# VIS4ROB-lab/covins

Hardware: AMD Instinct MI355X
Metric: GBA iterations/sec, 5-agent EuRoC merged map (higher is better)
Workload: dtype f64

## Files before the change

covins_amd/csrc/common.hpp:

```cpp
#pragma once
#include <hip/hip_runtime.h>
#include <atomic>
#include <cstdlib>
#include <stdint.h>

#include <map>
#include <unordered_map>
#include <utility>
#include <vector>

#include "../../include/covgpu.h"

namespace covgpu {

constexpr int kTile = 128;

struct DevProblem {
  int K, A, L, O, I, E, S;
  int D;
  int n;
  int npad;
  int N;
  int vi;
  int lm_group;
  double reproj_loss_a, gravity;

  double *pose, *sb, *lm;
  double *pose_c, *sb_c, *lm_c;
  double *pose0, *sb0, *lm0;
  uint8_t* fixed;
  int* kf_cam;
  double *cam_extr, *cam_intr, *cam_dist;
  int* cam_dist_type;

  int *lm_obs_ptr, *obs_kf, *obs_lm;
  double *obs_u, *obs_v, *obs_sigma;

  int *kf_obs_ptr, *kf_obs_idx;
  double* kobs;
  int *kobs_lm, *obs_zpos;
  int npairs;
  int *pair_ptr, *pair_i, *pair_j;
  int *pair_oa, *pair_ob;
  double *obsZ;
  double *lmRT;
  double *cost_part;

  int *imu_i, *imu_j, *imu_ptr;
  double *imu_samples, *imu_first;
  double *imu_noise;
  double *pre_delta;
  double *pre_J;
  double *pre_P;
  double *pre_W;
  double *pre_bias;

  int *edge_i, *edge_j;
  double *edge_meas, *edge_sqrt_info, *edge_loss_a;

  int nchains;
  int max_chain_len;
  int* perm;
  int* pos_kf;
  int* chain_ptr;
  int* pos_chain_end;

  double* Sred;
  double* bred;
  double *Ad, *Ae;
  double *Bp, *Bs, *Bn;
  int* pos_chain_begin;
  double* bp;
  double* grad;
  double* hdiag;
  double* HllInv;
  double* gn;
  double* step;
  double* vtmp;
  double* Linv;
  double* scal;
  double* part;
  int part_n, part_imu, part_edge, part_vec;
  double *imuAd, *imuBs, *imuCd, *imuG;
  double* edgeOut;
  int *kf_edge_ptr, *kf_edge_ent;
  int nepairs;
  int *epair_ptr, *epair_i, *epair_j, *epair_ent;
  int* flag;

  int shard;
  double* vw;

  int nd, nd_nnodes, nd_nlev, nd_maxd;
  int *nd_vnode, *nd_voff, *nd_vord;
  int *nd_vown;
  int *nd_ndepth, *nd_nI;
  long long* nd_ntab;
  int* nd_abase;
  int* nd_fidx;
  double *nd_M, *nd_rhs, *nd_Linv;
  double* nd_dummy;

  double* tr;
  double* scal_r; int* flag_r;

  int uni;
  int* cam_model;
  double* cam_xi;
};

enum {
  TR_RADIUS = 0, TR_MU, TR_LMDF, TR_COST, TR_ALPHA, TR_GG, TR_GN2, TR_GDOT, TR_DNORM, TR_CG, TR_CN, TR_MODEL, TR_SN, TR_RHO, TR_COSTNEW,
  TR_OK, TR_VALID, TR_ACC, TR_TERM, TR_FNCONV, TR_RETRY, TR_FIRST, TR_INITCOST, TR_REUSE,
  TR_JA, TR_JB, TR_JC, TR_VV, TR_VG, TR_NN, TR_XN2,
  TR_COUNT = 32
};
static_assert(TR_XN2 < TR_COUNT, "trust-region state slots");
struct TrConsts {
  int strategy;
  double max_radius, min_relative_decrease, function_tolerance, parameter_tolerance, gradient_tolerance;
};

__device__ __forceinline__ double* nd_entry(const DevProblem& P, int va, int vb, int ra, int rb) {
  const int na = P.nd_vnode[va], nb = P.nd_vnode[vb];
  if (na < 0 || nb < 0) return P.nd_dummy;
  if (na == nb) {
    const int oa = P.nd_voff[va] + ra, ob = P.nd_voff[vb] + rb;
    const int hi = oa > ob ? oa : ob, lo = oa > ob ? ob : oa;
    return P.nd_M + P.nd_ntab[2 * na] + (size_t)hi * (size_t)P.nd_ntab[2 * na + 1] + lo;
  }
  const int da = P.nd_ndepth[na], db = P.nd_ndepth[nb];
  const int no = da > db ? na : nb, vo = da > db ? va : vb, ro = da > db ? ra : rb;
  const int vA = da > db ? vb : va, rA = da > db ? rb : ra, dA = da > db ? db : da;
  const int base = P.nd_abase[(size_t)no * P.nd_maxd + dA];
  const int row = base < 0 ? -1 : P.nd_fidx[base + P.nd_vord[vA]];
  if (row < 0) return P.nd_dummy;
  return P.nd_M + P.nd_ntab[2 * no] + (size_t)(row + rA) * (size_t)P.nd_ntab[2 * no + 1] + (P.nd_voff[vo] + ro);
}

__device__ __forceinline__ double* c_entry(const DevProblem& P, int pi, int pj, int r, int c) {
  if (P.nd) return nd_entry(P, 2 * pi, 2 * pj, r, c);
  return P.Sred + (size_t)(6 * pi + r) * P.npad + (6 * pj + c);
}

enum { SC_COST = 0, SC_JV2 = 1, SC_GG = 2, SC_GN2 = 3, SC_GDOT = 4, SC_GMAX = 5, SC_GS = 6, SC_SN2 = 7, SC_XN2 = 8,
       SC_VV = 9, SC_VG = 10, SC_NN = 11, SC_JA = 12, SC_JB = 13, SC_JC = 14,
       SC_COUNT = 16 };

struct CholAux;
inline bool first_use_on_device(std::atomic<unsigned long long>& seen) {
  int d = 0;
  if (hipGetDevice(&d) != hipSuccess || d < 0 || d > 63) return true;
  const unsigned long long bit = 1ull << d;
  return (seen.fetch_or(bit, std::memory_order_acq_rel) & bit) == 0;
}
struct DevSignal { long long* flag = nullptr; long long seq = 0; };
inline int env_int(const char* name, int fallback) {
  const char* e = getenv(name);
  return e != nullptr ? atoi(e) : fallback;
}
void launch_kobs_build(const DevProblem& P, int* pair_oa, int* pair_ob, size_t nent, hipStream_t st);
void launch_lm_lin(const DevProblem& P, double mu, hipStream_t st, DevSignal sig = DevSignal());
void launch_lm_build(const DevProblem& P, double mu, hipStream_t st, hipEvent_t pose_system_cleared = nullptr, hipStream_t side = nullptr,
                     hipEvent_t ev_lin = nullptr, hipEvent_t ev_kf = nullptr, CholAux* ax = nullptr);
void launch_lm_backsub(const DevProblem& P, const double* dp, double* out_all, hipStream_t st);
void launch_obs_jvp(const DevProblem& P, const double* v_all, hipStream_t st);
void launch_obs_cost(const DevProblem& P, const double* pose, const double* lm, hipStream_t st);
void launch_obs_linearize(const DevProblem& P, double* r, double* Jp, double* Jl, double* cost, hipStream_t st);
void launch_obs_norms(const DevProblem& P, double* norms, hipStream_t st);
void launch_lm_outliers(const DevProblem& P, double th, unsigned char* erase, int* left, unsigned long long* counts, hipStream_t st);

void launch_preintegrate(const DevProblem& P, hipStream_t st);
void launch_imu_build(const DevProblem& P, hipStream_t st);
void launch_imu_jvp(const DevProblem& P, const double* v_all, hipStream_t st);
void launch_imu_cost(const DevProblem& P, const double* pose, const double* sb, hipStream_t st);
void launch_imu_linearize(const DevProblem& P, double* r, double* J, hipStream_t st);

void launch_edge_build(const DevProblem& P, hipStream_t st);
void launch_edge_jvp(const DevProblem& P, const double* v_all, hipStream_t st);
void launch_edge_cost(const DevProblem& P, const double* pose, hipStream_t st);
void launch_edge_linearize(const DevProblem& P, double* r, double* J, double* cost, hipStream_t st);

void launch_finalize_diag(const DevProblem& P, double mu, int which, hipStream_t st);
void launch_part_clear(const DevProblem& P, int slot0, int nslots, hipStream_t st);
void launch_part_finish(const DevProblem& P, int slot0, int nslots, hipStream_t st);
void launch_imu_gather(const DevProblem& P, int which, hipStream_t st);
void launch_edge_gather(const DevProblem& P, hipStream_t st);
struct PgoPlan;
void launch_pose_graph_solve(const DevProblem& P, double* dst, hipStream_t st, CholAux& ax, PgoPlan* pgo);
void launch_zero_system(const DevProblem& P, hipStream_t st);
enum KernelForm {
  KF_POTRF_PANEL = 0, KF_POTRF_PANEL_FRONTS, KF_POTRF_PANEL4, KF_POTRF_PANEL4_FRONTS, KF_POTRF_SKIPPED,
  KF_TRSM_SUB4_4, KF_TRSM_SUB4_8, KF_TRSM_SUB4_12, KF_TRSM_SUB4_16,
  KF_GEMM_TRI_FULL, KF_GEMM_TRI_QUAD, KF_GEMM_TRI_GRID, KF_GEMM_RECT_FULL, KF_GEMM_RECT_QUAD,
  KF_BULK_ONE_LAUNCH, KF_BULK_TWO_LAUNCHES, KF_LAST_UPDATE_WHOLE, KF_LAST_UPDATE_SPLIT, KF_PANEL_ONE_TILE, KF_KD_CUT, KF_KD_ZERO, KF_GEMM_BETA0,
  KF_BWD_FRONT, KF_BWD_PIPE, KF_BWD_PIPE64, KF_BWD_TREE, KF_BWD_TREE64, KF_BWD_GIVEN, KF_BWD_STEP_SUB,
  KF_ND_EXTEND_REC, KF_ND_EXTEND, KF_ND_EXTEND_SPLIT,
  KF_ND_TOP_PACK, KF_ND_GH, KF_ND_TOP_DAMP, KF_ND_PANEL_XFER, KF_DIST_PANEL,
  KF_PGO_ARROW, KF_PGO_DENSE,
  KF_COUNT
};
extern const char* const kFormNames[KF_COUNT];
struct FormCensus { long long n[KF_COUNT] = {}; };
extern thread_local FormCensus* t_forms;
inline void form_hit(int f, long long k = 1) { if (t_forms != nullptr) t_forms->n[f] += k; }
struct FormScope {
  FormCensus* prev;
  explicit FormScope(FormCensus* c) : prev(t_forms) { t_forms = c; }
  ~FormScope() { t_forms = prev; }
  FormScope(const FormScope&) = delete; FormScope& operator=(const FormScope&) = delete;
};
struct CholAux {
  hipStream_t aux = nullptr, mid = nullptr, head = nullptr;
  hipEvent_t ev_fill = nullptr;
  hipEvent_t ev_xb = nullptr;
  int* bwd_cnt = nullptr;
  double* bwd_scr = nullptr; size_t bwd_scr_elems = 0;
  double* bwd_pipe = nullptr; size_t bwd_pipe_elems = 0;
  bool pipe_broken = false;
  hipEvent_t ev_xa = nullptr;
  hipEvent_t ev_zero = nullptr;
  hipEvent_t ev_lin = nullptr, ev_kf = nullptr;
  std::vector<hipEvent_t> ev, prof_ev, panel_ev;
  std::vector<double> prof_flops;
  std::vector<hipEvent_t> prof_ev2;
  std::vector<double> prof_flops2;
  double potrf_ms = 0, potrf_flops = 0;
  long n_potrf = 0;
  struct TriCache {
    std::vector<int*> list; std::vector<int> count; int key = -1;
    std::vector<int*> listC; std::vector<int> countC;
    int *listA = nullptr, *listB = nullptr; int countA = 0, countB = 0;
    void clear();
  };
  FormCensus forms;
  TriCache tri0;
  std::vector<TriCache> tri_lev;
  void tri_clear();
  void (*reduce)(void* ctx, double* dev, size_t n, int op, hipStream_t st) = nullptr;
  void* reduce_ctx = nullptr;
  int panel_n = 0;
  std::vector<int> panel_tag;
  void mark(hipStream_t s, int tag);
  bool profile = false;
  double syrk_ms = 0, syrk_flops = 0;
  long n_syrk = 0;
  void init();
  void destroy();
// ... 27 lines not shown
  const int *own_g = nullptr, *st_g = nullptr, *own_dims = nullptr, *st_dims = nullptr;
  double* x = nullptr;
  int first = 0;
};
struct DenseBatch {
  int n = 0; size_t sM = 0, sL = 0, sR = 0;
  const int* live = nullptr; int tI = 0; const int* live_h = nullptr;
  const long long* tab = nullptr;
  int tri_slot = -1;
  BwdXfer xfer;
  int split_ta = 0;
  hipEvent_t pre_trsm = nullptr;
  int* bwd_cnt = nullptr;
  double* bwd_scr = nullptr;
  double* bwd_pipe = nullptr;
  int *pipe_dead = nullptr, *pipe_dead_h = nullptr; double pipe_timeout_s = 3.0;
  const int* own_dims_h = nullptr;
  const int* own_dims = nullptr;
  const int* beta0_off = nullptr; const int* beta0 = nullptr;
  const int* plist = nullptr; const int* pbig_h = nullptr; const int* psmall_h = nullptr;
  int own_max = 0;
};
void dense_cholesky_solve_raw(double* S, double* b, double* Linv, int* flag, int npad, hipStream_t st, CholAux& ax, int tstop = -1,
                              bool solve = true, DenseBatch bt = DenseBatch());
struct DistPanels {
  int np = 0;
  const int* const* tri = nullptr;
  const int* tri_cnt = nullptr;
  bool lead = false;
  void (*exchange)(void* ctx, int P) = nullptr;
  void* ctx = nullptr;
};
void dense_cholesky_dist(double* S, double* b, double* Linv, int* flag, int npad, hipStream_t st, CholAux& ax, int tstop, DenseBatch bt,
                         const DistPanels& d);
constexpr int kBwdFrontMaxTiles = 4;
constexpr int kBwdPipeMinTiles = 2;
bool bwd_pipe_on();
void dense_backward_solve(double* S, double* b, double* Linv, int npad, hipStream_t st, int tfact, int tend, DenseBatch bt = DenseBatch());
void launch_potrf_panel(double* S, size_t ld, int t0, int w, double* Linv, int* flag, double* b, int npad, int nbt, size_t sM, size_t sL, size_t sR,
                        hipStream_t st, const long long* btab = nullptr, int nb = -1, const int* own = nullptr, const int* list = nullptr, int n_big = 0,
                        int n_small = 0);
void launch_bwd_given(const double* S, size_t ld, int r0, int r1, double* y, double* x, int ncol, int nbt, size_t sM, size_t sR, hipStream_t st,
                      const long long* btab, const int* live, int tI, BwdXfer xf = BwdXfer());
void launch_bwd_front(const double* S, int tI, int ntiles, int nchunk, double* y, const double* Linv, int nbt, size_t sL, size_t sR, hipStream_t st,
                      const long long* btab, const int* live, BwdXfer xf, int* cnt, double* scr);
void launch_bwd_pipe(const double* S, int tI, int ntiles, int nchunk, double* y, const double* Linv, int nbt, size_t sL, size_t sR, hipStream_t st,
                     const long long* btab, const int* live, BwdXfer xf, double* pipe, int* dead, int* dead_h, double timeout_s);
void launch_pipe_fill(double* buf, size_t n, hipStream_t st);
constexpr int kBwdTreeMax = 8;
constexpr int kPipeChunk = 128;
struct BwdTreeLevel {
  int nbt, T, nchunk, tI, first;
  double* y; size_t bsR; const double* Dinv; size_t bsL; const long long* btab; const int* live;
  size_t scr_off, xpub_off;
};
void launch_bwd_tree(const double* M, const BwdTreeLevel* lev, int nlev, BwdXfer xf, double* pipe, int* dead, int* dead_h, double timeout_s, hipStream_t st,
                     bool form64 = false);
unsigned long long pipe_empty_word();
void launch_trsm_sub(double* S, size_t ld, int t0, int w, int r0, int r1, const double* Linv, double* b, int npad, int nbt, size_t sM, size_t sL,
                     size_t sR, const int* live, int tI, hipStream_t st, bool chain = false, const long long* btab = nullptr, int nb = -1, const int* own = nullptr);
void launch_bwd_step_sub(const double* S, size_t ld, int p, const double* Linv_p, double* y, double* x, int ncol, int nblocks, int nbt, size_t sM,
                         size_t sL, size_t sR, hipStream_t st, const long long* btab = nullptr, const int* live = nullptr, int tI = 0,
                         BwdXfer xf = BwdXfer());

struct PgoHostPlan { std::vector<std::vector<int>> block_kf; std::vector<int> border_kf; };
bool pgo_plan_analyse(int K, int E, const int* ei, const int* ej, PgoHostPlan& out);
struct PgoPlan {
  bool active = false;
  int nblk = 0, nIpad = 0, ntot = 0;
  int nb = 0;
  int* idx = nullptr;
  double *M = nullptr, *rhs = nullptr, *Linv = nullptr;
  int* idx_b = nullptr;
  double *Sb = nullptr, *rhs_b = nullptr, *Linv_b = nullptr;
};
void launch_pgo_block_solve(const DevProblem& P, PgoPlan& plan, hipStream_t st, CholAux& ax);

struct PairLists {
  int npairs = 0; size_t nent = 0;
  int *pair_ptr = nullptr, *pair_i = nullptr, *pair_j = nullptr;
  int *pair_oa = nullptr, *pair_ob = nullptr;
};
bool build_pairs_device(int L, int K, const int* d_lm_obs_ptr, const int* d_obs_kf, const int* d_key_of_kf, bool want_obs, hipStream_t st, PairLists& out);
void launch_obs_unpack(int L, int O, const int* lm_obs_ptr, const double* uv, int* obs_lm, double* u, double* v, int* iota, hipStream_t st);
bool build_kf_lists_device(int O, int K, const int* d_obs_kf, const int* d_iota, int* kf_obs_ptr, int* kf_obs_idx, hipStream_t st);
struct Round2Lists {
  int L2 = 0, O2 = 0;
  double *lm0 = nullptr, *obs_u = nullptr, *obs_v = nullptr, *obs_sigma = nullptr;
  int *lm_obs_ptr = nullptr, *lm_old = nullptr, *obs_kf = nullptr, *obs_lm = nullptr, *kf_obs_ptr = nullptr, *kf_obs_idx = nullptr;
  void free_all() {
    for (void* q : {(void*)lm0, (void*)obs_u, (void*)obs_v, (void*)obs_sigma, (void*)lm_obs_ptr, (void*)lm_old, (void*)obs_kf, (void*)obs_lm, (void*)kf_obs_ptr, (void*)kf_obs_idx})
      if (q) (void)hipFree(q);
  }
};
bool round2_compact_device(int L, int O, int K, const unsigned char* d_erase, const int* d_left, const int* d_obs_kf, const int* d_obs_lm, const double* d_u,
                           const double* d_v, const double* d_sigma, const double* d_lm0, hipStream_t st, Round2Lists& out);

struct NdHostPlan;
constexpr int kExtRec = 144;
struct NdLevel {
  int n = 0, nI = 0, ntot = 0;
  int first = 0;
  size_t rhs_off = 0, linv_off = 0;
  int* live = nullptr;
  std::vector<int> live_h;
  int own_max = 0;
  int* plist = nullptr; std::vector<int> plist_h, pbig, psmall;
  int ext_first = 0, ext_count = 0;
  int ext_countA = 0;
  int split_ta = 0;
  int ext2_first = 0, ext2_count = 0, ext2_countA = 0;
  std::vector<int> dx_first, dx_nt, dx_nr, dt_first, dt_cnt;
  std::vector<const int*> dt_dev;
};
struct NdDev {
  bool active = false;
  int nnodes = 0;
  int top_lev0 = 0;
  std::vector<NdLevel> lev;
  int *own_dims = nullptr, *st_dims = nullptr, *own_g = nullptr, *st_g = nullptr;
  int *gidx = nullptr;
  int tree_levels = 0; int* tree_fill = nullptr; std::vector<int> h_tree_fill;
  int tree_top0 = 0;
  int *cptr = nullptr, *cidx = nullptr;
  int *cptr2 = nullptr, *cidx2 = nullptr;
  int *inv_off = nullptr, *inv = nullptr;
  int *rhs_node = nullptr;
  int *ext = nullptr;
  int *extw = nullptr, *extc = nullptr, *extc2 = nullptr;
  std::vector<int> h_extw, h_extc, h_extc2, h_ext_kind;
  int* extr = nullptr; size_t ext_over = 0; std::vector<int> h_extr;
  int *bb_off = nullptr, *bb = nullptr;
  int *top_var = nullptr, *top_r = nullptr, *top_g = nullptr;
  int ntop = 0;
  int* top_tiles = nullptr; int n_top_tiles = 0; double* top_pack = nullptr;
  std::vector<int> h_top_tiles;
  size_t M_sub = 0, rhs_top = 0, gh_off = 0;
  std::vector<int> h_vnode, h_voff, h_vord, h_vown, h_ndepth, h_nI, h_abase, h_fidx, h_own_dims, h_st_dims, h_own_g, h_st_g, h_gidx, h_cptr, h_cidx, h_cptr2,
      h_cidx2, h_inv_off, h_inv, h_rhs_node, h_ext, h_top_var, h_top_r, h_top_g, h_bb_off, h_bb;
  std::vector<long long> h_ntab;
  bool dist = false, dist_lead = false;
  int* dist_ent = nullptr; int* dist_tri = nullptr; double* dist_buf = nullptr;
  std::vector<int> h_dist_ent, h_dist_tri;
  size_t dist_buf_elems = 0, dist_solve_elems = 0;
  size_t M_elems = 0, rhs_elems = 0, linv_elems = 0;
  double plan_flops = 0;
};
void nd_tables(const NdHostPlan& hp, const int* pos_kf, int D, int rank, NdDev& dev);
void launch_nd_init(const DevProblem& P, const NdDev& nd, hipStream_t st);
void launch_nd_zero(const DevProblem& P, const NdDev& nd, hipStream_t st);
bool launch_nd_solve(const DevProblem& P, NdDev& nd, double* dst, double mu, hipStream_t st, CholAux& ax);

void launch_tail_stats(const DevProblem& P, hipStream_t st);
void launch_tail_jvp(const DevProblem& P, bool two, hipStream_t st);
void launch_tail_cost(const DevProblem& P, hipStream_t st);
void launch_tail_finish(const DevProblem& P, TrConsts tc, int stage, bool two, bool with_logic, int fresh, hipStream_t st);
void launch_tail_logic(const DevProblem& P, TrConsts tc, int stage, int fresh, hipStream_t st);
void launch_tail_apply(const DevProblem& P, hipStream_t st);

void launch_dogleg_stats(const DevProblem& P, hipStream_t st);
void launch_cauchy_vec(const DevProblem& P, hipStream_t st);
void launch_combine_step(const DevProblem& P, double cg, double cn, hipStream_t st);
void launch_tr_after_solve(const DevProblem& P, TrConsts tc, int fresh, hipStream_t st);
void launch_combine_step_dev(const DevProblem& P, hipStream_t st);
void launch_tr_after_model(const DevProblem& P, TrConsts tc, hipStream_t st);
void launch_tr_decide(const DevProblem& P, TrConsts tc, hipStream_t st);
void launch_apply_step(const DevProblem& P, hipStream_t st);
void launch_accept(const DevProblem& P, hipStream_t st);
void launch_tr_accept(const DevProblem& P, hipStream_t st, double* box = nullptr, double seq = 0.0);
void launch_xnorm(const DevProblem& P, hipStream_t st);
void launch_relpose(int num, const int* ptr, const double* pB, const double* pA, const double* kpA, const double* kpB, const double* sigA,
                    const double* sigB, const double* camA, const int* distA, const double* camB, const int* distB, double th, int min_inliers,
                    double* T, unsigned char* outlier, int* inliers, hipStream_t st,
                    const int* modelA = nullptr, const double* xiA = nullptr, const int* modelB = nullptr, const double* xiB = nullptr);
void launch_abspose(int num, const int* ptr, const double* f, const double* P, const double* sig, const unsigned long long* seed, double* T,
                    unsigned char* inlier, int* inliers, int* iterations, int* best_draw, int min_inliers, int max_iterations, double probability,
                    double threshold, int max_n, hipStream_t st);
void launch_p3p(int num, const double* F, const double* P, double* T, int* nsol, int* chosen, hipStream_t st);
constexpr int kMatchScanRows = 256;
size_t match_assign_lds_bytes(int maxA, int maxB);
void launch_match(int mode, int num_jobs, int maxA, int maxB, const unsigned char* desc, const unsigned char* skip, const int* row_ptr,
                  const int* set_a, const int* set_b, const int* out_off, int* lists, int* match, int* dist, int* nmatches, int dcut,
                  float thr, float ratio, hipStream_t st);
void launch_reanchor(int K, const double* pose_old, const double* pose_new, double* vel, int L, const int* ref, double* lm,
                     hipStream_t st);

}
```

covins_amd/csrc/k_inertial.hip:

```cpp
#include "common.hpp"
#include "dev_math.hpp"
#include "reduce.hpp"
#include "inertial_dev.hpp"

namespace covgpu {
using namespace covdev;

__global__ __launch_bounds__(64 * kImuWaves) void k_preintegrate(DevProblem P) {
  __shared__ double sm[kImuWaves][225 * 4 + 270];
  const int lane = threadIdx.x & 63, wave = threadIdx.x >> 6;
  const int f = blockIdx.x * kImuWaves + wave;
  const bool live = f < P.I;
  double* F = sm[wave];
  double* J = F + 225;
  double* C = J + 225;
  double* T = C + 225;
  double* V = T + 225;
  const int fj = live ? P.imu_j[f] : 0;
  const V3 ba = ld3(P.sb + 9 * fj + 3), bg = ld3(P.sb + 9 * fj + 6);
  for (int k = lane; k < 225; k += 64) { F[k] = 0.0; J[k] = (k % 16 == 0) ? 1.0 : 0.0; C[k] = 0.0; }
  for (int k = lane; k < 270; k += 64) V[k] = 0.0;
  V3 dp = v3(0, 0, 0), dv = v3(0, 0, 0);
  Q4 dq = Q4{0, 0, 0, 1};
  double dtsum = 0.0;
// ... 72 lines not shown
    __syncthreads();
    if (on) {
#pragma unroll
      for (int u = 0; u < 4; ++u) {
        const int e = lane + 64 * u;
        if (e < 225) { J[e] = jn[u]; T[e] = tn[u]; }
      }
    }
    __syncthreads();
    if (on) {
#pragma unroll
      for (int u = 0; u < 4; ++u) {
        const int e = lane + 64 * u;
        if (e < 225) {
          const int r = e / 15, c = e - 15 * r;
          double s2 = 0.0;
#pragma unroll
          for (int k = 0; k < 15; ++k) s2 += T[15 * r + k] * F[15 * c + k];
#pragma unroll
          for (int k = 0; k < 18; ++k) s2 += V[18 * r + k] * nd[k / 3] * V[18 * c + k];
          C[e] = s2;
        }
      }
    }
    __syncthreads();
  }
  if (!live) return;
  if (lane == 0) {
    double* d = P.pre_delta + 11 * (size_t)f;
    d[0] = dp.x; d[1] = dp.y; d[2] = dp.z; d[3] = dq.x; d[4] = dq.y; d[5] = dq.z; d[6] = dq.w;
    d[7] = dv.x; d[8] = dv.y; d[9] = dv.z; d[10] = dtsum;
    double* pb = P.pre_bias + 6 * (size_t)f;
    pb[0] = ba.x; pb[1] = ba.y; pb[2] = ba.z; pb[3] = bg.x; pb[4] = bg.y; pb[5] = bg.z;
  }
  for (int k = lane; k < 225; k += 64) { P.pre_J[225 * (size_t)f + k] = J[k]; P.pre_P[225 * (size_t)f + k] = C[k]; }
  __builtin_amdgcn_fence(__ATOMIC_ACQ_REL, "workgroup");
  __builtin_amdgcn_wave_barrier();
  double* Wm = P.pre_W + 225 * (size_t)f;
  if (lane == 0) {
    bool ok = true;
    for (int c = 0; c < 15 && ok; ++c) {
      double dd = C[16 * c];
      for (int k = 0; k < c; ++k) dd -= C[15 * c + k] * C[15 * c + k];
      if (!(dd > 0.0)) { ok = false; break; }
      dd = sqrt(dd);
      C[16 * c] = dd;
      for (int r = c + 1; r < 15; ++r) {
        double s2 = C[15 * r + c];
        for (int k = 0; k < c; ++k) s2 -= C[15 * r + k] * C[15 * c + k];
        C[15 * r + c] = s2 / dd;
      }
    }
    for (int k = 0; k < 225; ++k) F[k] = 0.0;
    if (!ok) atomicAdd(P.flag + 1, 1);
    if (ok)
      for (int c = 0; c < 15; ++c) {
        F[16 * c] = 1.0 / C[16 * c];
        for (int r = c + 1; r < 15; ++r) {
          double s2 = 0.0;
          for (int k = c; k < r; ++k) s2 += C[15 * r + k] * F[15 * k + c];
          F[15 * r + c] = -s2 / C[16 * r];
        }
      }
    for (int k = 0; k < 225; ++k) Wm[k] = F[k];
  }
}

__global__ __launch_bounds__(64 * kImuWaves) void k_imu_build(DevProblem P) {
  __shared__ double sm[kImuWaves][kImuLds];
  const int lane = threadIdx.x & 63, wave = threadIdx.x >> 6;
  const int f = blockIdx.x * kImuWaves + wave;
  const bool live = f < P.I;
  double* sl = sm[wave];
  imu_stage<true>(P, P.pose, P.sb, f, live, lane, sl);
  {
    double c2 = (live && lane < 15) ? 0.5 * sl[1141 + lane] * sl[1141 + lane] : 0.0;
    c2 = wave_sum(c2);
    part_put(P, SC_COST, P.part_imu + blockIdx.x * kImuWaves + wave, c2);
  }
  if (!live) return;
  const double* Jw = sl + 450;
  const double* r = sl + 1141;
  const int i = P.imu_i[f], j = P.imu_j[f];
  const int pi = P.perm[i], pj = P.perm[j];
  const size_t K = (size_t)P.K;
  if (lane < 30) {
    const int a = lane, role = a / 15, la = a % 15;
    double ga = 0.0, haa = 0.0;
    for (int k = 0; k < 15; ++k) { ga += Jw[30 * k + a] * r[k]; haa += Jw[30 * k + a] * Jw[30 * k + a]; }
    double* g = P.imuG + (role * K + (role ? pj : pi)) * 30;
    g[la] = ga; g[15 + la] = haa;
  }
  for (int e = lane; e < 900; e += 64) {
    const int a = e / 30, b = e - 30 * a;
    const int ga_ = a / 15, la = a % 15, gb_ = b / 15, lb = b % 15;
    double h = 0.0;
#pragma unroll
    for (int k = 0; k < 15; ++k) h += Jw[30 * k + a] * Jw[30 * k + b];
    const size_t slot = ga_ * K + (ga_ ? pj : pi);
    if (la < 6 && lb < 6) {
      if (ga_ == gb_) P.imuCd[slot * 36 + 6 * la + lb] = h;
      else if (ga_ == 1) P.imuCd[(2 * K + pj) * 36 + 6 * la + lb] = h;
    } else if (la >= 6 && lb >= 6) {
      if (ga_ == gb_) P.imuAd[slot * 81 + 9 * (la - 6) + (lb - 6)] = h;
      else if (ga_ == 1) P.Ae[(size_t)81 * pj + 9 * (la - 6) + (lb - 6)] = h;
    } else if (la >= 6) {
      if (ga_ == gb_) P.imuBs[slot * 54 + 6 * (la - 6) + lb] = h;
      else if (ga_ == 0) P.Bn[(size_t)54 * pi + 6 * (la - 6) + lb] = h;
      else P.Bp[(size_t)54 * pj + 6 * (la - 6) + lb] = h;
    }
  }
}

__global__ __launch_bounds__(256) void k_imu_gather(DevProblem P, int which) {
  const int t = blockIdx.x * blockDim.x + threadIdx.x;
  const int pos = t / 201, e = t - 201 * pos;
  if (pos >= P.K) return;
  const size_t K = (size_t)P.K, s0 = (size_t)pos, s1 = K + pos;
  if (e < 81) {
    if (which != 0) P.Ad[81 * s0 + e] = P.imuAd[81 * s0 + e] + P.imuAd[81 * s1 + e];
  } else if (e < 135) {
    const int q = e - 81;
    if (which != 0) P.Bs[54 * s0 + q] = P.imuBs[54 * s0 + q] + P.imuBs[54 * s1 + q];
  } else if (e < 171) {
    const int q = e - 135, r = q / 6, c = q - 6 * r;
    if (which != 1) {
      if (c <= r) *c_entry(P, pos, pos, r, c) += P.imuCd[36 * s0 + q] + P.imuCd[36 * s1 + q];
      const double x = P.imuCd[36 * (2 * K + pos) + q];
      if (x != 0.0) *c_entry(P, pos, pos - 1, r, c) += x;
    }
  } else {
    const int q = e - 171, kf = P.pos_kf[pos];
    const int dim = q < 15 ? q : q - 15;
    if (which != 2 && (which == 0) != (dim < 6)) return;
    const double v = P.imuG[30 * s0 + q] + P.imuG[30 * s1 + q];
    if (q < 15) { P.grad[(size_t)15 * kf + q] += v; P.bred[(size_t)15 * kf + q] -= v; }
    else P.hdiag[(size_t)15 * kf + q - 15] += v;
  }
}

__global__ __launch_bounds__(64 * kImuWaves) void k_imu_jvp(DevProblem P, const double* __restrict__ v_all) {
  __shared__ double sm[kImuWaves][kImuLds];
  const int lane = threadIdx.x & 63, wave = threadIdx.x >> 6;
  const int f = blockIdx.x * kImuWaves + wave;
  const bool live = f < P.I;
  double* sl = sm[wave];
  imu_stage<true>(P, P.pose, P.sb, f, live, lane, sl);
  double acc = 0.0;
  if (live && lane < 15) {
    const double* Jw = sl + 450;
    const double* vi = v_all + 15 * (size_t)P.imu_i[f];
    const double* vj = v_all + 15 * (size_t)P.imu_j[f];
    double s2 = 0.0;
    for (int c = 0; c < 15; ++c) s2 += Jw[30 * lane + c] * vi[c] + Jw[30 * lane + 15 + c] * vj[c];
    acc = s2 * s2;
  }
  acc = wave_sum(acc);
  part_put(P, SC_JV2, P.part_imu + blockIdx.x * kImuWaves + wave, acc);
}

__global__ __launch_bounds__(64 * kImuWaves) void k_imu_cost(DevProblem P, const double* __restrict__ pose, const double* __restrict__ sb) {
  __shared__ double sm[kImuWaves][kImuLds];
  const int lane = threadIdx.x & 63, wave = threadIdx.x >> 6;
  const int f = blockIdx.x * kImuWaves + wave;
  const bool live = f < P.I;
  double* sl = sm[wave];
// ... 48 lines not shown
```

covins_amd/csrc/k_pairs.hip:

```cpp
#include <rocprim/device/device_radix_sort.hpp>
#include <rocprim/device/device_run_length_encode.hpp>
#include <rocprim/device/device_scan.hpp>

#include <algorithm>

#include "common.hpp"

namespace covgpu {

__global__ __launch_bounds__(256) void k_pair_count(int L, const int* __restrict__ lm_obs_ptr, const int* __restrict__ obs_kf, const int* __restrict__ key_of_kf,
                                                     unsigned long long* __restrict__ cnt) {
  const int l = blockIdx.x * blockDim.x + threadIdx.x;
  if (l >= L) return;
  const int o0 = lm_obs_ptr[l], o1 = lm_obs_ptr[l + 1];
  unsigned long long n = 0;
  for (int a = o0; a < o1; ++a) {
    const int pa = key_of_kf[obs_kf[a]];
    if (pa < 0) continue;
    for (int b = o0; b < o1; ++b) { const int pb = key_of_kf[obs_kf[b]]; n += (pb >= 0 && pb < pa) ? 1 : 0; }
  }
  cnt[l] = n;
}
__global__ __launch_bounds__(256) void k_pair_emit(int L, const int* __restrict__ lm_obs_ptr, const int* __restrict__ obs_kf, const int* __restrict__ key_of_kf,
                                                    const unsigned long long* __restrict__ off, unsigned long long* __restrict__ keys,
// ... 90 lines not shown
  R2_HIP(hipMalloc((void**)&keepO, (size_t)O * 4)); R2_HIP(hipMalloc((void**)&opos, (size_t)O * 4));
  hipLaunchKernelGGL(k_r2_keep_lm, dim3((L + 255) / 256), dim3(256), 0, st, L, d_left, keepL);
  hipLaunchKernelGGL(k_r2_keep_obs, dim3((O + 255) / 256), dim3(256), 0, st, O, d_erase, d_obs_lm, (const unsigned*)keepL, keepO);
  if (!scan(keepL, lpos, (size_t)L) || !scan(keepO, opos, (size_t)O)) { ok = false; goto done; }
  R2_HIP(hipMemcpyAsync(&tail[0], keepL + (L - 1), 4, hipMemcpyDeviceToHost, st)); R2_HIP(hipMemcpyAsync(&tail[1], lpos + (L - 1), 4, hipMemcpyDeviceToHost, st));
  R2_HIP(hipMemcpyAsync(&tail[2], keepO + (O - 1), 4, hipMemcpyDeviceToHost, st)); R2_HIP(hipMemcpyAsync(&tail[3], opos + (O - 1), 4, hipMemcpyDeviceToHost, st));
  R2_HIP(hipStreamSynchronize(st));
  out.L2 = (int)(tail[0] + tail[1]); out.O2 = (int)(tail[2] + tail[3]);
  {
    const size_t L2 = (size_t)std::max(out.L2, 1), O2 = (size_t)std::max(out.O2, 1);
    R2_HIP(hipMalloc((void**)&out.lm0, 3 * L2 * 8)); R2_HIP(hipMalloc((void**)&out.lm_obs_ptr, (L2 + 1) * 4)); R2_HIP(hipMalloc((void**)&out.lm_old, L2 * 4));
    R2_HIP(hipMalloc((void**)&out.obs_kf, O2 * 4)); R2_HIP(hipMalloc((void**)&out.obs_lm, O2 * 4));
    R2_HIP(hipMalloc((void**)&out.obs_u, O2 * 8)); R2_HIP(hipMalloc((void**)&out.obs_v, O2 * 8)); R2_HIP(hipMalloc((void**)&out.obs_sigma, O2 * 8));
    R2_HIP(hipMalloc((void**)&out.kf_obs_ptr, ((size_t)K + 1) * 4)); R2_HIP(hipMalloc((void**)&out.kf_obs_idx, O2 * 4));
    R2_HIP(hipMalloc((void**)&nobs, L2 * 4)); R2_HIP(hipMalloc((void**)&nw, L2 * 4)); R2_HIP(hipMalloc((void**)&nscan, L2 * 4));
    R2_HIP(hipMalloc((void**)&iota, O2 * 4)); R2_HIP(hipMalloc((void**)&keys2, O2 * 4));
    R2_HIP(hipMalloc((void**)&kcnt, (size_t)K * 4)); R2_HIP(hipMalloc((void**)&kscan, (size_t)K * 4));
    R2_HIP(hipMemsetAsync(kcnt, 0, (size_t)K * 4, st));
    R2_HIP(hipMemsetAsync(out.lm_obs_ptr, 0, (L2 + 1) * 4, st)); R2_HIP(hipMemsetAsync(out.kf_obs_ptr, 0, ((size_t)K + 1) * 4, st));
  }
  if (out.L2 > 0 && out.O2 > 0) {
    hipLaunchKernelGGL(k_r2_gather_lm, dim3((L + 255) / 256), dim3(256), 0, st, L, (const unsigned*)keepL, (const unsigned*)lpos, d_left, d_lm0, out.lm0, nobs, out.lm_old);
    hipLaunchKernelGGL(k_r2_gather_obs, dim3((O + 255) / 256), dim3(256), 0, st, O, (const unsigned*)keepO, (const unsigned*)opos, (const unsigned*)lpos, d_obs_kf, d_obs_lm,
                       d_u, d_v, d_sigma, out.obs_kf, out.obs_lm, out.obs_u, out.obs_v, out.obs_sigma, iota);
    hipLaunchKernelGGL(k_r2_widen, dim3((out.L2 + 255) / 256), dim3(256), 0, st, out.L2, (const int*)nobs, nw);
    if (!scan(nw, nscan, (size_t)out.L2)) { ok = false; goto done; }
    hipLaunchKernelGGL(k_r2_ptr, dim3((out.L2 + 255) / 256), dim3(256), 0, st, out.L2, (const unsigned*)nscan, (const unsigned*)nw, out.lm_obs_ptr);
    hipLaunchKernelGGL(k_r2_kf_count, dim3((out.O2 + 255) / 256), dim3(256), 0, st, out.O2, (const int*)out.obs_kf, kcnt);
    if (!scan(kcnt, kscan, (size_t)K)) { ok = false; goto done; }
    hipLaunchKernelGGL(k_r2_ptr, dim3((K + 255) / 256), dim3(256), 0, st, K, (const unsigned*)kscan, (const unsigned*)kcnt, out.kf_obs_ptr);
    {
      size_t b = 0;
      R2_HIP(rocprim::radix_sort_pairs(nullptr, b, out.obs_kf, keys2, iota, out.kf_obs_idx, (size_t)out.O2, 0u, (unsigned)kbits, st));
      if (!need_tmp(b)) { ok = false; goto done; }
      R2_HIP(rocprim::radix_sort_pairs(tmp, b, out.obs_kf, keys2, iota, out.kf_obs_idx, (size_t)out.O2, 0u, (unsigned)kbits, st));
    }
  }
  R2_HIP(hipStreamSynchronize(st));
done:
  for (void* q : {(void*)keepL, (void*)keepO, (void*)lpos, (void*)opos, (void*)kcnt, (void*)kscan, (void*)nw, (void*)nscan, (void*)nobs, (void*)iota, (void*)keys2, tmp}) if (q) (void)hipFree(q);
  if (!ok) { out.free_all(); out = Round2Lists(); }
  return ok;
}

__global__ __launch_bounds__(256) void k_obs_unpack(int L, int O, const int* __restrict__ lm_obs_ptr, const double* __restrict__ uv, int* __restrict__ obs_lm,
                                                     double* __restrict__ u, double* __restrict__ v, int* __restrict__ iota) {
  const int t = blockIdx.x * 256 + threadIdx.x;
  if (t < O) { u[t] = uv[2 * (size_t)t]; v[t] = uv[2 * (size_t)t + 1]; iota[t] = t; }
  if (t < L) for (int o = lm_obs_ptr[t]; o < lm_obs_ptr[t + 1]; ++o) obs_lm[o] = t;
}
bool build_kf_lists_device(int O, int K, const int* d_obs_kf, const int* d_iota, int* kf_obs_ptr, int* kf_obs_idx, hipStream_t st) {
  bool ok = true;
  unsigned *kcnt = nullptr, *kscan = nullptr; int* keys2 = nullptr; void* tmp = nullptr;
  int kbits = 1;
  while ((1 << kbits) < K) ++kbits;
  if (hipMemsetAsync(kf_obs_ptr, 0, ((size_t)K + 1) * 4, st) != hipSuccess) return false;
  if (O <= 0) return true;
  if (hipMalloc((void**)&kcnt, (size_t)K * 4) != hipSuccess || hipMalloc((void**)&kscan, (size_t)K * 4) != hipSuccess || hipMalloc((void**)&keys2, (size_t)O * 4) != hipSuccess) ok = false;
  if (ok) {
    (void)hipMemsetAsync(kcnt, 0, (size_t)K * 4, st);
    hipLaunchKernelGGL(k_r2_kf_count, dim3((O + 255) / 256), dim3(256), 0, st, O, d_obs_kf, kcnt);
    size_t b1 = 0, b2 = 0;
    ok = rocprim::exclusive_scan(nullptr, b1, kcnt, kscan, 0u, (size_t)K, rocprim::plus<unsigned>(), st) == hipSuccess &&
         rocprim::radix_sort_pairs(nullptr, b2, d_obs_kf, keys2, d_iota, kf_obs_idx, (size_t)O, 0u, (unsigned)kbits, st) == hipSuccess;
    const size_t b = std::max(b1, b2);
    if (ok && hipMalloc(&tmp, std::max<size_t>(b, 16)) != hipSuccess) ok = false;
    if (ok) {
      size_t bb = b1;
      ok = rocprim::exclusive_scan(tmp, bb, kcnt, kscan, 0u, (size_t)K, rocprim::plus<unsigned>(), st) == hipSuccess;
      hipLaunchKernelGGL(k_r2_ptr, dim3((K + 255) / 256), dim3(256), 0, st, K, (const unsigned*)kscan, (const unsigned*)kcnt, kf_obs_ptr);
      bb = b2;
      ok = ok && rocprim::radix_sort_pairs(tmp, bb, d_obs_kf, keys2, d_iota, kf_obs_idx, (size_t)O, 0u, (unsigned)kbits, st) == hipSuccess;
      ok = ok && hipStreamSynchronize(st) == hipSuccess;
    }
  }
  for (void* q : {(void*)kcnt, (void*)kscan, (void*)keys2, tmp}) if (q) (void)hipFree(q);
  return ok;
}
void launch_obs_unpack(int L, int O, const int* lm_obs_ptr, const double* uv, int* obs_lm, double* u, double* v, int* iota, hipStream_t st) {
  const int n = std::max(L, O);
  if (n > 0) hipLaunchKernelGGL(k_obs_unpack, dim3((n + 255) / 256), dim3(256), 0, st, L, O, lm_obs_ptr, uv, obs_lm, u, v, iota);
}

#define PB_HIP(expr) do { if ((expr) != hipSuccess) { ok = false; goto done; } } while (0)

bool build_pairs_device(int L, int K, const int* d_lm_obs_ptr, const int* d_obs_kf, const int* d_key_of_kf, bool want_obs, hipStream_t st, PairLists& out) {
  out = PairLists();
  bool ok = true;
  unsigned long long *d_cnt = nullptr, *d_off = nullptr, *d_keys = nullptr, *d_vals = nullptr, *d_keys2 = nullptr, *d_vals2 = nullptr, *d_uniq = nullptr, *d_scan = nullptr;
  int *d_counts = nullptr, *d_nruns = nullptr;
  void* d_tmp = nullptr; size_t tmp_bytes = 0;
  unsigned long long total = 0, last_cnt = 0, last_off = 0;
  int nruns = 0;
  int kbits = 1;
  while ((1 << kbits) < K) ++kbits;
  auto need_tmp = [&](size_t bytes) { if (bytes > tmp_bytes) { if (d_tmp) (void)hipFree(d_tmp); d_tmp = nullptr; if (hipMalloc(&d_tmp, bytes) != hipSuccess) return false; tmp_bytes = bytes; } return true; };
  if (L <= 0) { goto empty; }
  PB_HIP(hipMalloc((void**)&d_cnt, (size_t)L * 8)); PB_HIP(hipMalloc((void**)&d_off, (size_t)L * 8));
  hipLaunchKernelGGL(k_pair_count, dim3((L + 255) / 256), dim3(256), 0, st, L, d_lm_obs_ptr, d_obs_kf, d_key_of_kf, d_cnt);
  {
    size_t b = 0;
    PB_HIP(rocprim::exclusive_scan(nullptr, b, d_cnt, d_off, 0ull, (size_t)L, rocprim::plus<unsigned long long>(), st));
    if (!need_tmp(b)) { ok = false; goto done; }
    PB_HIP(rocprim::exclusive_scan(d_tmp, b, d_cnt, d_off, 0ull, (size_t)L, rocprim::plus<unsigned long long>(), st));
  }
  PB_HIP(hipMemcpyAsync(&last_cnt, d_cnt + (L - 1), 8, hipMemcpyDeviceToHost, st));
  PB_HIP(hipMemcpyAsync(&last_off, d_off + (L - 1), 8, hipMemcpyDeviceToHost, st));
  PB_HIP(hipStreamSynchronize(st));
  total = last_cnt + last_off;
  if (total == 0) goto empty;
  if (total >= (1ull << 31)) { ok = false; goto done; }
  PB_HIP(hipMalloc((void**)&d_keys, total * 8)); PB_HIP(hipMalloc((void**)&d_vals, total * 8));
  PB_HIP(hipMalloc((void**)&d_keys2, total * 8)); PB_HIP(hipMalloc((void**)&d_vals2, total * 8));
  hipLaunchKernelGGL(k_pair_emit, dim3((L + 255) / 256), dim3(256), 0, st, L, d_lm_obs_ptr, d_obs_kf, d_key_of_kf, d_off, d_keys, d_vals);
  {
    size_t b = 0;
    PB_HIP(rocprim::radix_sort_pairs(nullptr, b, d_keys, d_keys2, d_vals, d_vals2, (size_t)total, 0u, (unsigned)(32 + kbits), st));
    if (!need_tmp(b)) { ok = false; goto done; }
    PB_HIP(rocprim::radix_sort_pairs(d_tmp, b, d_keys, d_keys2, d_vals, d_vals2, (size_t)total, 0u, (unsigned)(32 + kbits), st));
  }
  PB_HIP(hipMalloc((void**)&d_counts, total * 4)); PB_HIP(hipMalloc((void**)&d_nruns, 4));
  d_uniq = d_keys;
  {
    size_t b = 0;
    PB_HIP(rocprim::run_length_encode(nullptr, b, d_keys2, (unsigned)total, d_uniq, d_counts, d_nruns, st));
    if (!need_tmp(b)) { ok = false; goto done; }
    PB_HIP(rocprim::run_length_encode(d_tmp, b, d_keys2, (unsigned)total, d_uniq, d_counts, d_nruns, st));
  }
  PB_HIP(hipMemcpyAsync(&nruns, d_nruns, 4, hipMemcpyDeviceToHost, st));
  PB_HIP(hipStreamSynchronize(st));
  out.npairs = nruns; out.nent = (size_t)total;
  PB_HIP(hipMalloc((void**)&out.pair_i, (size_t)nruns * 4)); PB_HIP(hipMalloc((void**)&out.pair_j, (size_t)nruns * 4));
  PB_HIP(hipMalloc((void**)&out.pair_ptr, ((size_t)nruns + 1) * 4));
  hipLaunchKernelGGL(k_pair_split, dim3((unsigned)((nruns + 255) / 256)), dim3(256), 0, st, (size_t)nruns, d_uniq, out.pair_i, out.pair_j);
  d_scan = d_vals;
  if ((size_t)2 * nruns > total) { d_scan = nullptr; PB_HIP(hipMalloc((void**)&d_scan, (size_t)2 * nruns * 8)); }
  hipLaunchKernelGGL(k_count_widen, dim3((nruns + 255) / 256), dim3(256), 0, st, nruns, d_counts, d_scan);
  {
    size_t b = 0;
    PB_HIP(rocprim::exclusive_scan(nullptr, b, d_scan, d_scan + nruns, 0ull, (size_t)nruns, rocprim::plus<unsigned long long>(), st));
    if (!need_tmp(b)) { ok = false; goto done; }
    PB_HIP(rocprim::exclusive_scan(d_tmp, b, d_scan, d_scan + nruns, 0ull, (size_t)nruns, rocprim::plus<unsigned long long>(), st));
  }
  hipLaunchKernelGGL(k_pair_ptr, dim3((nruns + 255) / 256), dim3(256), 0, st, nruns, d_scan + nruns, d_counts, out.pair_ptr);
  if (want_obs) {
    PB_HIP(hipMalloc((void**)&out.pair_oa, (size_t)total * 4)); PB_HIP(hipMalloc((void**)&out.pair_ob, (size_t)total * 4));
    hipLaunchKernelGGL(k_pair_split, dim3((unsigned)((total + 255) / 256)), dim3(256), 0, st, (size_t)total, d_vals2, out.pair_oa, out.pair_ob);
  }
  PB_HIP(hipStreamSynchronize(st));
  goto done;
empty:
  PB_HIP(hipMalloc((void**)&out.pair_ptr, 4)); PB_HIP(hipMemsetAsync(out.pair_ptr, 0, 4, st));
  PB_HIP(hipMalloc((void**)&out.pair_i, 4)); PB_HIP(hipMalloc((void**)&out.pair_j, 4));
  if (want_obs) { PB_HIP(hipMalloc((void**)&out.pair_oa, 4)); PB_HIP(hipMalloc((void**)&out.pair_ob, 4)); }
  PB_HIP(hipStreamSynchronize(st));
done:
  if (d_scan != nullptr && d_scan != d_vals) (void)hipFree(d_scan);
  for (void* q : {(void*)d_cnt, (void*)d_off, (void*)d_keys, (void*)d_vals, (void*)d_keys2, (void*)d_vals2, (void*)d_counts, (void*)d_nruns, d_tmp}) if (q) (void)hipFree(q);
  if (!ok) { for (int* q : {out.pair_ptr, out.pair_i, out.pair_j, out.pair_oa, out.pair_ob}) if (q) (void)hipFree(q); out = PairLists(); }
  return ok;
}

}
```

covins_amd/csrc/k_tail.hip:

```cpp
#include "between_dev.hpp"
#include "common.hpp"
#include "dev_math.hpp"
#include "inertial_dev.hpp"
#include "reduce.hpp"
#include "visual_dev.hpp"

namespace covgpu {
using namespace covdev;

static inline int tail_grid(int n, int cap) {
  const int b = (n + 255) / 256;
  return b < 1 ? 1 : (b > cap ? cap : b);
}
COV_DEV void tail_put(const DevProblem& P, double v, int slot, int index) {
  v = wave_sum(v);
  part_put(P, slot, index, v);
}

__global__ __launch_bounds__(256) void k_tail_stats(DevProblem P) {
  double gg = 0, gn2 = 0, gd = 0, gm = 0, vv = 0, vg = 0, nn = 0, xn = 0;
  const int stride = gridDim.x * blockDim.x, t0 = blockIdx.x * blockDim.x + threadIdx.x;
  for (int q = t0; q < P.N; q += stride) {
    const double g = P.grad[q], d = clamp_diag(P.hdiag[q]), s = P.gn[q];
    const double w = P.vw ? P.vw[q] : 1.0;
    const double c = g / (d * d);
    P.vtmp[q] = c;
    gg += w * (g / d) * (g / d); gn2 += w * (d * s) * (d * s); gd += w * g * s; gm = fmax(gm, w * fabs(g));
    vv += w * c * c; vg += w * c * s; nn += w * s * s;
  }
  for (int t = t0; t < P.K; t += stride) {
    const double wp = P.vw ? P.vw[(size_t)P.D * t] : 1.0, ws = (P.vw && P.vi) ? P.vw[(size_t)P.D * t + 6] : 1.0;
    if (!P.fixed[t]) for (int k = 0; k < 7; ++k) xn += wp * P.pose[7 * t + k] * P.pose[7 * t + k];
    if (P.vi) for (int k = 0; k < 9; ++k) xn += ws * P.sb[9 * t + k] * P.sb[9 * t + k];
  }
  for (int q = t0; q < 3 * P.L; q += stride) xn += P.lm[q] * P.lm[q];
  const int idx = P.part_vec + blockIdx.x * 4 + (threadIdx.x >> 6);
  tail_put(P, gg, SC_GG, idx); tail_put(P, gn2, SC_GN2, idx); tail_put(P, gd, SC_GDOT, idx);
  tail_put(P, vv, SC_VV, idx); tail_put(P, vg, SC_VG, idx); tail_put(P, nn, SC_NN, idx); tail_put(P, xn, SC_XN2, idx);
#pragma unroll
  for (int off = 32; off >= 1; off >>= 1) gm = fmax(gm, __shfl_xor(gm, off, 64));
  if ((threadIdx.x & 63) == 0) atomicMax(reinterpret_cast<unsigned long long*>(&P.scal[SC_GMAX]), (unsigned long long)__double_as_longlong(gm));
}

static_assert(kImuWaves == 4, "k_tail_jvp / k_tail_cost index their IMU and edge segments as 4 waves / 256 threads per workgroup");
template <bool TWO, bool UNI>
__global__ __launch_bounds__(64 * kImuWaves) void k_tail_jvp(DevProblem P, const double* __restrict__ va, const double* __restrict__ vb, int nb_obs, int nb_imu) {
  __shared__ double sm[kImuWaves][kImuLds];
  const int lane = threadIdx.x & 63, wave = threadIdx.x >> 6;
  double ja = 0.0, jb = 0.0, jc = 0.0;
  int idx;
  if ((int)blockIdx.x < nb_obs) {
    for (int o = blockIdx.x * blockDim.x + threadIdx.x; o < P.O; o += nb_obs * blockDim.x) {
      ObsLin e;
      const int kf = P.obs_kf[o], l = P.obs_lm[o];
      eval_obs<true, UNI>(P, P.pose, P.lm, o, kf, l, e);
      {
        const double* vp = vb + (size_t)P.D * kf;
        const double* vl = vb + P.n + 3 * (size_t)l;
        double s0 = e.jl[0] * vl[0] + e.jl[1] * vl[1] + e.jl[2] * vl[2];
        double s1 = e.jl[3] * vl[0] + e.jl[4] * vl[1] + e.jl[5] * vl[2];
#pragma unroll
        for (int k = 0; k < 6; ++k) { s0 += e.jp[k] * vp[k]; s1 += e.jp[6 + k] * vp[k]; }
        jb += s0 * s0 + s1 * s1;
        if (TWO) {
          const double* up = va + (size_t)P.D * kf;
          const double* ul = va + P.n + 3 * (size_t)l;
          double t0 = e.jl[0] * ul[0] + e.jl[1] * ul[1] + e.jl[2] * ul[2];
          double t1 = e.jl[3] * ul[0] + e.jl[4] * ul[1] + e.jl[5] * ul[2];
#pragma unroll
          for (int k = 0; k < 6; ++k) { t0 += e.jp[k] * up[k]; t1 += e.jp[6 + k] * up[k]; }
          ja += t0 * t0 + t1 * t1; jc += t0 * s0 + t1 * s1;
        }
      }
    }
    idx = blockIdx.x * 4 + wave;
  } else if ((int)blockIdx.x < nb_obs + nb_imu) {
    const int bi = blockIdx.x - nb_obs;
    const int f = bi * kImuWaves + wave;
    const bool live = f < P.I;
    double* sl = sm[wave];
    imu_stage<true>(P, P.pose, P.sb, f, live, lane, sl);
    if (live && lane < 15) {
      const double* Jw = sl + 450;
      const size_t oi = 15 * (size_t)P.imu_i[f], oj = 15 * (size_t)P.imu_j[f];
      double s2 = 0.0, t2 = 0.0;
      for (int c = 0; c < 15; ++c) {
        s2 += Jw[30 * lane + c] * vb[oi + c] + Jw[30 * lane + 15 + c] * vb[oj + c];
        if (TWO) t2 += Jw[30 * lane + c] * va[oi + c] + Jw[30 * lane + 15 + c] * va[oj + c];
      }
      jb = s2 * s2; ja = t2 * t2; jc = s2 * t2;
    }
    idx = P.part_imu + bi * kImuWaves + wave;
  } else {
    const int be = blockIdx.x - nb_obs - nb_imu;
    const int e = be * 256 + threadIdx.x;
    if (e < P.E) {
      double r[6], J[72];
      eval_edge<true>(P, P.pose, e, r, J);
      const size_t oi = (size_t)P.D * P.edge_i[e], oj = (size_t)P.D * P.edge_j[e];
#pragma unroll
      for (int a = 0; a < 6; ++a) {
        double s = 0.0, t = 0.0;
#pragma unroll
        for (int c = 0; c < 6; ++c) {
          s += J[12 * a + c] * vb[oi + c] + J[12 * a + 6 + c] * vb[oj + c];
          if (TWO) t += J[12 * a + c] * va[oi + c] + J[12 * a + 6 + c] * va[oj + c];
        }
        jb += s * s; ja += t * t; jc += s * t;
      }
    }
    idx = P.part_edge + be * 4 + wave;
    if (be * 4 + wave >= (P.E + 63) / 64) idx = -1;
  }
  jb = wave_sum(jb);
  if (TWO) { ja = wave_sum(ja); jc = wave_sum(jc); }
  if (idx >= 0) {
    part_put(P, SC_JB, idx, jb);
    if (TWO) { part_put(P, SC_JA, idx, ja); part_put(P, SC_JC, idx, jc); }
  }
}

template <bool UNI>
__global__ __launch_bounds__(64 * kImuWaves) void k_tail_cost(DevProblem P, int nb_obs, int nb_imu) {
  __shared__ double sm[kImuWaves][kImuLds];
  const int lane = threadIdx.x & 63, wave = threadIdx.x >> 6;
  double acc = 0.0;
  int idx;
  if ((int)blockIdx.x < nb_obs) {
    for (int o = blockIdx.x * blockDim.x + threadIdx.x; o < P.O; o += nb_obs * blockDim.x) {
      ObsLin e;
      eval_obs<false, UNI>(P, P.pose_c, P.lm_c, o, P.obs_kf[o], P.obs_lm[o], e);
      acc += e.cost;
    }
    idx = blockIdx.x * 4 + wave;
  } else if ((int)blockIdx.x < nb_obs + nb_imu) {
    const int bi = blockIdx.x - nb_obs;
    const int f = bi * kImuWaves + wave;
    const bool live = f < P.I;
    double* sl = sm[wave];
    imu_stage<false>(P, P.pose_c, P.sb_c, f, live, lane, sl);
    if (live && lane < 15) { const double rv = sl[1141 + lane]; acc = 0.5 * rv * rv; }
    idx = P.part_imu + bi * kImuWaves + wave;
  } else {
    const int be = blockIdx.x - nb_obs - nb_imu;
    const int e = be * 256 + threadIdx.x;
    if (e < P.E) { double r[6]; acc = eval_edge<false>(P, P.pose_c, e, r, nullptr); }
    idx = P.part_edge + be * 4 + wave;
    if (be * 4 + wave >= (P.E + 63) / 64) idx = -1;
  }
  acc = wave_sum(acc);
  if (idx >= 0) part_put(P, SC_COST, idx, acc);
}

struct ScalRead {
  const double* p; bool dev_scope;
  COV_DEV double operator()(int i) const { return dev_scope ? __hip_atomic_load(p + i, __ATOMIC_RELAXED, __HIP_MEMORY_SCOPE_AGENT) : p[i]; }
};
COV_DEV void tail_logic_a(const DevProblem& P, const TrConsts& tc, int fresh, const ScalRead& sc, int flag0) {
  double* t = P.tr;
  t[TR_RETRY] = 0.0; t[TR_VALID] = 0.0; t[TR_ACC] = 0.0; t[TR_FNCONV] = 0.0; t[TR_MODEL] = 0.0; t[TR_SN] = 0.0;
  if (fresh) {
    if (t[TR_FIRST] != 0.0) { t[TR_COST] = sc(SC_COST); t[TR_INITCOST] = sc(SC_COST); t[TR_FIRST] = 0.0; }
    const bool ok = flag0 == 0;
    t[TR_OK] = ok ? 1.0 : 0.0;
    if (!ok && tc.strategy == COVGPU_DOGLEG && t[TR_MU] * 10.0 < 1.0) { t[TR_MU] *= 10.0; t[TR_RETRY] = 1.0; return; }
    if (!ok && tc.strategy == COVGPU_DOGLEG) t[TR_MU] *= 10.0;
    if (sc(SC_GMAX) <= tc.gradient_tolerance) { t[TR_TERM] = 3.0; return; }
    t[TR_GG] = sc(SC_GG); t[TR_GN2] = sc(SC_GN2); t[TR_GDOT] = sc(SC_GDOT);
    t[TR_JA] = sc(SC_JA); t[TR_JB] = sc(SC_JB); t[TR_JC] = sc(SC_JC); t[TR_VV] = sc(SC_VV); t[TR_VG] = sc(SC_VG); t[TR_NN] = sc(SC_NN);
    t[TR_XN2] = sc(SC_XN2);
    if (tc.strategy == COVGPU_DOGLEG) t[TR_ALPHA] = t[TR_GG] / t[TR_JA];
  }
  double cg = 0.0, cn = 1.0;
  if (tc.strategy == COVGPU_DOGLEG) {
    const double radius = t[TR_RADIUS], alpha = t[TR_ALPHA], GG = t[TR_GG], GN2 = t[TR_GN2], GDOT = t[TR_GDOT];
    const double gn_norm = sqrt(GN2), g_norm = sqrt(GG);
    if (gn_norm <= radius) { cg = 0.0; cn = 1.0; t[TR_DNORM] = gn_norm; }
    else if (g_norm * alpha >= radius) { cg = -radius / g_norm; cn = 0.0; t[TR_DNORM] = radius; }
    else {
      const double b_dot_a = -alpha * GDOT, a_sq = alpha * alpha * GG;
      const double bma = GN2 - 2.0 * b_dot_a + a_sq, cc = b_dot_a - a_sq;
      const double dd = sqrt(cc * cc + bma * (radius * radius - a_sq));
      const double beta = (cc <= 0.0) ? (dd - cc) / bma : (radius * radius - a_sq) / (dd + cc);
      cg = -alpha * (1.0 - beta); cn = beta; t[TR_DNORM] = radius;
    }
  }
  t[TR_CG] = cg; t[TR_CN] = cn;
  if (t[TR_TERM] != 0.0) return;
  const bool ok = t[TR_OK] != 0.0;
  const double gs = cg * t[TR_GG] + cn * t[TR_GDOT];
  const double jv2 = cg * cg * t[TR_JA] + 2.0 * cg * cn * t[TR_JC] + cn * cn * t[TR_JB];
  const double sn2 = cg * cg * t[TR_VV] + 2.0 * cg * cn * t[TR_VG] + cn * cn * t[TR_NN];
  const double model = ok ? -(gs + 0.5 * jv2) : 0.0, sn = ok ? sqrt(fmax(sn2, 0.0)) : 0.0;
  t[TR_MODEL] = model; t[TR_SN] = sn;
  const bool valid = ok && model > 0.0;
  t[TR_VALID] = valid ? 1.0 : 0.0;
  if (valid && sn <= tc.parameter_tolerance * (sqrt(t[TR_XN2]) + tc.parameter_tolerance)) t[TR_TERM] = 2.0;
}
COV_DEV void tail_logic_b(const DevProblem& P, const TrConsts& tc, const ScalRead& sc) {
  double* t = P.tr;
  if (t[TR_RETRY] != 0.0 || t[TR_TERM] != 0.0) return;
  const bool lm = tc.strategy == COVGPU_LM;
  int acc = 0;
  if (t[TR_VALID] == 0.0) {
// ... 8 lines not shown
    acc = rho > tc.min_relative_decrease;
    if (acc) {
      t[TR_FNCONV] = fabs(cost - cost_new) <= tc.function_tolerance * cost ? 1.0 : 0.0;
      t[TR_COST] = cost_new;
      if (lm) {
        const double u = 2.0 * rho - 1.0;
        t[TR_RADIUS] = fmin(tc.max_radius, t[TR_RADIUS] / fmax(1.0 / 3.0, 1.0 - u * u * u));
        t[TR_LMDF] = 2.0;
      } else {
        if (rho < 0.25) t[TR_RADIUS] *= 0.5;
        if (rho > 0.75) t[TR_RADIUS] = fmax(t[TR_RADIUS], 3.0 * t[TR_DNORM]);
        t[TR_MU] = fmax(1e-8, 2.0 * t[TR_MU] / 10.0);
      }
      t[TR_REUSE] = 0.0;
    } else if (lm) { t[TR_RADIUS] /= t[TR_LMDF]; t[TR_LMDF] *= 2.0; t[TR_REUSE] = 0.0; }
    else { t[TR_RADIUS] *= 0.5; t[TR_REUSE] = 1.0; }
    if (t[TR_FNCONV] != 0.0) t[TR_TERM] = 1.0;
  }
  t[TR_ACC] = acc ? 1.0 : 0.0;
}

struct SlotList { int n; int slot[12]; };
__global__ __launch_bounds__(1024) void k_tail_finish(DevProblem P, SlotList sl, TrConsts tc, int logic, int fresh) {
  __shared__ double sc[1024];
  __shared__ int s_ticket;
  const int slot = sl.slot[blockIdx.x];
  const double* src = P.part + (size_t)slot * P.part_n;
  double a0 = 0.0, a1 = 0.0, a2 = 0.0, a3 = 0.0;
  int k = threadIdx.x;
  for (; k + 3072 < P.part_n; k += 4096) { a0 += src[k]; a1 += src[k + 1024]; a2 += src[k + 2048]; a3 += src[k + 3072]; }
  for (; k < P.part_n; k += 1024) a0 += src[k];
  sc[threadIdx.x] = (a0 + a1) + (a2 + a3);
  __syncthreads();
  for (int s2 = 512; s2 > 0; s2 >>= 1) {
    if (threadIdx.x < s2) sc[threadIdx.x] += sc[threadIdx.x + s2];
    __syncthreads();
  }
  if (logic == 0) { if (threadIdx.x == 0) P.scal[slot] = sc[0]; return; }
  if (threadIdx.x == 0) {
    __hip_atomic_store(&P.scal[slot], sc[0], __ATOMIC_RELAXED, __HIP_MEMORY_SCOPE_AGENT);
    asm volatile("s_waitcnt vmcnt(0)" ::: "memory");
    s_ticket = __hip_atomic_fetch_add(&P.flag[2], 1, __ATOMIC_ACQ_REL, __HIP_MEMORY_SCOPE_AGENT);
  }
  __syncthreads();
  if (s_ticket != (int)gridDim.x - 1 || threadIdx.x != 0) return;
  __hip_atomic_store(&P.flag[2], 0, __ATOMIC_RELAXED, __HIP_MEMORY_SCOPE_AGENT);
  const ScalRead rd{P.scal, true};
  if (logic == 1) tail_logic_a(P, tc, fresh, rd, __hip_atomic_load(&P.flag[0], __ATOMIC_RELAXED, __HIP_MEMORY_SCOPE_AGENT));
  else tail_logic_b(P, tc, rd);
}
__global__ void k_tail_logic(DevProblem P, TrConsts tc, int stage, int fresh) {
  if (threadIdx.x != 0 || blockIdx.x != 0) return;
  const ScalRead rd{P.scal_r, false};
  if (stage == 1) tail_logic_a(P, tc, fresh, rd, P.flag_r[0]);
  else tail_logic_b(P, tc, rd);
}

__global__ __launch_bounds__(256) void k_tail_apply(DevProblem P) {
  const double cg = P.tr[TR_CG], cn = P.tr[TR_CN];
  const int t = blockIdx.x * blockDim.x + threadIdx.x;
  auto st = [&](size_t q) { const double s = cn * P.gn[q]; return cg != 0.0 ? s + cg * P.vtmp[q] : s; };
  if (t < P.K) {
    const size_t b = (size_t)P.D * t;
    const double* x = P.pose + 7 * t;
    double* y = P.pose_c + 7 * t;
    if (P.fixed[t]) {
      for (int k = 0; k < 7; ++k) y[k] = x[k];
    } else {
      const Q4 q = qnormalize(qmul(ldq(x), qexp(V3{st(b), st(b + 1), st(b + 2)})));
      y[0] = q.x; y[1] = q.y; y[2] = q.z; y[3] = q.w;
      y[4] = x[4] + st(b + 3); y[5] = x[5] + st(b + 4); y[6] = x[6] + st(b + 5);
    }
    if (P.vi)
      for (int k = 0; k < 9; ++k) P.sb_c[9 * t + k] = P.sb[9 * t + k] + st(b + 6 + k);
  }
  for (int q = t; q < 3 * P.L; q += gridDim.x * blockDim.x) P.lm_c[q] = P.lm[q] + st((size_t)P.n + q);
}

static inline void tail_segments(const DevProblem& P, int& nb_obs, int& nb_imu, int& nb_edge) {
  nb_obs = P.O > 0 ? tail_grid(P.O, 2048) : 0;
  nb_imu = (P.vi && P.I > 0) ? (P.I + kImuWaves - 1) / kImuWaves : 0;
  nb_edge = P.E > 0 ? (P.E + 255) / 256 : 0;
}
void launch_tail_stats(const DevProblem& P, hipStream_t st) {
  hipLaunchKernelGGL(k_tail_stats, dim3(tail_grid(P.N, 256)), dim3(256), 0, st, P);
}
void launch_tail_jvp(const DevProblem& P, bool two, hipStream_t st) {
  int a, b, c;
  tail_segments(P, a, b, c);
  if (a + b + c == 0) return;
  if (P.uni) {
    if (two) hipLaunchKernelGGL((k_tail_jvp<true, true>), dim3(a + b + c), dim3(64 * kImuWaves), 0, st, P, (const double*)P.vtmp, (const double*)P.gn, a, b);
    else hipLaunchKernelGGL((k_tail_jvp<false, true>), dim3(a + b + c), dim3(64 * kImuWaves), 0, st, P, (const double*)nullptr, (const double*)P.gn, a, b);
    return;
  }
  if (two) hipLaunchKernelGGL((k_tail_jvp<true, false>), dim3(a + b + c), dim3(64 * kImuWaves), 0, st, P, (const double*)P.vtmp, (const double*)P.gn, a, b);
  else hipLaunchKernelGGL((k_tail_jvp<false, false>), dim3(a + b + c), dim3(64 * kImuWaves), 0, st, P, (const double*)nullptr, (const double*)P.gn, a, b);
}
void launch_tail_cost(const DevProblem& P, hipStream_t st) {
  int a, b, c;
  tail_segments(P, a, b, c);
  if (a + b + c == 0) return;
  if (P.uni) hipLaunchKernelGGL(k_tail_cost<true>, dim3(a + b + c), dim3(64 * kImuWaves), 0, st, P, a, b);
  else hipLaunchKernelGGL(k_tail_cost<false>, dim3(a + b + c), dim3(64 * kImuWaves), 0, st, P, a, b);
}
void launch_tail_finish(const DevProblem& P, TrConsts tc, int stage, bool two, bool with_logic, int fresh, hipStream_t st) {
  SlotList sl;
  sl.n = 0;
  auto add = [&](int s) { sl.slot[sl.n++] = s; };
  if (stage == 1) {
    add(SC_GG); add(SC_GN2); add(SC_GDOT); add(SC_VV); add(SC_VG); add(SC_NN); add(SC_XN2); add(SC_JB);
    if (two) { add(SC_JA); add(SC_JC); }
  } else add(SC_COST);
  for (int i = sl.n; i < 12; ++i) sl.slot[i] = 0;
  hipLaunchKernelGGL(k_tail_finish, dim3(sl.n), dim3(1024), 0, st, P, sl, tc, with_logic ? stage : 0, fresh);
}
void launch_tail_logic(const DevProblem& P, TrConsts tc, int stage, int fresh, hipStream_t st) {
  hipLaunchKernelGGL(k_tail_logic, dim3(1), dim3(64), 0, st, P, tc, stage, fresh);
}
void launch_tail_apply(const DevProblem& P, hipStream_t st) {
  const int n = P.K > 3 * P.L ? P.K : 3 * P.L;
  int g = (P.K + 255) / 256;
  const int g2 = tail_grid(n, 2048);
  if (g2 > g) g = g2;
  hipLaunchKernelGGL(k_tail_apply, dim3(g), dim3(256), 0, st, P);
}

}
```

covins_amd/csrc/k_visual.hip:

```cpp
#include <type_traits>

#include "common.hpp"
#include "dev_math.hpp"
#include "reduce.hpp"
#include "visual_dev.hpp"

namespace covgpu {
using namespace covdev;

COV_DEV void group_sync() {
  __builtin_amdgcn_fence(__ATOMIC_ACQ_REL, "workgroup");
  __builtin_amdgcn_wave_barrier();
}

template <int G>
COV_DEV double group_sum(double v) {
#pragma unroll
  for (int off = G / 2; off >= 1; off >>= 1) v += __shfl_xor(v, off, G);
  return v;
}

COV_DEV void inv3sym(const double* h, double* o) {
  const double c00 = h[3] * h[5] - h[4] * h[4], c01 = h[2] * h[4] - h[1] * h[5], c02 = h[1] * h[4] - h[2] * h[3];
  const double det = h[0] * c00 + h[1] * c01 + h[2] * c02;
  const double id = (fabs(det) > 0.0) ? 1.0 / det : 0.0;
  o[0] = c00 * id; o[1] = c01 * id; o[2] = c02 * id;
  o[3] = (h[0] * h[5] - h[2] * h[2]) * id; o[4] = (h[1] * h[2] - h[0] * h[4]) * id; o[5] = (h[0] * h[3] - h[1] * h[1]) * id;
}

constexpr int kBuildThreads = 256;

constexpr int kRec = 39;

COV_DEV void chol3(const double* h, double* r) {
  const double r00 = h[0] > 0.0 ? sqrt(h[0]) : 0.0, i00 = r00 > 0.0 ? 1.0 / r00 : 0.0;
  const double r10 = h[1] * i00, r20 = h[2] * i00;
  const double d1 = h[3] - r10 * r10, r11 = d1 > 0.0 ? sqrt(d1) : 0.0, i11 = r11 > 0.0 ? 1.0 / r11 : 0.0;
  const double r21 = (h[4] - r20 * r10) * i11;
  const double d2 = h[5] - r20 * r20 - r21 * r21, r22 = d2 > 0.0 ? sqrt(d2) : 0.0;
  r[0] = r00; r[1] = r10; r[2] = r11; r[3] = r20; r[4] = r21; r[5] = r22;
}
COV_DEV void z_of(const ObsLin& e, const double* R, double* Z) {
#pragma unroll
  for (int r = 0; r < 6; ++r) {
    const double w0 = e.jp[r] * e.jl[0] + e.jp[6 + r] * e.jl[3], w1 = e.jp[r] * e.jl[1] + e.jp[6 + r] * e.jl[4], w2 = e.jp[r] * e.jl[2] + e.jp[6 + r] * e.jl[5];
    Z[3 * r] = w0 * R[0] + w1 * R[1] + w2 * R[3];
    Z[3 * r + 1] = w1 * R[2] + w2 * R[4];
    Z[3 * r + 2] = w2 * R[5];
  }
}

template <int G, bool UNI>
__global__ __launch_bounds__(kBuildThreads) void k_lm_lin(DevProblem P, double mu, DevSignal sig) {
  constexpr int GROUPS = kBuildThreads / G;
  if (sig.flag != nullptr && blockIdx.x == 0 && threadIdx.x == 0) __hip_atomic_store(sig.flag, sig.seq, __ATOMIC_RELAXED, __HIP_MEMORY_SCOPE_AGENT);
  const int lane = threadIdx.x % G, grp = threadIdx.x / G;
  const int l = blockIdx.x * GROUPS + grp;
  const bool lm_ok = l < P.L;
  const int o0 = lm_ok ? P.lm_obs_ptr[l] : 0;
  const int nobs = lm_ok ? P.lm_obs_ptr[l + 1] - o0 : 0;
  const int nchunk = (nobs + G - 1) / G;

  double h[6] = {0, 0, 0, 0, 0, 0}, gl[3] = {0, 0, 0}, cost = 0.0;
  ObsLin e;
  int kf = 0;
  for (int c = 0; c < nchunk; ++c) {
    const int a = c * G + lane;
    if (a < nobs) {
      kf = P.obs_kf[o0 + a];
      eval_obs<true, UNI>(P, P.pose, P.lm, o0 + a, kf, l, e);
      h[0] += e.jl[0] * e.jl[0] + e.jl[3] * e.jl[3];
      h[1] += e.jl[0] * e.jl[1] + e.jl[3] * e.jl[4];
      h[2] += e.jl[0] * e.jl[2] + e.jl[3] * e.jl[5];
      h[3] += e.jl[1] * e.jl[1] + e.jl[4] * e.jl[4];
      h[4] += e.jl[1] * e.jl[2] + e.jl[4] * e.jl[5];
      h[5] += e.jl[2] * e.jl[2] + e.jl[5] * e.jl[5];
      gl[0] += e.jl[0] * e.r0 + e.jl[3] * e.r1;
      gl[1] += e.jl[1] * e.r0 + e.jl[4] * e.r1;
      gl[2] += e.jl[2] * e.r0 + e.jl[5] * e.r1;
      cost += e.cost;
    }
  }
#pragma unroll
  for (int k = 0; k < 6; ++k) h[k] = group_sum<G>(h[k]);
#pragma unroll
  for (int k = 0; k < 3; ++k) gl[k] = group_sum<G>(gl[k]);
  double hi[6];
  {
    double hd[6] = {h[0], h[1], h[2], h[3], h[4], h[5]};
    const double d0 = clamp_diag(h[0]), d1 = clamp_diag(h[3]), d2 = clamp_diag(h[5]);
    hd[0] += mu * d0 * d0; hd[3] += mu * d1 * d1; hd[5] += mu * d2 * d2;
    inv3sym(hd, hi);
  }
  double R[6];
  chol3(hi, R);
  if (lm_ok && lane == 0) {
    double* gg = P.grad + P.n + 3 * (size_t)l;
    double* hh = P.hdiag + P.n + 3 * (size_t)l;
    gg[0] = gl[0]; gg[1] = gl[1]; gg[2] = gl[2];
    hh[0] = h[0]; hh[1] = h[3]; hh[2] = h[5];
    double* hv = P.HllInv + 6 * (size_t)l;
#pragma unroll
    for (int k = 0; k < 6; ++k) hv[k] = hi[k];
    double* rt = P.lmRT + 9 * (size_t)l;
#pragma unroll
    for (int k = 0; k < 6; ++k) rt[k] = R[k];
    rt[6] = R[0] * gl[0] + R[1] * gl[1] + R[3] * gl[2];
    rt[7] = R[2] * gl[1] + R[4] * gl[2];
    rt[8] = R[5] * gl[2];
  }
  cost = wave_sum(cost);
  __shared__ double scost[kBuildThreads / 64];
  if ((threadIdx.x & 63) == 0) scost[threadIdx.x >> 6] = cost;
  __syncthreads();
  if (threadIdx.x == 0) {
    double c4 = 0.0;
#pragma unroll
    for (int k = 0; k < kBuildThreads / 64; ++k) c4 += scost[k];
    P.cost_part[blockIdx.x] = c4;
  }

  for (int c = 0; c < nchunk; ++c) {
    const int a = c * G + lane;
    if (a >= nobs) continue;
    if (nchunk > 1) {
      kf = P.obs_kf[o0 + a];
      eval_obs<true, UNI>(P, P.pose, P.lm, o0 + a, kf, l, e);
    }
    double Z[18];
    z_of(e, R, Z);
    double2* zo = reinterpret_cast<double2*>(P.obsZ + 18 * (size_t)P.obs_zpos[o0 + a]);
#pragma unroll
    for (int k = 0; k < 9; ++k) zo[k] = double2{Z[2 * k], Z[2 * k + 1]};
  }
}

__global__ __launch_bounds__(256) void k_cost_finish(DevProblem P, int nparts) {
  __shared__ double sc[256];
  double acc = 0.0;
  for (int k = threadIdx.x; k < nparts; k += 256) acc += P.cost_part[k];
  sc[threadIdx.x] = acc;
  __syncthreads();
  for (int s2 = 128; s2 > 0; s2 >>= 1) {
    if (threadIdx.x < s2) sc[threadIdx.x] += sc[threadIdx.x + s2];
    __syncthreads();
  }
  if (threadIdx.x == 0) P.part[(size_t)SC_COST * P.part_n + 0] = sc[0];
}

template <bool UNI>
__global__ __launch_bounds__(64) void k_kf_reduce(DevProblem P) {
  __shared__ double sp[kRec][65];
  const int kf = blockIdx.x, lane = threadIdx.x;
  if (P.fixed[kf]) return;
  const int o0 = P.kf_obs_ptr[kf], o1 = P.kf_obs_ptr[kf + 1];
  double part[kRec];
#pragma unroll
  for (int k = 0; k < kRec; ++k) part[k] = 0.0;
  for (int t = o0 + lane; t < o1; t += 64) {
    const int l = P.kobs_lm[t];
    const double* uvs = P.kobs + 3 * (size_t)t;
    ObsLin e;
    eval_obs_uvs<true, UNI>(P, P.pose, P.lm, uvs[0], uvs[1], uvs[2], kf, l, e);
    const double* rt = P.lmRT + 9 * (size_t)l;
    double R[6], Z[18];
#pragma unroll
    for (int k = 0; k < 6; ++k) R[k] = rt[k];
    const double t0 = rt[6], t1 = rt[7], t2 = rt[8];
    z_of(e, R, Z);
    int q = 0;
#pragma unroll
    for (int r = 0; r < 6; ++r)
#pragma unroll
      for (int cc = 0; cc <= r; ++cc)
        part[q++] += e.jp[r] * e.jp[cc] + e.jp[6 + r] * e.jp[6 + cc] - (Z[3 * r] * Z[3 * cc] + Z[3 * r + 1] * Z[3 * cc + 1] + Z[3 * r + 2] * Z[3 * cc + 2]);
#pragma unroll
    for (int r = 0; r < 6; ++r) {
      part[21 + r] += e.jp[r] * e.jp[r] + e.jp[6 + r] * e.jp[6 + r];
      part[27 + r] += e.jp[r] * e.r0 + e.jp[6 + r] * e.r1;
      part[33 + r] += Z[3 * r] * t0 + Z[3 * r + 1] * t1 + Z[3 * r + 2] * t2;
    }
  }
#pragma unroll
  for (int k = 0; k < kRec; ++k) sp[k][lane] = part[k];
  __syncthreads();
  double acc = 0.0;
  if (lane < kRec) {
    double a0 = 0.0, a1 = 0.0, a2 = 0.0, a3 = 0.0;
#pragma unroll
    for (int t = 0; t < 64; t += 4) { a0 += sp[lane][t]; a1 += sp[lane][t + 1]; a2 += sp[lane][t + 2]; a3 += sp[lane][t + 3]; }
    acc = (a0 + a1) + (a2 + a3);
  }
  const double gp = __shfl(acc, (lane >= 33 && lane < 39) ? lane - 6 : lane, 64);
  const size_t base = (size_t)P.D * kf;
  const int pos = P.perm[kf];
  if (lane < 21) {
    int r = 0;
    while ((r + 1) * (r + 2) / 2 <= lane) ++r;
    const int c = lane - r * (r + 1) / 2;
    *c_entry(P, pos, pos, r, c) = acc;
  } else if (lane < 27) {
    P.hdiag[base + lane - 21] = acc;
  } else if (lane < 33) {
    P.grad[base + lane - 27] = acc;
  } else if (lane < 39) {
    P.bred[base + lane - 33] = acc - gp;
  }
}

constexpr int kPairLanes = 16, kPairsPerWg = 8;
constexpr int kPairChunk = 64;
__global__ __launch_bounds__(kPairLanes * kPairsPerWg) void k_pair_blocks(DevProblem P) {
  __shared__ double sp[kPairsPerWg][36][kPairLanes + 1];
  const int grp = threadIdx.x / kPairLanes, g = threadIdx.x % kPairLanes;
  const int nblk = (P.npairs + kPairsPerWg - 1) / kPairsPerWg;
  const int kx = (int)blockIdx.x >> 3, xcd = (int)blockIdx.x & 7;
  const int lb = ((kx / kPairChunk) * 8 + xcd) * kPairChunk + kx % kPairChunk;
  const int p = lb * kPairsPerWg + grp;
  const bool ok = lb < nblk && p < P.npairs;
  const int e0 = ok ? P.pair_ptr[p] : 0, e1 = ok ? P.pair_ptr[p + 1] : 0;
  double acc[36];
#pragma unroll
  for (int k = 0; k < 36; ++k) acc[k] = 0.0;
  for (int e = e0 + g; e < e1; e += 2 * kPairLanes) {
    const int e2 = e + kPairLanes;
    const bool two = e2 < e1;
    const double2* y = reinterpret_cast<const double2*>(P.obsZ + 18 * (size_t)P.pair_oa[e]);
    const double2* w = reinterpret_cast<const double2*>(P.obsZ + 18 * (size_t)P.pair_ob[e]);
    const double2* y2 = reinterpret_cast<const double2*>(P.obsZ + 18 * (size_t)P.pair_oa[two ? e2 : e]);
    const double2* w2 = reinterpret_cast<const double2*>(P.obsZ + 18 * (size_t)P.pair_ob[two ? e2 : e]);
    double yv[18], wv[18], yu[18], wu[18];
#pragma unroll
    for (int k = 0; k < 9; ++k) {
      const double2 a2 = y[k], b2 = w[k], c2 = y2[k], d2 = w2[k];
      yv[2 * k] = a2.x; yv[2 * k + 1] = a2.y; wv[2 * k] = b2.x; wv[2 * k + 1] = b2.y;
      yu[2 * k] = c2.x; yu[2 * k + 1] = c2.y; wu[2 * k] = d2.x; wu[2 * k + 1] = d2.y;
    }
#pragma unroll
    for (int r = 0; r < 6; ++r)
#pragma unroll
      for (int c = 0; c < 6; ++c) acc[6 * r + c] += yv[3 * r] * wv[3 * c] + yv[3 * r + 1] * wv[3 * c + 1] + yv[3 * r + 2] * wv[3 * c + 2];
    if (two) {
#pragma unroll
      for (int r = 0; r < 6; ++r)
#pragma unroll
        for (int c = 0; c < 6; ++c) acc[6 * r + c] += yu[3 * r] * wu[3 * c] + yu[3 * r + 1] * wu[3 * c + 1] + yu[3 * r + 2] * wu[3 * c + 2];
    }
  }
#pragma unroll
  for (int k = 0; k < 36; ++k) sp[grp][k][g] = acc[k];
  __syncthreads();
  if (!ok) return;
  const int pi = P.pair_i[p], pj = P.pair_j[p];
  for (int k = g; k < 36; k += kPairLanes) {
    double a0 = 0.0, a1 = 0.0;
#pragma unroll
    for (int t = 0; t < kPairLanes; t += 2) { a0 += sp[grp][k][t]; a1 += sp[grp][k][t + 1]; }
    *c_entry(P, pi, pj, k / 6, k % 6) = -(a0 + a1);
  }
}

template <int G, bool UNI>
__global__ __launch_bounds__(kBuildThreads) void k_lm_backsub(DevProblem P, const double* __restrict__ dp, double* __restrict__ out_all) {
  constexpr int GROUPS = kBuildThreads / G;
  const int lane = threadIdx.x % G, grp = threadIdx.x / G;
  const int l = blockIdx.x * GROUPS + grp;
  const bool lm_ok = l < P.L;
  const int o0 = lm_ok ? P.lm_obs_ptr[l] : 0;
  const int nobs = lm_ok ? P.lm_obs_ptr[l + 1] - o0 : 0;
  double t[3] = {0, 0, 0};
  for (int a = lane; a < nobs; a += G) {
    ObsLin e;
    const int kf = P.obs_kf[o0 + a];
    eval_obs<true, UNI>(P, P.pose, P.lm, o0 + a, kf, l, e);
    const double* d = dp + (size_t)P.D * kf;
    const double s0 = e.jp[0] * d[0] + e.jp[1] * d[1] + e.jp[2] * d[2] + e.jp[3] * d[3] + e.jp[4] * d[4] + e.jp[5] * d[5];
    const double s1 = e.jp[6] * d[0] + e.jp[7] * d[1] + e.jp[8] * d[2] + e.jp[9] * d[3] + e.jp[10] * d[4] + e.jp[11] * d[5];
    t[0] += e.jl[0] * s0 + e.jl[3] * s1;
    t[1] += e.jl[1] * s0 + e.jl[4] * s1;
    t[2] += e.jl[2] * s0 + e.jl[5] * s1;
  }
#pragma unroll
  for (int k = 0; k < 3; ++k) t[k] = group_sum<G>(t[k]);
  if (lm_ok && lane == 0) {
    const double* gl = P.grad + P.n + 3 * (size_t)l;
    const double* hi = P.HllInv + 6 * (size_t)l;
    const double x = -gl[0] - t[0], y = -gl[1] - t[1], z = -gl[2] - t[2];
    double* o = out_all + P.n + 3 * (size_t)l;
    o[0] = hi[0] * x + hi[1] * y + hi[2] * z;
    o[1] = hi[1] * x + hi[3] * y + hi[4] * z;
    o[2] = hi[2] * x + hi[4] * y + hi[5] * z;
  }
}

template <bool UNI>
__global__ __launch_bounds__(256) void k_obs_jvp(DevProblem P, const double* __restrict__ v_all) {
  double acc = 0.0;
  for (int o = blockIdx.x * blockDim.x + threadIdx.x; o < P.O; o += gridDim.x * blockDim.x) {
    ObsLin e;
    const int kf = P.obs_kf[o], l = P.obs_lm[o];
    eval_obs<true, UNI>(P, P.pose, P.lm, o, kf, l, e);
    const double* vp = v_all + (size_t)P.D * kf;
    const double* vl = v_all + P.n + 3 * (size_t)l;
    double s0 = e.jl[0] * vl[0] + e.jl[1] * vl[1] + e.jl[2] * vl[2];
    double s1 = e.jl[3] * vl[0] + e.jl[4] * vl[1] + e.jl[5] * vl[2];
#pragma unroll
    for (int k = 0; k < 6; ++k) { s0 += e.jp[k] * vp[k]; s1 += e.jp[6 + k] * vp[k]; }
    acc += s0 * s0 + s1 * s1;
  }
  acc = wave_sum(acc);
  part_put(P, SC_JV2, blockIdx.x * 4 + (threadIdx.x >> 6), acc);
}

template <bool UNI>
__global__ __launch_bounds__(256) void k_obs_cost(DevProblem P, const double* __restrict__ pose, const double* __restrict__ lm) {
  double acc = 0.0;
  for (int o = blockIdx.x * blockDim.x + threadIdx.x; o < P.O; o += gridDim.x * blockDim.x) {
    ObsLin e;
    eval_obs<false, UNI>(P, pose, lm, o, P.obs_kf[o], P.obs_lm[o], e);
    acc += e.cost;
  }
  acc = wave_sum(acc);
  part_put(P, SC_COST, blockIdx.x * 4 + (threadIdx.x >> 6), acc);
}

template <bool UNI>
__global__ __launch_bounds__(256) void k_obs_linearize(DevProblem P, double* r, double* Jp, double* Jl, double* cost) {
  const int o = blockIdx.x * blockDim.x + threadIdx.x;
  if (o >= P.O) return;
  ObsLin e;
  eval_obs<true, UNI>(P, P.pose, P.lm, o, P.obs_kf[o], P.obs_lm[o], e);
  r[2 * o] = e.r0; r[2 * o + 1] = e.r1; cost[o] = e.cost;
  for (int k = 0; k < 12; ++k) Jp[12 * (size_t)o + k] = e.jp[k];
  for (int k = 0; k < 6; ++k) Jl[6 * (size_t)o + k] = e.jl[k];
}

template <bool UNI>
__global__ __launch_bounds__(256) void k_obs_norms(DevProblem P, double* norms) {
  const int o = blockIdx.x * blockDim.x + threadIdx.x;
  if (o >= P.O) return;
  ObsLin e;
  eval_obs<false, UNI>(P, P.pose, P.lm, o, P.obs_kf[o], P.obs_lm[o], e);
  norms[o] = sqrt(e.r0 * e.r0 + e.r1 * e.r1);
}

static inline int stream_grid(int n) {
  const int b = (n + 255) / 256;
  return b < 1 ? 1 : (b > 2048 ? 2048 : b);
}

template <typename F> static void with_group(int g, F&& f) {
  if (g == 4) f(std::integral_constant<int, 4>()); else if (g == 8) f(std::integral_constant<int, 8>()); else f(std::integral_constant<int, 16>());
}
template <typename F> static void with_uni(const DevProblem& P, F&& f) {
  if (P.uni) f(std::true_type()); else f(std::false_type());
}
static int lm_blocks(const DevProblem& P) { const int g = P.lm_group == 4 || P.lm_group == 8 ? P.lm_group : 16; const int groups = kBuildThreads / g; return (P.L + groups - 1) / groups; }

void launch_lm_lin(const DevProblem& P, double mu, hipStream_t st, DevSignal sig) {
  if (P.L == 0) return;
  const int nblk = lm_blocks(P);
  with_uni(P, [&](auto U) { with_group(P.lm_group, [&](auto G) {
    hipLaunchKernelGGL((k_lm_lin<decltype(G)::value, decltype(U)::value>), dim3(nblk), dim3(kBuildThreads), 0, st, P, mu, sig); }); });
}
void launch_lm_build(const DevProblem& P, double mu, hipStream_t st, hipEvent_t pose_system_cleared, hipStream_t side, hipEvent_t ev_lin, hipEvent_t ev_kf, CholAux* ax) {
  auto record = [&](hipEvent_t e, hipStream_t s) { if (ax) ax->record(e, s); else (void)hipEventRecord(e, s); };
  auto wait = [&](hipStream_t s, hipEvent_t e0, hipEvent_t e1 = nullptr) { if (ax) ax->wait(s, e0, e1); else { if (e0) (void)hipStreamWaitEvent(s, e0, 0); if (e1) (void)hipStreamWaitEvent(s, e1, 0); } };
  if (P.L == 0) { if (pose_system_cleared) wait(st, pose_system_cleared); return; }
  const int nblk = lm_blocks(P);
  const bool fork = side != nullptr && ev_lin != nullptr && ev_kf != nullptr && P.npairs > 0;
  hipStream_t s2 = fork ? side : st;
  if (fork) { record(ev_lin, st); wait(s2, ev_lin, pose_system_cleared); if (pose_system_cleared) wait(st, pose_system_cleared); }
  else if (pose_system_cleared) wait(s2, pose_system_cleared);
  hipLaunchKernelGGL(k_cost_finish, dim3(1), dim3(256), 0, s2, P, nblk);
  with_uni(P, [&](auto U) { hipLaunchKernelGGL(k_kf_reduce<decltype(U)::value>, dim3(P.K), dim3(64), 0, s2, P); });
  if (P.npairs) {
    const int nblk = (P.npairs + kPairsPerWg - 1) / kPairsPerWg;
    const int nchunk8 = (nblk + 8 * kPairChunk - 1) / (8 * kPairChunk);
    hipLaunchKernelGGL(k_pair_blocks, dim3(nchunk8 * 8 * kPairChunk), dim3(kPairLanes * kPairsPerWg), 0, st, P);
  }
}
__global__ __launch_bounds__(256) void k_kobs_build(DevProblem P) {
  const int t = blockIdx.x * blockDim.x + threadIdx.x;
  if (t >= P.O) return;
  const int o = P.kf_obs_idx[t];
  P.kobs[3 * (size_t)t] = P.obs_u[o]; P.kobs[3 * (size_t)t + 1] = P.obs_v[o]; P.kobs[3 * (size_t)t + 2] = P.obs_sigma[o];
  P.kobs_lm[t] = P.obs_lm[o];
  P.obs_zpos[o] = t;
}
__global__ __launch_bounds__(256) void k_remap_idx(size_t n, int* __restrict__ a, int* __restrict__ b, const int* __restrict__ map) {
  const size_t q = (size_t)blockIdx.x * 256 + threadIdx.x;
  if (q < n) { a[q] = map[a[q]]; b[q] = map[b[q]]; }
}
void launch_kobs_build(const DevProblem& P, int* pair_oa, int* pair_ob, size_t nent, hipStream_t st) {
  if (P.O == 0) return;
  hipLaunchKernelGGL(k_kobs_build, dim3((P.O + 255) / 256), dim3(256), 0, st, P);
  if (nent > 0) hipLaunchKernelGGL(k_remap_idx, dim3((unsigned)((nent + 255) / 256)), dim3(256), 0, st, nent, pair_oa, pair_ob, (const int*)P.obs_zpos);
}
void launch_lm_backsub(const DevProblem& P, const double* dp, double* out_all, hipStream_t st) {
  if (P.L == 0) return;
  with_uni(P, [&](auto U) { with_group(P.lm_group, [&](auto G) {
    hipLaunchKernelGGL((k_lm_backsub<decltype(G)::value, decltype(U)::value>), dim3(lm_blocks(P)), dim3(kBuildThreads), 0, st, P, dp, out_all); }); });
}
void launch_obs_jvp(const DevProblem& P, const double* v_all, hipStream_t st) {
  if (P.O == 0) return;
  with_uni(P, [&](auto U) { hipLaunchKernelGGL(k_obs_jvp<decltype(U)::value>, dim3(stream_grid(P.O)), dim3(256), 0, st, P, v_all); });
}
void launch_obs_cost(const DevProblem& P, const double* pose, const double* lm, hipStream_t st) {
  if (P.O == 0) return;
  with_uni(P, [&](auto U) { hipLaunchKernelGGL(k_obs_cost<decltype(U)::value>, dim3(stream_grid(P.O)), dim3(256), 0, st, P, pose, lm); });
}
void launch_obs_linearize(const DevProblem& P, double* r, double* Jp, double* Jl, double* cost, hipStream_t st) {
  if (P.O == 0) return;
  with_uni(P, [&](auto U) { hipLaunchKernelGGL(k_obs_linearize<decltype(U)::value>, dim3((P.O + 255) / 256), dim3(256), 0, st, P, r, Jp, Jl, cost); });
}
template <int G, bool UNI>
__global__ __launch_bounds__(kBuildThreads) void k_lm_outliers(DevProblem P, double th, unsigned char* __restrict__ erase, int* __restrict__ left,
                                                               unsigned long long* __restrict__ counts) {
  constexpr int GROUPS = kBuildThreads / G;
  const int lane = threadIdx.x % G, grp = threadIdx.x / G;
  const int l = blockIdx.x * GROUPS + grp;
  const bool lm_ok = l < P.L;
  const int o0 = lm_ok ? P.lm_obs_ptr[l] : 0;
  const int nobs = lm_ok ? P.lm_obs_ptr[l + 1] - o0 : 0;
  double kept = 0.0, bad = 0.0;
  for (int a = lane; a < nobs; a += G) {
    ObsLin e;
    eval_obs<false, UNI>(P, P.pose, P.lm, o0 + a, P.obs_kf[o0 + a], l, e);
    const bool out = sqrt(e.r0 * e.r0 + e.r1 * e.r1) > th;
    erase[o0 + a] = out ? 1 : 0;
    kept += out ? 0.0 : 1.0; bad += out ? 1.0 : 0.0;
  }
  kept = group_sum<G>(kept); bad = group_sum<G>(bad);
  if (lm_ok && lane == 0) {
    left[l] = (int)kept;
    if (bad > 0.0) atomicAdd(&counts[0], (unsigned long long)bad);
    if (kept < 2.0) atomicAdd(&counts[1], 1ull);
  }
}
void launch_lm_outliers(const DevProblem& P, double th, unsigned char* erase, int* left, unsigned long long* counts, hipStream_t st) {
  if (P.L == 0) return;
  with_uni(P, [&](auto U) { with_group(P.lm_group, [&](auto G) {
    hipLaunchKernelGGL((k_lm_outliers<decltype(G)::value, decltype(U)::value>), dim3(lm_blocks(P)), dim3(kBuildThreads), 0, st, P, th, erase, left, counts); }); });
}

void launch_obs_norms(const DevProblem& P, double* norms, hipStream_t st) {
  if (P.O == 0) return;
  with_uni(P, [&](auto U) { hipLaunchKernelGGL(k_obs_norms<decltype(U)::value>, dim3((P.O + 255) / 256), dim3(256), 0, st, P, norms); });
}

}
```

covins_amd/csrc/solver.hip:

```cpp
#include <dlfcn.h>

#include <algorithm>
#include <atomic>
#include <chrono>
#include <condition_variable>
#include <memory>
#include <mutex>
#include <cmath>
#include <cstdio>
#include <cstdlib>
#include <cstring>
#include <string>
#include <thread>
#include <vector>

#include "common.hpp"
#include "nd_plan.hpp"

using namespace covgpu;

static thread_local std::string g_err;
extern "C" const char* covgpu_last_error(void) { return g_err.c_str(); }

#define HIPCHK(expr)                                                                            \
// ... 596 lines not shown
    for (int v : h.own[n]) own_var[o++] = ir(v);
    for (int v : h.strct[n]) st_var[s++] = ir(v);
  }
  own_ptr[h.nnodes] = o; st_ptr[h.nnodes] = s;
}

extern "C" int32_t covgpu_shard_plan(const covgpu_options* opt, const covgpu_problem* p, int32_t world, covgpu_nd_plan** plan_out, int32_t* lm_rank,
                                     int32_t* imu_rank, int32_t* edge_rank) {
  *plan_out = nullptr;
  if (world < 1) return 0;
  int policy = opt->shard_policy;
  if (const char* e = getenv("COVGPU_SHARD_POLICY")) policy = atoi(e);
  if (policy != 0 && policy != 1) { g_err = "covgpu_shard_plan: shard_policy must be 0 or 1"; return 0; }
  covgpu_nd_plan* pl = nullptr;
  {
    const char* e_tree = getenv("COVGPU_SHARD_TREE");
    const char* e_cap = getenv("COVGPU_SHARD_CAP_MIB");
    std::vector<int> modes = e_tree ? std::vector<int>{atoi(e_tree) != 0 ? 1 : 0} : std::vector<int>{0, 1};
    std::vector<double> caps = e_cap ? std::vector<double>{atof(e_cap)} : std::vector<double>{48.0, 512.0};
    double best_cost = 0.0;
    for (int mode : modes) {
      covgpu_nd_plan* cand = nullptr;
      if (nd_plan_create_mode(opt, p, 0, &cand, mode) != COVGPU_OK) continue;
      for (double cap : caps) {
        NdHostPlan trial = cand->hp;
        if (policy == 1) nd_shard_assign_dist(trial, world, cap * 1048576.0);
        else nd_shard_assign(trial, world, cap * 1048576.0);
        if (trial.nsub == 0) continue;
        const double cost = nd_shard_cost(trial, world);
        if (pl == nullptr || cost < best_cost) {
          if (pl == nullptr) { pl = new covgpu_nd_plan(); pl->pos_kf = cand->pos_kf; }
          pl->hp = std::move(trial); best_cost = cost;
        }
      }
      delete cand;
    }
    if (pl == nullptr) return 0;
  }
  NdHostPlan& hp = pl->hp;
  const bool vi = !opt->visual_only;
  std::vector<int> perm(p->num_kf);
  for (int q = 0; q < p->num_kf; ++q) perm[pl->pos_kf[q]] = q;
  auto owner = [&](std::initializer_list<int> vars) {
    int best = -1, depth = -1;
    for (int v : vars) { const int n = hp.vnode[v]; if (n >= 0 && hp.depth[n] > depth) { depth = hp.depth[n]; best = n; } }
    return best < 0 ? -1 : hp.node_rank[best];
  };
  for (int l = 0; l < p->num_lm; ++l) {
    int best = -1, depth = -1;
    for (int o = p->lm_obs_ptr[l]; o < p->lm_obs_ptr[l + 1]; ++o) {
      const int kf = p->obs_kf[o];
      if (p->kf_fixed[kf]) continue;
      const int n = hp.vnode[2 * perm[kf]];
      if (hp.depth[n] > depth) { depth = hp.depth[n]; best = n; }
    }
    const int r = best < 0 ? -1 : hp.node_rank[best];
    lm_rank[l] = r >= 0 ? r : l % world;
  }
  for (int f = 0; f < p->num_imu; ++f) {
    const int a = perm[p->imu_kf_i[f]], b = perm[p->imu_kf_j[f]];
    const int r = vi ? owner({2 * a, 2 * a + 1, 2 * b, 2 * b + 1}) : -1;
    imu_rank[f] = r >= 0 ? r : f % world;
  }
  for (int e = 0; e < p->num_edge; ++e) {
    const int r = owner({2 * perm[p->edge_i[e]], 2 * perm[p->edge_j[e]]});
    edge_rank[e] = r >= 0 ? r : e % world;
  }
  *plan_out = pl;
  return hp.nsub;
}
extern "C" void covgpu_nd_plan_ranks(const covgpu_nd_plan* pl, int32_t* node_rank) {
  for (int n = 0; n < pl->hp.nnodes; ++n) node_rank[n] = pl->hp.node_rank.empty() ? 0 : pl->hp.node_rank[n];
}
extern "C" void covgpu_nd_plan_owner(const covgpu_nd_plan* pl, int32_t* pose_rank, int32_t* sb_rank) {
  const NdHostPlan& hp = pl->hp;
  for (int q = 0; q < hp.K; ++q) {
    const int kf = pl->pos_kf[q];
    const int np = hp.vnode[2 * q], ns = hp.vnode[2 * q + 1];
    pose_rank[kf] = (np >= 0 && !hp.node_rank.empty()) ? hp.node_rank[np] : -1;
    sb_rank[kf] = (ns >= 0 && !hp.node_rank.empty()) ? hp.node_rank[ns] : -1;
  }
}

static int upload_impl(covgpu_context* c, const covgpu_options* opt, const covgpu_problem* p, bool pgo, bool allow_arrow = true) {
  HIPCHK(hipSetDevice(c->device));
  static const bool tm_on = getenv("COVGPU_PLAN_TIMING") != nullptr;
  auto tm_last = std::chrono::steady_clock::now();
  auto tm = [&](const char* what) {
    if (!tm_on) return;
    const auto now = std::chrono::steady_clock::now();
    std::fprintf(stderr, "[covgpu] upload: %-28s %.2f ms\n", what, std::chrono::duration<double>(now - tm_last).count() * 1e3);
    tm_last = now;
  };
  const bool vi = !pgo && !opt->visual_only;
  RC(validate(p, pgo, vi));
  free_problem(c);
  c->chol.forms = FormCensus();
  DevProblem& P = c->P;
  std::memset(&P, 0, sizeof(P));
  P.K = p->num_kf; P.A = p->num_cam;
  P.L = pgo ? 0 : p->num_lm; P.O = pgo ? 0 : p->num_obs;
  P.I = vi ? p->num_imu : 0; P.E = p->num_edge;
  P.S = P.I ? p->imu_sample_ptr[P.I] : 0;
  P.vi = vi; P.D = vi ? 15 : 6; P.n = P.D * P.K;
  {
    const double mean_track = P.L > 0 ? (double)P.O / P.L : 0.0;
    P.lm_group = mean_track <= 5.0 ? 4 : (mean_track <= 8.0 ? 8 : 16);
  }
  P.npad = ((6 * P.K + kTile - 1) / kTile) * kTile;
  P.N = P.n + 3 * P.L;
  std::vector<int> perm, pos_kf, chain_ptr;
  const bool pgo_nd_on = env_int("COVGPU_PGO_ND", 1) != 0;
  const char* e_pgo_dense = getenv("COVGPU_PGO_DENSE");
  const bool pgo_nd = pgo && pgo_nd_on && allow_arrow && p->num_edge > 0 && !(e_pgo_dense && e_pgo_dense[0] == '1') && !c->sharded;
  if (pgo_nd) build_chains_pgo(p, perm, pos_kf, chain_ptr);
  else RC(build_chains(p, vi, perm, pos_kf, chain_ptr));
  std::vector<int> chain_end(P.K);
  P.nchains = (int)chain_ptr.size() - 1;
  P.max_chain_len = 1;
  for (int ci = 0; ci < P.nchains; ++ci) P.max_chain_len = std::max(P.max_chain_len, chain_ptr[ci + 1] - chain_ptr[ci]);
  for (int c = 0; c < P.nchains; ++c)
    for (int q = chain_ptr[c]; q < chain_ptr[c + 1]; ++q) chain_end[q] = chain_ptr[c + 1];
  P.reproj_loss_a = opt->reproj_loss_a; P.gravity = opt->gravity;
  const char* e_dense = getenv("COVGPU_GBA_DENSE");
  const bool use_nd = (!pgo && allow_arrow) || pgo_nd;
  if (c->sharded && !use_nd) { g_err = "the agent-sharded solve is for GBA problems (covgpu_upload)"; return COVGPU_ERR_INVALID_ARG; }
  const size_t K = P.K;
  RC(dev_upload(c, &P.pose0, p->kf_pose, 7 * K));
  if (p->kf_speed_bias) RC(dev_upload(c, &P.sb0, p->kf_speed_bias, 9 * K)); else { RC(dev_alloc(c, &P.sb0, 9 * K)); HIPCHK(hipMemsetAsync(P.sb0, 0, 9 * K * sizeof(double), c->st)); }
  RC(dev_upload(c, &P.lm0, p->lm_pos, (size_t)3 * P.L));
  RC(dev_alloc(c, &P.pose, 7 * K)); RC(dev_alloc(c, &P.sb, 9 * K)); RC(dev_alloc(c, &P.lm, (size_t)3 * P.L));
  RC(dev_alloc(c, &P.pose_c, 7 * K)); RC(dev_alloc(c, &P.sb_c, 9 * K)); RC(dev_alloc(c, &P.lm_c, (size_t)3 * P.L));
  RC(dev_upload(c, &P.fixed, (const uint8_t*)p->kf_fixed, K));
  RC(dev_upload(c, &P.kf_cam, (const int*)p->kf_cam, K));
  RC(dev_upload(c, &P.cam_extr, p->cam_extr, (size_t)7 * P.A));
  RC(dev_upload(c, &P.cam_intr, p->cam_intr, (size_t)4 * P.A));
  RC(dev_upload(c, &P.cam_dist, p->cam_dist, (size_t)4 * P.A));
  RC(dev_upload(c, &P.cam_dist_type, (const int*)p->cam_dist_type, (size_t)P.A));
  if (!pgo && p->cam_model) {
    std::vector<int> model(P.A);
    std::vector<double> xi(P.A, 0.0);
    for (int a = 0; a < P.A; ++a) {
      model[a] = p->cam_model[a];
      if (model[a] == COVGPU_CAM_UNIFIED) { xi[a] = p->cam_xi[a]; P.uni = 1; }
    }
    if (P.uni) {
      RC(dev_upload(c, &P.cam_model, (const int*)model.data(), (size_t)P.A));
      RC(dev_upload(c, &P.cam_xi, (const double*)xi.data(), (size_t)P.A));
      HIPCHK(hipStreamSynchronize(c->st));
    }
  }
  std::vector<int> ptr0(1, 0);
  RC(dev_upload(c, &P.lm_obs_ptr, P.L ? (const int*)p->lm_obs_ptr : ptr0.data(), (size_t)P.L + 1));
  RC(dev_upload(c, &P.obs_kf, (const int*)p->obs_kf, (size_t)P.O));
  RC(dev_upload(c, &P.obs_sigma, p->obs_sigma, (size_t)P.O));
  RC(dev_alloc(c, &P.obs_lm, (size_t)P.O)); RC(dev_alloc(c, &P.obs_u, (size_t)P.O)); RC(dev_alloc(c, &P.obs_v, (size_t)P.O));
  RC(dev_alloc(c, &P.kf_obs_ptr, (size_t)P.K + 1)); RC(dev_alloc(c, &P.kf_obs_idx, (size_t)P.O));
  {
    double* d_uv = nullptr; int* d_iota = nullptr;
    HIPCHK(hipMalloc((void**)&d_uv, std::max<size_t>((size_t)2 * P.O, 2) * sizeof(double)));
    if (hipMalloc((void**)&d_iota, std::max<size_t>((size_t)P.O, 1) * sizeof(int)) != hipSuccess) { (void)hipFree(d_uv); g_err = "hipMalloc: out of memory"; return COVGPU_ERR_OUT_OF_MEMORY; }
    hipError_t e = P.O ? hipMemcpyAsync(d_uv, p->obs_uv, (size_t)2 * P.O * sizeof(double), hipMemcpyHostToDevice, c->st) : hipSuccess;
    launch_obs_unpack(P.L, P.O, P.lm_obs_ptr, d_uv, P.obs_lm, P.obs_u, P.obs_v, d_iota, c->st);
    const bool ok = e == hipSuccess && build_kf_lists_device(P.O, P.K, P.obs_kf, d_iota, P.kf_obs_ptr, P.kf_obs_idx, c->st);
    (void)hipStreamSynchronize(c->st);
    (void)hipFree(d_uv); (void)hipFree(d_iota);
    if (!ok) { g_err = "upload: device-side observation lists failed (allocation)"; return COVGPU_ERR_OUT_OF_MEMORY; }
  }
  tm("validate, chains, states, observation stream");
  std::vector<int> h_pair_i, h_pair_j;
  {
    std::vector<int> key(P.K);
    for (int k = 0; k < P.K; ++k) key[k] = p->kf_fixed[k] ? -1 : perm[k];
    int* d_key = nullptr;
    RC(dev_upload(c, &d_key, key.data(), key.size()));
    c->d_pairkey = d_key; c->h_perm = perm;
    PairLists pl;
    if (!build_pairs_device(P.L, P.K, P.lm_obs_ptr, P.obs_kf, d_key, true, c->st, pl)) { g_err = "covisible pair lists: device allocation failed (or more than 2^31 entries)"; return COVGPU_ERR_OUT_OF_MEMORY; }
    for (int* q : {pl.pair_ptr, pl.pair_i, pl.pair_j, pl.pair_oa, pl.pair_ob}) if (q) c->allocs.push_back(q);
    c->alloc_bytes += ((size_t)pl.npairs * 3 + 1 + 2 * pl.nent) * sizeof(int);
    P.npairs = pl.npairs; P.pair_ptr = pl.pair_ptr; P.pair_i = pl.pair_i; P.pair_j = pl.pair_j; P.pair_oa = pl.pair_oa; P.pair_ob = pl.pair_ob;
    std::vector<int> pi(P.npairs), pj(P.npairs);
    if (P.npairs) {
      HIPCHK(hipMemcpyAsync(pi.data(), P.pair_i, (size_t)P.npairs * sizeof(int), hipMemcpyDeviceToHost, c->st));
      HIPCHK(hipMemcpyAsync(pj.data(), P.pair_j, (size_t)P.npairs * sizeof(int), hipMemcpyDeviceToHost, c->st));
    }
    RC(dev_alloc(c, &P.obsZ, (size_t)18 * P.O)); RC(dev_alloc(c, &P.lmRT, (size_t)9 * P.L));
    RC(dev_alloc(c, &P.kobs, (size_t)3 * P.O)); RC(dev_alloc(c, &P.kobs_lm, (size_t)P.O)); RC(dev_alloc(c, &P.obs_zpos, (size_t)P.O));
    launch_kobs_build(P, P.pair_oa, P.pair_ob, pl.nent, c->st);
    RC(dev_alloc(c, &P.cost_part, (size_t)(P.L / 4 + 64)));
    HIPCHK(hipStreamSynchronize(c->st));
    h_pair_i.swap(pi); h_pair_j.swap(pj);
  }
  tm("covisible pair lists");
  RC(dev_upload(c, &P.imu_i, (const int*)p->imu_kf_i, (size_t)P.I));
  RC(dev_upload(c, &P.imu_j, (const int*)p->imu_kf_j, (size_t)P.I));
  RC(dev_upload(c, &P.imu_ptr, P.I ? (const int*)p->imu_sample_ptr : ptr0.data(), (size_t)P.I + 1));
  RC(dev_upload(c, &P.imu_samples, p->imu_samples, (size_t)7 * P.S));
  RC(dev_upload(c, &P.imu_first, p->imu_first, (size_t)6 * P.I));
  {
    std::vector<double> nz((size_t)5 * P.I);
    for (int f = 0; f < P.I; ++f) {
      double* r = &nz[(size_t)5 * f];
      if (p->imu_noise) std::memcpy(r, p->imu_noise + (size_t)5 * f, 5 * sizeof(double));
      else { r[0] = opt->sigma_a; r[1] = opt->sigma_g; r[2] = opt->sigma_aw; r[3] = opt->sigma_gw; r[4] = opt->gravity; }
      if (!(r[0] > 0 && r[1] > 0 && r[2] > 0 && r[3] > 0) || !(r[4] >= 9.0)) {
        g_err = "invalid problem: IMU noise must be positive and gravity >= 9 (factor " + std::to_string(f) + ")";
        return COVGPU_ERR_INVALID_ARG;
      }
    }
    RC(dev_upload(c, &P.imu_noise, nz.data(), nz.size()));
    HIPCHK(hipStreamSynchronize(c->st));
  }
  RC(dev_alloc(c, &P.pre_delta, (size_t)11 * P.I)); RC(dev_alloc(c, &P.pre_J, (size_t)225 * P.I));
  RC(dev_alloc(c, &P.pre_P, (size_t)225 * P.I)); RC(dev_alloc(c, &P.pre_W, (size_t)225 * P.I));
  RC(dev_alloc(c, &P.pre_bias, (size_t)6 * P.I));
  RC(dev_upload(c, &P.edge_i, (const int*)p->edge_i, (size_t)P.E));
  RC(dev_upload(c, &P.edge_j, (const int*)p->edge_j, (size_t)P.E));
  RC(dev_upload(c, &P.edge_meas, p->edge_meas, (size_t)7 * P.E));
  RC(dev_upload(c, &P.edge_sqrt_info, p->edge_sqrt_info, (size_t)36 * P.E));
  RC(dev_upload(c, &P.edge_loss_a, p->edge_loss_a, (size_t)P.E));
  RC(dev_upload(c, &P.perm, perm.data(), K)); RC(dev_upload(c, &P.pos_kf, pos_kf.data(), K));
  RC(dev_upload(c, &P.chain_ptr, chain_ptr.data(), chain_ptr.size()));
  RC(dev_upload(c, &P.pos_chain_end, chain_end.data(), K));
  RC(dev_alloc(c, &P.bred, (size_t)P.n));
  RC(dev_alloc(c, &P.bp, (size_t)2 * P.npad));
  const size_t Kv = vi ? K : 0;
  RC(dev_alloc(c, &P.Ad, 81 * Kv)); RC(dev_alloc(c, &P.Ae, 81 * Kv));
  RC(dev_alloc(c, &P.Bp, 54 * Kv)); RC(dev_alloc(c, &P.Bs, 54 * Kv)); RC(dev_alloc(c, &P.Bn, 54 * Kv));
  {
    std::vector<int> cbeg(P.K);
    for (int ch = 0; ch < P.nchains; ++ch) for (int q = chain_ptr[ch]; q < chain_ptr[ch + 1]; ++q) cbeg[q] = chain_ptr[ch];
    RC(dev_upload(c, &P.pos_chain_begin, cbeg.data(), cbeg.size()));
    HIPCHK(hipStreamSynchronize(c->st));
  }
  RC(dev_alloc(c, &P.grad, (size_t)P.N)); RC(dev_alloc(c, &P.hdiag, (size_t)P.N));
  RC(dev_alloc(c, &P.HllInv, (size_t)6 * P.L));
  RC(dev_alloc(c, &P.gn, (size_t)P.N)); RC(dev_alloc(c, &P.step, (size_t)P.N)); RC(dev_alloc(c, &P.vtmp, (size_t)P.N));
  HIPCHK(hipMemsetAsync(P.gn, 0, (size_t)P.N * sizeof(double), c->st)); HIPCHK(hipMemsetAsync(P.step, 0, (size_t)P.N * sizeof(double), c->st));
  HIPCHK(hipMemsetAsync(P.vtmp, 0, (size_t)P.N * sizeof(double), c->st));
  RC(dev_alloc(c, &P.scal, (size_t)SC_COUNT)); RC(dev_alloc(c, &P.flag, (size_t)4));
  RC(dev_alloc(c, &P.tr, (size_t)TR_COUNT));
  P.scal_r = P.scal; P.flag_r = P.flag;
  P.part_imu = 8192; P.part_edge = P.part_imu + ((P.I + 3) / 4) * 4; P.part_vec = P.part_edge + (P.E + 63) / 64;
  P.part_n = P.part_vec + 8192;
  RC(dev_alloc(c, &P.part, (size_t)SC_COUNT * P.part_n));
  HIPCHK(hipMemsetAsync(P.part, 0, (size_t)SC_COUNT * P.part_n * sizeof(double), c->st));
  RC(dev_alloc(c, &P.imuAd, 2 * 81 * Kv)); RC(dev_alloc(c, &P.imuBs, 2 * 54 * Kv));
  RC(dev_alloc(c, &P.imuCd, 3 * 36 * Kv)); RC(dev_alloc(c, &P.imuG, 2 * 30 * Kv));
  RC(dev_alloc(c, &P.edgeOut, (size_t)132 * P.E));
  {
    std::vector<int> kptr(P.K + 1, 0), kent(2 * (size_t)P.E);
    for (int e = 0; e < P.E; ++e) {
      if (p->edge_i[e] == p->edge_j[e]) { g_err = "invalid problem: self edge"; return COVGPU_ERR_INVALID_ARG; }
      kptr[p->edge_i[e] + 1]++; kptr[p->edge_j[e] + 1]++;
    }
    for (int k = 0; k < P.K; ++k) kptr[k + 1] += kptr[k];
    { std::vector<int> cur(kptr.begin(), kptr.end() - 1);
      for (int e = 0; e < P.E; ++e) { kent[cur[p->edge_i[e]]++] = 2 * e; kent[cur[p->edge_j[e]]++] = 2 * e + 1; } }
    struct PE { int i, j, ent; };
    std::vector<PE> pe(P.E);
    for (int e = 0; e < P.E; ++e) {
      const int a = perm[p->edge_i[e]], b = perm[p->edge_j[e]];
      pe[e] = (a > b) ? PE{a, b, 2 * e} : PE{b, a, 2 * e + 1};
    }
    std::stable_sort(pe.begin(), pe.end(), [](const PE& x, const PE& y) { return x.i != y.i ? x.i < y.i : x.j < y.j; });
    std::vector<int> eptr, ei, ej, eent(P.E);
    for (int q = 0; q < P.E; ++q) {
      if (q == 0 || pe[q].i != pe[q - 1].i || pe[q].j != pe[q - 1].j) { eptr.push_back(q); ei.push_back(pe[q].i); ej.push_back(pe[q].j); }
      eent[q] = pe[q].ent;
    }
    eptr.push_back(P.E);
    P.nepairs = (int)ei.size();
    RC(dev_upload(c, &P.kf_edge_ptr, kptr.data(), kptr.size())); RC(dev_upload(c, &P.kf_edge_ent, kent.data(), kent.size()));
    RC(dev_upload(c, &P.epair_ptr, eptr.data(), eptr.size())); RC(dev_upload(c, &P.epair_i, ei.data(), ei.size()));
    RC(dev_upload(c, &P.epair_j, ej.data(), ej.size())); RC(dev_upload(c, &P.epair_ent, eent.data(), eent.size()));
    HIPCHK(hipStreamSynchronize(c->st));
    tm("IMU, edges, vectors");
    if (use_nd) {
      NdHostPlan nhp;
      if (c->sharded) {
        if ((int)c->shard_plan->K != P.K || (c->shard_plan->vi != 0) != vi) { g_err = "sharded solve: the problem does not match the shard plan"; return COVGPU_ERR_INVALID_ARG; }
        nhp = *c->shard_plan;
        std::vector<int> to_pos(2 * (size_t)P.K);
        for (int k = 0; k < P.K; ++k) { to_pos[2 * k] = 2 * perm[k]; to_pos[2 * k + 1] = 2 * perm[k] + 1; }
        nd_plan_remap(nhp, to_pos);
      } else {
        const bool one_front = e_dense && e_dense[0] == '1';
        const int leaf = one_front ? 0x3fffffff : nd_leaf_dims(0);
        std::vector<uint64_t> keys(h_pair_i.size() + ei.size());
        {
          std::vector<uint64_t> ka(h_pair_i.size()), kb(ei.size());
          for (size_t q = 0; q < ka.size(); ++q) ka[q] = ((uint64_t)(uint32_t)h_pair_i[q] << 32) | (uint32_t)h_pair_j[q];
          for (size_t q = 0; q < kb.size(); ++q) kb[q] = ((uint64_t)(uint32_t)ei[q] << 32) | (uint32_t)ej[q];
          if (!std::is_sorted(ka.begin(), ka.end())) std::sort(ka.begin(), ka.end());
          std::merge(ka.begin(), ka.end(), kb.begin(), kb.end(), keys.begin());
          keys.erase(std::unique(keys.begin(), keys.end()), keys.end());
        }
        PlanCache& pc = c->plan_cache;
// ... 95 lines not shown
      plan.nb = (((int)idxb.size() + kTile - 1) / kTile) * kTile;
      if (plan.nb == 0) plan.nb = kTile;
      idxb.resize(plan.nb, -1);
      RC(dev_upload(c, &plan.idx_b, idxb.data(), idxb.size()));
      RC(dev_alloc(c, &plan.Sb, (size_t)plan.nb * plan.nb)); RC(dev_alloc(c, &plan.rhs_b, (size_t)2 * plan.nb));
      RC(dev_alloc(c, &plan.Linv_b, (size_t)plan.nb * kTile));
      plan.nblk = (int)hp.block_kf.size();
      size_t big = 0;
      for (auto& bk : hp.block_kf) big = std::max(big, bk.size());
      plan.nIpad = (((int)big * 6 + 2 * kTile - 1) / (2 * kTile)) * (2 * kTile);
      plan.ntot = plan.nIpad + plan.nb;
      std::vector<int> idx((size_t)plan.nblk * plan.ntot, -1);
      for (int a = 0; a < plan.nblk; ++a) {
        int* row = idx.data() + (size_t)a * plan.ntot;
        int q = 0;
        for (int kf : hp.block_kf[a]) for (int r = 0; r < 6; ++r) row[q++] = 6 * kf + r;
        std::copy(idxb.begin(), idxb.end(), row + plan.nIpad);
      }
      RC(dev_upload(c, &plan.idx, idx.data(), idx.size()));
      RC(dev_alloc(c, &plan.M, (size_t)plan.nblk * plan.ntot * plan.ntot)); RC(dev_alloc(c, &plan.rhs, (size_t)plan.nblk * 2 * plan.ntot));
      RC(dev_alloc(c, &plan.Linv, (size_t)plan.nblk * plan.nIpad * kTile));
      plan.active = true;
    }
  }
  HIPCHK(hipMemsetAsync(P.scal, 0, SC_COUNT * sizeof(double), c->st));
  HIPCHK(hipMemsetAsync(P.flag, 0, 4 * sizeof(int), c->st));
  HIPCHK(hipStreamSynchronize(c->st));
  c->have = true; c->pgo = pgo;
  return COVGPU_OK;
}

static int reset_state(covgpu_context* c) {
  DevProblem& P = c->P;
  HIPCHK(hipMemcpyAsync(P.pose, P.pose0, (size_t)7 * P.K * sizeof(double), hipMemcpyDeviceToDevice, c->st));
  HIPCHK(hipMemcpyAsync(P.sb, P.sb0, (size_t)9 * P.K * sizeof(double), hipMemcpyDeviceToDevice, c->st));
  if (P.L) HIPCHK(hipMemcpyAsync(P.lm, P.lm0, (size_t)3 * P.L * sizeof(double), hipMemcpyDeviceToDevice, c->st));
  return COVGPU_OK;
}

static int read_scalars(covgpu_context* c) {
  HIPCHK(hipMemcpyAsync(c->h_scal, c->P.scal, SC_COUNT * sizeof(double), hipMemcpyDeviceToHost, c->st));
  HIPCHK(hipMemcpyAsync(c->h_scal + SC_COUNT, c->P.flag, sizeof(int), hipMemcpyDeviceToHost, c->st));
  HIPCHK(hipStreamSynchronize(c->st));
  HIPCHK(hipGetLastError());
  return COVGPU_OK;
}
static int chol_failed(covgpu_context* c) { int f; std::memcpy(&f, c->h_scal + SC_COUNT, sizeof(int)); return f; }

static void enqueue_build(covgpu_context* c, double mu) {
  const DevProblem& P = c->P;
  c->cur_damp = mu;
  if (c->profiling) (void)hipEventRecord(c->ev[0], c->st);
  c->chol.init();
  hipStream_t side = c->chol.mid;
  {
    DevSignal sig = P.L > 0 ? c->chol.publish_handle(c->chol.ev_zero, c->st, 1) : DevSignal();
    if (sig.flag == nullptr) c->chol.record(c->chol.ev_zero, c->st, 1);
    launch_lm_lin(P, mu, c->st, sig);
  }
  c->chol.wait(side, c->chol.ev_zero);
  launch_zero_system(P, side);
  const bool forked = P.L > 0 && P.npairs > 0;
  if (!forked) { c->chol.record(c->chol.ev_lin, side, 2); c->chol.wait(c->st, c->chol.ev_lin); }
  if (P.nd) { launch_nd_zero(P, c->nd, c->chol.head); (void)hipMemsetAsync(P.nd_rhs, 0, c->nd.rhs_elems * sizeof(double), c->chol.head); }
  else (void)hipMemsetAsync(P.Sred, 0, (size_t)P.npad * P.npad * sizeof(double), c->chol.head);
  c->chol.record(c->chol.ev_fill, c->chol.head, 3);
  launch_imu_build(P, side);
  if (P.vi) {
    launch_imu_gather(P, 1, side);
    launch_finalize_diag(P, mu, 1, side);
  }
  launch_edge_build(P, side);
  launch_lm_build(P, mu, c->st, c->chol.ev_fill, side, c->chol.ev_lin, c->chol.ev_kf, &c->chol);
  if (forked) launch_part_finish(P, SC_COST, 1, side);
  c->chol.record(c->chol.ev_kf, side, 4);
  c->chol.wait(c->st, c->chol.ev_kf);
  launch_imu_gather(P, 0, c->st);
  launch_edge_gather(P, c->st);
  launch_finalize_diag(P, mu, P.vi ? 0 : 2, c->st);
  if (!forked) launch_part_finish(P, SC_COST, 1, c->st);
  if (c->profiling) (void)hipEventRecord(c->ev[1], c->st);
}

static void enqueue_solve(covgpu_context* c, double* dst_all) {
  const DevProblem& P = c->P;
  if (c->profiling) (void)hipEventRecord(c->ev[2], c->st);
  FormScope census(&c->chol.forms);
  if (P.nd) {
    if (!launch_nd_solve(P, c->nd, dst_all, c->cur_damp, c->st, c->chol) && !c->coll_failed) { c->coll_failed = true; c->coll_err = "scratch allocation of the backward substitution failed"; }
  }
  else launch_pose_graph_solve(P, dst_all, c->st, c->chol, c->pgo_plan.active ? &c->pgo_plan : nullptr);
  if (c->profiling) (void)hipEventRecord(c->ev[3], c->st);
  launch_lm_backsub(P, dst_all, dst_all, c->st);
}

static void collect_profile(covgpu_context* c, bool built, bool solved) {
  if (solved && !c->profiling) c->chol.collect();
  if (!c->profiling) return;
  float ms = 0;
  if (built && hipEventElapsedTime(&ms, c->ev[0], c->ev[1]) == hipSuccess) { c->prof.t_build_ms += ms; c->prof.n_build++; }
  if (solved && hipEventElapsedTime(&ms, c->ev[2], c->ev[3]) == hipSuccess) { c->prof.t_factor_ms += ms; c->prof.n_factor++; }
  if (solved) c->chol.collect();
}

static void enqueue_jvp(covgpu_context* c, const double* v_all) {
  const DevProblem& P = c->P;
  launch_obs_jvp(P, v_all, c->st);
  launch_imu_jvp(P, v_all, c->st);
  launch_edge_jvp(P, v_all, c->st);
  launch_part_finish(P, SC_JV2, 1, c->st);
}

static void enqueue_cost_candidate(covgpu_context* c) {
  const DevProblem& P = c->P;
  launch_obs_cost(P, P.pose_c, P.lm_c, c->st);
  launch_imu_cost(P, P.pose_c, P.sb_c, c->st);
  launch_edge_cost(P, P.pose_c, c->st);
  launch_part_finish(P, SC_COST, 1, c->st);
}

__global__ void k_shard_scal_pack(DevProblem P, double* buf, int rank, int world) {
  const int t = threadIdx.x;
  if (t < SC_COUNT) buf[t] = (t == SC_GMAX) ? 0.0 : P.scal[t];
  if (t < world) { buf[SC_COUNT + t] = t == rank ? P.scal[SC_GMAX] : 0.0; buf[SC_COUNT + world + t] = t == rank ? (double)P.flag[0] : 0.0; }
}
__global__ void k_shard_scal_unpack(DevProblem P, const double* buf, int world) {
  const int t = threadIdx.x;
  if (t < SC_COUNT && t != SC_GMAX) P.scal_r[t] = buf[t];
  if (t == 0) {
    double gm = 0.0, fl = 0.0;
    for (int r = 0; r < world; ++r) { gm = fmax(gm, buf[SC_COUNT + r]); fl = fmax(fl, buf[SC_COUNT + world + r]); }
    P.scal_r[SC_GMAX] = gm; P.flag_r[0] = fl != 0.0 ? 1 : 0;
  }
}
static void reduce_scalars(covgpu_context* c) {
  if (!c->sharded || !c->reducer) return;
  hipLaunchKernelGGL(k_shard_scal_pack, dim3(1), dim3(64), 0, c->st, c->P, c->d_red, c->rank, c->world);
  if (c->reducer->allreduce(c->d_red, (size_t)SC_COUNT + 2 * (size_t)c->world, 0, c->st) != 0) coll_latch(c);
  hipLaunchKernelGGL(k_shard_scal_unpack, dim3(1), dim3(64), 0, c->st, c->P, (const double*)c->d_red, c->world);
}

static bool dist_sharded(const covgpu_context* c) { return c->sharded && c->shard_plan && c->shard_plan->shard_policy == 1; }
static int dist_fail(covgpu_context* c) {
  if (c->reducer) c->reducer->abort();
  if (c->peer_fail) c->peer_fail->store(1);
  const std::string why = c->coll_failed ? c->coll_err
                                         : std::string("a device-flag gate or a hand-over of the backward substitution timed out (the distributed top does not repeat a solve on one rank)");
  g_err = "sharded solve, rank " + std::to_string(c->rank) + ": " + why;
  return COVGPU_ERR_NO_DEVICE;
}

static int wait_iteration(covgpu_context* c) {
  if (c->sharded && c->reducer) {
    static const double limit = getenv("COVGPU_COLL_TIMEOUT_S") ? std::max(1.0, atof(getenv("COVGPU_COLL_TIMEOUT_S"))) : 300.0;
    RcclReducer* rr = dynamic_cast<RcclReducer*>(c->reducer);
    const auto t0 = std::chrono::steady_clock::now();
    long spins = 0;
    for (;;) {
      const hipError_t q = hipStreamQuery(c->st);
      if (q == hipSuccess) break;
      if (q != hipErrorNotReady) { g_err = std::string("hipStreamQuery: ") + hipGetErrorString(q); return COVGPU_ERR_NO_DEVICE; }
      ++spins;
      if (spins == 256 || (spins > 256 && (spins & 63) == 0)) {
        const char* why = nullptr;
        if (c->peer_fail && c->peer_fail->load(std::memory_order_relaxed)) why = "another rank of the call gave up";
        else if (rr && rr->async_error() != 0) why = "RCCL reported an asynchronous communicator error";
        else if (std::chrono::duration<double>(std::chrono::steady_clock::now() - t0).count() > limit) why = "collective timed out (COVGPU_COLL_TIMEOUT_S)";
        if (why) { if (!c->coll_failed) { c->coll_failed = true; c->coll_err = why; } c->reducer->abort(); break; }
      } else if (spins > 256) std::this_thread::sleep_for(std::chrono::microseconds(50));
    }
  }
  HIPCHK(hipStreamSynchronize(c->st));
  HIPCHK(hipGetLastError());
  if (dist_sharded(c) && (c->coll_failed || c->chol.gate_failed())) return dist_fail(c);
  if (c->chol.gate_failed()) {
    g_err = "solve: a device-flag gate between the context's streams timed out (COVGPU_GATE_TIMEOUT_S; COVGPU_GATES=0 selects HIP events)";
    return COVGPU_ERR_GATE_TIMEOUT;
  }
  if (c->coll_failed) {
    if (c->reducer) c->reducer->abort();
    if (c->peer_fail) c->peer_fail->store(1);
    g_err = (c->sharded ? "sharded solve, rank " + std::to_string(c->rank) + ": " : std::string("solve: ")) + c->coll_err;
    return COVGPU_ERR_NO_DEVICE;
  }
  return COVGPU_OK;
}

static int solve_impl_dev(covgpu_context* c, const covgpu_options* opt, covgpu_result* res) {
  if (!c->have) { g_err = "no problem uploaded"; return COVGPU_ERR_INVALID_ARG; }
  HIPCHK(hipSetDevice(c->device));
  DevProblem& P = c->P;
  const covgpu_options& o = *opt;
  P.reproj_loss_a = o.reproj_loss_a;
  std::memset(res, 0, sizeof(*res));
  c->coll_failed = false; c->coll_err.clear();
  const auto t_begin = std::chrono::steady_clock::now();
  c->chol.init();
  if (c->sharded) c->chol.gate_timeout_s = std::max(c->chol.gate_timeout_s, 120.0);
  RC(reset_state(c));
  HIPCHK(hipMemsetAsync(P.flag + 1, 0, sizeof(int), c->st));
  launch_preintegrate(P, c->st);
  double* h = c->h_tr;
  std::memset(h, 0, TR_COUNT * sizeof(double));
  h[TR_RADIUS] = o.initial_radius; h[TR_MU] = 1e-8; h[TR_LMDF] = 2.0; h[TR_FIRST] = 1.0; h[TR_OK] = 1.0;
  HIPCHK(hipMemcpyAsync(P.tr, h, TR_COUNT * sizeof(double), hipMemcpyHostToDevice, c->st));
  HIPCHK(hipStreamSynchronize(c->st));
  const TrConsts tc{o.strategy, o.max_radius, o.min_relative_decrease, o.function_tolerance, o.parameter_tolerance, o.gradient_tolerance};
  bool reuse = false, got_initial = false;
  int it = 0, accepted = 0, term = 0;
  static const bool fused_tail = env_int("COVGPU_TAIL", 1) != 0;
  const bool two = o.strategy == COVGPU_DOGLEG;
  const bool coll = c->sharded && c->reducer != nullptr;
  bool use_box = false;
  while (it < o.max_iterations) {
    use_box = false;
    if (fused_tail) {
      if (!reuse) {
        const double damp = (o.strategy == COVGPU_LM) ? 1.0 / h[TR_RADIUS] : h[TR_MU];
        enqueue_build(c, damp);
        enqueue_solve(c, P.gn);
        launch_tail_stats(P, c->st);
        launch_tail_jvp(P, two, c->st);
        launch_tail_finish(P, tc, 1, two, !coll, 1, c->st);
        if (coll) { reduce_scalars(c); launch_tail_logic(P, tc, 1, 1, c->st); }
      } else launch_tail_logic(P, tc, 1, 0, c->st);
      launch_tail_apply(P, c->st);
      launch_tail_cost(P, c->st);
      launch_tail_finish(P, tc, 2, two, !coll, 0, c->st);
      if (coll) { reduce_scalars(c); launch_tail_logic(P, tc, 2, 0, c->st); }
      static const bool dev_aids = getenv("COVGPU_TRACE_PANELS") != nullptr || getenv("COVGPU_GATE_LOG") != nullptr;
      use_box = c->d_box != nullptr && !coll && !c->profiling && !dev_aids;
      if (use_box) c->box_seq += 1.0;
      launch_tr_accept(P, c->st, use_box ? c->d_box : nullptr, c->box_seq);
    } else {
    if (!reuse) {
      const double damp = (o.strategy == COVGPU_LM) ? 1.0 / h[TR_RADIUS] : h[TR_MU];
      enqueue_build(c, damp);
      enqueue_solve(c, P.gn);
      if (o.strategy == COVGPU_DOGLEG) { launch_cauchy_vec(P, c->st); enqueue_jvp(c, P.vtmp); }
      launch_dogleg_stats(P, c->st);
      reduce_scalars(c);
    }
    launch_tr_after_solve(P, tc, reuse ? 0 : 1, c->st);
    launch_combine_step_dev(P, c->st);
    enqueue_jvp(c, P.step);
    launch_xnorm(P, c->st);
    reduce_scalars(c);
    launch_tr_after_model(P, tc, c->st);
    launch_apply_step(P, c->st);
    enqueue_cost_candidate(c);
    reduce_scalars(c);
    launch_tr_decide(P, tc, c->st);
    }
    if (use_box) {
      volatile double* box = c->h_box;
      bool got = false;
      for (unsigned spins = 1; !got; ++spins) {
        if (box[TR_COUNT] == c->box_seq) { got = true; break; }
        if ((spins & 4095u) == 0) { const hipError_t q = hipStreamQuery(c->st); if (q != hipErrorNotReady) break; }
      }
      std::atomic_thread_fence(std::memory_order_acquire);
      if (got) {
        for (int i = 0; i < TR_COUNT; ++i) h[i] = box[i];
        HIPCHK(hipGetLastError());
        if (dist_sharded(c) && (c->coll_failed || c->chol.gate_failed())) { HIPCHK(hipStreamSynchronize(c->st)); return dist_fail(c); }
        if (c->chol.gate_failed()) { HIPCHK(hipStreamSynchronize(c->st)); g_err = "solve: a device-flag gate between the context's streams timed out"; return COVGPU_ERR_GATE_TIMEOUT; }
      } else {
        HIPCHK(hipMemcpyAsync(h, P.tr, TR_COUNT * sizeof(double), hipMemcpyDeviceToHost, c->st));
        RC(wait_iteration(c));
      }
    } else {
      HIPCHK(hipMemcpyAsync(h, P.tr, TR_COUNT * sizeof(double), hipMemcpyDeviceToHost, c->st));
      RC(wait_iteration(c));
    }
    collect_profile(c, !reuse, !reuse);
    if (!got_initial) { res->initial_cost = h[TR_INITCOST]; got_initial = true; }
    if (h[TR_RETRY] != 0.0) { reuse = false; continue; }
    term = (int)h[TR_TERM];
    if (term == 3 || term == 2) break;
    const int acc = h[TR_ACC] != 0.0;
    accepted += acc;
    if (it < COVGPU_MAX_TRACE) { res->cost_trace[it] = h[TR_COST]; res->radius_trace[it] = h[TR_RADIUS]; res->accepted_trace[it] = acc; }
    if (o.verbose) std::printf("[covgpu] it %2d cost %.9e rho %.3f radius %.3e %s\n", it, h[TR_COST], h[TR_RHO], h[TR_RADIUS], acc ? "ok" : "rej");
    reuse = h[TR_REUSE] != 0.0;
    ++it;
    if (term == 1 || term == 4) break;
  }
  {
    int dropped = 0;
    HIPCHK(hipMemcpy(&dropped, P.flag + 1, sizeof(int), hipMemcpyDeviceToHost));
    res->reserved = dropped;
  }
  res->iterations = it; res->accepted = accepted; res->termination = term;
  res->final_cost = h[TR_COST];
  res->t_solve_s = std::chrono::duration<double>(std::chrono::steady_clock::now() - t_begin).count();
  res->t_linear_solve_s = 0.0;
  return COVGPU_OK;
}

static int download_impl(covgpu_context* c, covgpu_problem* p) {
  if (!c->have) { g_err = "no problem uploaded"; return COVGPU_ERR_INVALID_ARG; }
  const DevProblem& P = c->P;
  HIPCHK(hipMemcpyAsync(p->kf_pose, P.pose, (size_t)7 * P.K * sizeof(double), hipMemcpyDeviceToHost, c->st));
  if (P.vi && p->kf_speed_bias) HIPCHK(hipMemcpyAsync(p->kf_speed_bias, P.sb, (size_t)9 * P.K * sizeof(double), hipMemcpyDeviceToHost, c->st));
  if (P.L) HIPCHK(hipMemcpyAsync(p->lm_pos, P.lm, (size_t)3 * P.L * sizeof(double), hipMemcpyDeviceToHost, c->st));
// ... 4 lines not shown
extern "C" int covgpu_upload(covgpu_context* c, const covgpu_options* opt, const covgpu_problem* p) { return guarded([&] { return upload_impl(c, opt, p, false); }); }
extern "C" int covgpu_upload_pgo(covgpu_context* c, const covgpu_options* opt, const covgpu_problem* p) { return guarded([&] { return upload_impl(c, opt, p, true); }); }
static int solve_impl_dev(covgpu_context* c, const covgpu_options* opt, covgpu_result* res);
static int solve_any(covgpu_context* c, const covgpu_options* opt, covgpu_result* out) {
  int rc = solve_impl_dev(c, opt, out);
  if (rc == COVGPU_ERR_GATE_TIMEOUT) {
    if (c->chol.gate_dead_h[1] == -2)
      std::fprintf(stderr, "[covgpu] warning: a hand-over inside the pipelined backward substitution timed out (workgroup %d of front %d of its level); repeating the solve with a launch per tile and HIP events (this context keeps them)\n",
                   c->chol.gate_dead_h[2], c->chol.gate_dead_h[3]);
    else
    std::fprintf(stderr, "[covgpu] warning: device-flag stream ordering timed out (slot %d awaited %d, found %d; %ld signals, %ld gates so far); repeating the solve with HIP events (this context keeps them)\n",
                 c->chol.gate_dead_h[1], c->chol.gate_dead_h[2], c->chol.gate_dead_h[3], c->chol.gate_signals, c->chol.gate_waits);
    if (c->chol.gate_dead_h[1] >= 0 && c->chol.gate_dead_h[1] < (int)c->chol.gate_tag_of_slot.size()) std::fprintf(stderr, "[covgpu]          (tag of that slot: %d)\n", c->chol.gate_tag_of_slot[c->chol.gate_dead_h[1]]);
    (void)hipDeviceSynchronize();
    c->chol.gates_disable();
    rc = solve_impl_dev(c, opt, out);
    if (rc == COVGPU_ERR_GATE_TIMEOUT) { g_err = "solve: stream ordering failed"; rc = COVGPU_ERR_NO_DEVICE; }
  }
  return rc;
}
extern "C" int covgpu_solve_resident(covgpu_context* c, const covgpu_options* opt, covgpu_result* out) { return guarded([&] { return solve_any(c, opt, out); }); }
extern "C" int covgpu_download(covgpu_context* c, covgpu_problem* p) { return guarded([&] { return download_impl(c, p); }); }

static int full_solve(covgpu_context* c, const covgpu_options* opt, covgpu_problem* p, covgpu_result* out, bool pgo) {
  covgpu_result local;
  auto t0 = std::chrono::steady_clock::now();
  RC(upload_impl(c, opt, p, pgo));
  const double t_up = std::chrono::duration<double>(std::chrono::steady_clock::now() - t0).count();
  RC(solve_any(c, opt, &local));
  t0 = std::chrono::steady_clock::now();
  RC(download_impl(c, p));
  local.t_download_s = std::chrono::duration<double>(std::chrono::steady_clock::now() - t0).count();
  local.t_upload_s = t_up;
  if (out) *out = local;
  return COVGPU_OK;
}
extern "C" int covgpu_gba_solve(covgpu_context* c, const covgpu_options* opt, covgpu_problem* p, covgpu_result* out) { return guarded([&] { return full_solve(c, opt, p, out, false); }); }
extern "C" int covgpu_pgo_solve(covgpu_context* c, const covgpu_options* opt, covgpu_problem* p, covgpu_result* out) { return guarded([&] { return full_solve(c, opt, p, out, true); }); }

static int gba_two_round_impl(covgpu_context* c, const covgpu_options* opt, covgpu_problem* p, const covgpu_two_round* tr, uint8_t* obs_erase,
                              int32_t* lm_left, int64_t* counts, covgpu_result* round1, covgpu_result* round2);
extern "C" int covgpu_gba_two_round(covgpu_context* c, const covgpu_options* opt, covgpu_problem* p, const covgpu_two_round* tr, uint8_t* obs_erase,
                                    int32_t* lm_left, int64_t* counts, covgpu_result* round1, covgpu_result* round2) {
  const int rc = gba_two_round_impl(c, opt, p, tr, obs_erase, lm_left, counts, round1, round2);
  if (c) { c->have = false; }
  return rc;
}
static int gba_two_round_impl(covgpu_context* c, const covgpu_options* opt, covgpu_problem* p, const covgpu_two_round* tr, uint8_t* obs_erase,
                              int32_t* lm_left, int64_t* counts, covgpu_result* round1, covgpu_result* round2) {
  return guarded([&]() -> int {
    if (!tr || !obs_erase || !lm_left) { g_err = "covgpu_gba_two_round: NULL argument"; return (int)COVGPU_ERR_INVALID_ARG; }
    covgpu_options o1 = *opt;
    o1.max_iterations = tr->round1_iterations > 0 ? tr->round1_iterations : 5;
    auto t0 = std::chrono::steady_clock::now();
    RC(upload_impl(c, &o1, p, false));
    covgpu_result a, b;
    const double t_up = std::chrono::duration<double>(std::chrono::steady_clock::now() - t0).count();
    RC(solve_any(c, &o1, &a));
    a.t_upload_s = t_up;
    DevProblem& P = c->P;
    t0 = std::chrono::steady_clock::now();
    unsigned char* de = nullptr; int* dl = nullptr; unsigned long long* dc = nullptr;
    RC(dev_alloc(c, &de, (size_t)std::max(P.O, 1))); RC(dev_alloc(c, &dl, (size_t)std::max(P.L, 1))); RC(dev_alloc(c, &dc, (size_t)2));
    HIPCHK(hipMemsetAsync(dc, 0, 2 * sizeof(unsigned long long), c->st));
    launch_lm_outliers(P, tr->outlier_threshold, de, dl, dc, c->st);
    unsigned long long hc[2] = {0, 0};
    if (P.O) HIPCHK(hipMemcpyAsync(obs_erase, de, (size_t)P.O, hipMemcpyDeviceToHost, c->st));
    if (P.L) HIPCHK(hipMemcpyAsync(lm_left, dl, sizeof(int) * (size_t)P.L, hipMemcpyDeviceToHost, c->st));
    HIPCHK(hipMemcpyAsync(hc, dc, sizeof(hc), hipMemcpyDeviceToHost, c->st));
    Round2Lists R;
    if (!round2_compact_device(P.L, P.O, P.K, de, dl, P.obs_kf, P.obs_lm, P.obs_u, P.obs_v, P.obs_sigma, P.lm0, c->st, R)) {
      g_err = "covgpu_gba_two_round: device allocation failed while compacting the observation stream"; return (int)COVGPU_ERR_OUT_OF_MEMORY;
    }
    for (void* q : {(void*)R.lm0, (void*)R.obs_u, (void*)R.obs_v, (void*)R.obs_sigma, (void*)R.lm_obs_ptr, (void*)R.lm_old, (void*)R.obs_kf, (void*)R.obs_lm, (void*)R.kf_obs_ptr,
                    (void*)R.kf_obs_idx})
      if (q) c->allocs.push_back(q);
    if (counts) { counts[0] = (int64_t)hc[0]; counts[1] = (int64_t)hc[1]; }
    const int L1 = P.L;
    if (R.L2 > 0 && R.O2 > 0) {
      P.L = R.L2; P.O = R.O2; P.N = P.n + 3 * P.L;
      P.lm0 = R.lm0; P.lm_obs_ptr = R.lm_obs_ptr; P.obs_kf = R.obs_kf; P.obs_lm = R.obs_lm; P.obs_u = R.obs_u; P.obs_v = R.obs_v; P.obs_sigma = R.obs_sigma;
      P.kf_obs_ptr = R.kf_obs_ptr; P.kf_obs_idx = R.kf_obs_idx;
    } else { P.L = 0; P.O = 0; P.N = P.n; }
    if (tr->kf_fixed_round2 != nullptr) {
      HIPCHK(hipMemcpyAsync(P.fixed, tr->kf_fixed_round2, (size_t)P.K, hipMemcpyHostToDevice, c->st));
      std::vector<int> key(P.K);
      for (int k = 0; k < P.K; ++k) key[k] = tr->kf_fixed_round2[k] ? -1 : c->h_perm[k];
      HIPCHK(hipMemcpyAsync(c->d_pairkey, key.data(), sizeof(int) * (size_t)P.K, hipMemcpyHostToDevice, c->st));
      HIPCHK(hipStreamSynchronize(c->st));
    }
    {
      PairLists pl;
      if (!build_pairs_device(P.L, P.K, P.lm_obs_ptr, P.obs_kf, c->d_pairkey, true, c->st, pl)) { g_err = "covisible pair lists: device allocation failed"; return (int)COVGPU_ERR_OUT_OF_MEMORY; }
      for (int* q : {pl.pair_ptr, pl.pair_i, pl.pair_j, pl.pair_oa, pl.pair_ob}) if (q) c->allocs.push_back(q);
      P.npairs = pl.npairs; P.pair_ptr = pl.pair_ptr; P.pair_i = pl.pair_i; P.pair_j = pl.pair_j; P.pair_oa = pl.pair_oa; P.pair_ob = pl.pair_ob;
      launch_kobs_build(P, P.pair_oa, P.pair_ob, pl.nent, c->st);
    }
    HIPCHK(hipMemsetAsync(P.part, 0, (size_t)SC_COUNT * P.part_n * sizeof(double), c->st));
    if (!tr->use_loops_round2) { P.E = 0; P.nepairs = 0; }
    else if (P.E > 0) {
      std::vector<double> la((size_t)P.E, tr->loop_loss_round2);
      HIPCHK(hipMemcpyAsync(P.edge_loss_a, la.data(), sizeof(double) * (size_t)P.E, hipMemcpyHostToDevice, c->st));
    }
    HIPCHK(hipStreamSynchronize(c->st));
    const double t_prep = std::chrono::duration<double>(std::chrono::steady_clock::now() - t0).count();
    RC(solve_any(c, opt, &b));
    b.t_upload_s = t_prep;
    t0 = std::chrono::steady_clock::now();
    HIPCHK(hipMemcpyAsync(p->kf_pose, P.pose, (size_t)7 * P.K * sizeof(double), hipMemcpyDeviceToHost, c->st));
    if (P.vi && p->kf_speed_bias) HIPCHK(hipMemcpyAsync(p->kf_speed_bias, P.sb, (size_t)9 * P.K * sizeof(double), hipMemcpyDeviceToHost, c->st));
    std::vector<double> lm2((size_t)3 * P.L);
    std::vector<int> old((size_t)P.L);
    if (P.L) {
      HIPCHK(hipMemcpyAsync(lm2.data(), P.lm, lm2.size() * sizeof(double), hipMemcpyDeviceToHost, c->st));
      HIPCHK(hipMemcpyAsync(old.data(), R.lm_old, old.size() * sizeof(int), hipMemcpyDeviceToHost, c->st));
    }
    HIPCHK(hipStreamSynchronize(c->st));
    for (int q = 0; q < P.L; ++q) {
      if (old[q] < 0 || old[q] >= L1) { g_err = "covgpu_gba_two_round: landmark map out of range"; return (int)COVGPU_ERR_INVALID_ARG; }
      std::memcpy(p->lm_pos + 3 * (size_t)old[q], lm2.data() + 3 * (size_t)q, 3 * sizeof(double));
    }
    b.t_download_s = std::chrono::duration<double>(std::chrono::steady_clock::now() - t0).count();
    if (round1) *round1 = a;
    if (round2) *round2 = b;
    return (int)COVGPU_OK;
  });
}

namespace {
struct SubProblem {
  std::vector<double> lm_pos, obs_uv, obs_sigma, imu_samples, imu_first, imu_noise, edge_meas, edge_info, edge_loss, pose, sb;
  std::vector<int32_t> lm_obs_ptr, obs_kf, imu_i, imu_j, imu_ptr, edge_i, edge_j, lm_id, obs_id;
  covgpu_problem view;
};
void make_sub(const covgpu_problem& p, int r, const int32_t* lm_rank, const int32_t* imu_rank, const int32_t* edge_rank, SubProblem& s) {
  s.pose.assign(p.kf_pose, p.kf_pose + 7 * (size_t)p.num_kf);
  if (p.kf_speed_bias) s.sb.assign(p.kf_speed_bias, p.kf_speed_bias + 9 * (size_t)p.num_kf);
  s.lm_obs_ptr.assign(1, 0);
  for (int l = 0; l < p.num_lm; ++l) {
    if (lm_rank[l] != r) continue;
    s.lm_id.push_back(l);
    s.lm_pos.insert(s.lm_pos.end(), p.lm_pos + 3 * (size_t)l, p.lm_pos + 3 * (size_t)l + 3);
    for (int o = p.lm_obs_ptr[l]; o < p.lm_obs_ptr[l + 1]; ++o) {
      s.obs_id.push_back(o); s.obs_kf.push_back(p.obs_kf[o]);
      s.obs_uv.push_back(p.obs_uv[2 * (size_t)o]); s.obs_uv.push_back(p.obs_uv[2 * (size_t)o + 1]); s.obs_sigma.push_back(p.obs_sigma[o]);
    }
    s.lm_obs_ptr.push_back((int32_t)s.obs_kf.size());
  }
  s.imu_ptr.assign(1, 0);
  for (int f = 0; f < p.num_imu; ++f) {
    if (imu_rank[f] != r) continue;
    s.imu_i.push_back(p.imu_kf_i[f]); s.imu_j.push_back(p.imu_kf_j[f]);
    s.imu_samples.insert(s.imu_samples.end(), p.imu_samples + 7 * (size_t)p.imu_sample_ptr[f], p.imu_samples + 7 * (size_t)p.imu_sample_ptr[f + 1]);
    s.imu_ptr.push_back((int32_t)(s.imu_samples.size() / 7));
    s.imu_first.insert(s.imu_first.end(), p.imu_first + 6 * (size_t)f, p.imu_first + 6 * (size_t)f + 6);
    if (p.imu_noise) s.imu_noise.insert(s.imu_noise.end(), p.imu_noise + 5 * (size_t)f, p.imu_noise + 5 * (size_t)f + 5);
  }
  for (int e = 0; e < p.num_edge; ++e) {
    if (edge_rank[e] != r) continue;
    s.edge_i.push_back(p.edge_i[e]); s.edge_j.push_back(p.edge_j[e]);
    s.edge_meas.insert(s.edge_meas.end(), p.edge_meas + 7 * (size_t)e, p.edge_meas + 7 * (size_t)e + 7);
    s.edge_info.insert(s.edge_info.end(), p.edge_sqrt_info + 36 * (size_t)e, p.edge_sqrt_info + 36 * (size_t)e + 36);
    s.edge_loss.push_back(p.edge_loss_a[e]);
  }
  covgpu_problem& v = s.view;
  v = p;
// ... 601 lines not shown
```

Baseline: 290.5.

## Bin landmarks by track length and fuse back-substitution with JVP tail

Replaces the single global landmark group width with a per-landmark work list, radix-sorted into six segments by observation count so each segment uses a matching lane width. Landmark back-substitution is fused with the Jacobian-vector products for observations, IMU and edges. Per-observation JVP terms go to a buffer that the stats kernel reduces, and IMU Jacobians are cached during the build, so the separate tail JVP kernel that re-evaluated every residual is removed. The price is extra device memory for the cached IMU Jacobians and per-observation values, a sort plus host sync at setup, and more kernel specializations.

```diff
diff --git a/covins_amd/csrc/common.hpp b/covins_amd/csrc/common.hpp
--- a/covins_amd/csrc/common.hpp
+++ b/covins_amd/csrc/common.hpp
@@ -14,6 +14,9 @@
 namespace covgpu {
 
 constexpr int kTile = 128;
+constexpr int kLmSegs = 6;
+constexpr int kLmSegLanes[kLmSegs] = {64, 64, 32, 16, 8, 4};
+constexpr int kLmThreads = 256;
 
 struct DevProblem {
   int K, A, L, O, I, E, S;
@@ -22,8 +25,10 @@
   int npad;
   int N;
   int vi;
-  int lm_group;
   double reproj_loss_a, gravity;
+
+  int* lm_work;
+  int lm_seg_lm[kLmSegs + 1], lm_seg_blk[kLmSegs + 1];
 
   double *pose, *sb, *lm;
   double *pose_c, *sb_c, *lm_c;
@@ -45,6 +50,7 @@
   double *obsZ;
   double *lmRT;
   double *cost_part;
+  double *obs_jv;
 
   int *imu_i, *imu_j, *imu_ptr;
   double *imu_samples, *imu_first;
@@ -54,6 +60,7 @@
   double *pre_P;
   double *pre_W;
   double *pre_bias;
+  double *imuJ;
 
   int *edge_i, *edge_j;
   double *edge_meas, *edge_sqrt_info, *edge_loss_a;
@@ -164,6 +171,7 @@
 void launch_lm_build(const DevProblem& P, double mu, hipStream_t st, hipEvent_t pose_system_cleared = nullptr, hipStream_t side = nullptr,
                      hipEvent_t ev_lin = nullptr, hipEvent_t ev_kf = nullptr, CholAux* ax = nullptr);
 void launch_lm_backsub(const DevProblem& P, const double* dp, double* out_all, hipStream_t st);
+void launch_lm_backsub_jvp(const DevProblem& P, bool two, hipStream_t st);
 void launch_obs_jvp(const DevProblem& P, const double* v_all, hipStream_t st);
 void launch_obs_cost(const DevProblem& P, const double* pose, const double* lm, hipStream_t st);
 void launch_obs_linearize(const DevProblem& P, double* r, double* Jp, double* Jl, double* cost, hipStream_t st);
@@ -357,6 +365,7 @@
   int *pair_oa = nullptr, *pair_ob = nullptr;
 };
 bool build_pairs_device(int L, int K, const int* d_lm_obs_ptr, const int* d_obs_kf, const int* d_key_of_kf, bool want_obs, hipStream_t st, PairLists& out);
+bool build_lm_work_device(int L, const int* d_lm_obs_ptr, int* d_lm_work, int counts[kLmSegs], hipStream_t st);
 void launch_obs_unpack(int L, int O, const int* lm_obs_ptr, const double* uv, int* obs_lm, double* u, double* v, int* iota, hipStream_t st);
 bool build_kf_lists_device(int O, int K, const int* d_obs_kf, const int* d_iota, int* kf_obs_ptr, int* kf_obs_idx, hipStream_t st);
 struct Round2Lists {
@@ -426,8 +435,7 @@
 void launch_nd_zero(const DevProblem& P, const NdDev& nd, hipStream_t st);
 bool launch_nd_solve(const DevProblem& P, NdDev& nd, double* dst, double mu, hipStream_t st, CholAux& ax);
 
-void launch_tail_stats(const DevProblem& P, hipStream_t st);
-void launch_tail_jvp(const DevProblem& P, bool two, hipStream_t st);
+void launch_tail_stats(const DevProblem& P, bool two, hipStream_t st);
 void launch_tail_cost(const DevProblem& P, hipStream_t st);
 void launch_tail_finish(const DevProblem& P, TrConsts tc, int stage, bool two, bool with_logic, int fresh, hipStream_t st);
 void launch_tail_logic(const DevProblem& P, TrConsts tc, int stage, int fresh, hipStream_t st);
diff --git a/covins_amd/csrc/k_inertial.hip b/covins_amd/csrc/k_inertial.hip
--- a/covins_amd/csrc/k_inertial.hip
+++ b/covins_amd/csrc/k_inertial.hip
@@ -178,6 +178,7 @@
   const double* Jw = sl + 450;
   const double* r = sl + 1141;
   const int i = P.imu_i[f], j = P.imu_j[f];
+  for (int e = lane; e < 450; e += 64) P.imuJ[450 * (size_t)f + e] = Jw[e];
   const int pi = P.perm[i], pj = P.perm[j];
   const size_t K = (size_t)P.K;
   if (lane < 30) {
diff --git a/covins_amd/csrc/k_pairs.hip b/covins_amd/csrc/k_pairs.hip
--- a/covins_amd/csrc/k_pairs.hip
+++ b/covins_amd/csrc/k_pairs.hip
@@ -196,6 +196,34 @@
   if (n > 0) hipLaunchKernelGGL(k_obs_unpack, dim3((n + 255) / 256), dim3(256), 0, st, L, O, lm_obs_ptr, uv, obs_lm, u, v, iota);
 }
 
+__global__ __launch_bounds__(256) void k_lmw_keys(int L, const int* __restrict__ lm_obs_ptr, unsigned* __restrict__ key, int* __restrict__ iota, int* __restrict__ counts) {
+  const int l = blockIdx.x * 256 + threadIdx.x;
+  if (l >= L) return;
+  const int n = lm_obs_ptr[l + 1] - lm_obs_ptr[l];
+  static_assert(kLmSegs == 6 && kLmSegLanes[1] == 64 && kLmSegLanes[2] == 32 && kLmSegLanes[3] == 16 && kLmSegLanes[4] == 8 && kLmSegLanes[5] == 4, "segment bounds");
+  const int s = n > 64 ? 0 : (n > 32 ? 1 : (n > 16 ? 2 : (n > 8 ? 3 : (n > 4 ? 4 : 5))));
+  key[l] = (unsigned)s; iota[l] = l;
+  atomicAdd(&counts[s], 1);
+}
+bool build_lm_work_device(int L, const int* d_lm_obs_ptr, int* d_lm_work, int counts[kLmSegs], hipStream_t st) {
+  for (int s = 0; s < kLmSegs; ++s) counts[s] = 0;
+  if (L <= 0) return true;
+  unsigned *key = nullptr, *key2 = nullptr; int *iota = nullptr, *cnt = nullptr; void* tmp = nullptr;
+  size_t b = 0;
+  bool ok = hipMalloc((void**)&key, (size_t)L * 4) == hipSuccess && hipMalloc((void**)&key2, (size_t)L * 4) == hipSuccess &&
+            hipMalloc((void**)&iota, (size_t)L * 4) == hipSuccess && hipMalloc((void**)&cnt, kLmSegs * 4) == hipSuccess;
+  ok = ok && hipMemsetAsync(cnt, 0, kLmSegs * 4, st) == hipSuccess;
+  if (ok) {
+    hipLaunchKernelGGL(k_lmw_keys, dim3((L + 255) / 256), dim3(256), 0, st, L, d_lm_obs_ptr, key, iota, cnt);
+    ok = rocprim::radix_sort_pairs(nullptr, b, key, key2, iota, d_lm_work, (size_t)L, 0u, 3u, st) == hipSuccess &&
+         hipMalloc(&tmp, std::max<size_t>(b, 16)) == hipSuccess &&
+         rocprim::radix_sort_pairs(tmp, b, key, key2, iota, d_lm_work, (size_t)L, 0u, 3u, st) == hipSuccess &&
+         hipMemcpyAsync(counts, cnt, kLmSegs * 4, hipMemcpyDeviceToHost, st) == hipSuccess && hipStreamSynchronize(st) == hipSuccess;
+  }
+  for (void* q : {(void*)key, (void*)key2, (void*)iota, (void*)cnt, tmp}) if (q) (void)hipFree(q);
+  return ok;
+}
+
 #define PB_HIP(expr) do { if ((expr) != hipSuccess) { ok = false; goto done; } } while (0)
 
 bool build_pairs_device(int L, int K, const int* d_lm_obs_ptr, const int* d_obs_kf, const int* d_key_of_kf, bool want_obs, hipStream_t st, PairLists& out) {
diff --git a/covins_amd/csrc/k_tail.hip b/covins_amd/csrc/k_tail.hip
--- a/covins_amd/csrc/k_tail.hip
+++ b/covins_amd/csrc/k_tail.hip
@@ -17,9 +17,21 @@
   part_put(P, slot, index, v);
 }
 
-__global__ __launch_bounds__(256) void k_tail_stats(DevProblem P) {
+__global__ __launch_bounds__(256) void k_tail_stats(DevProblem P, int nb_stat, int two) {
+  if ((int)blockIdx.x >= nb_stat) {
+    const int b = blockIdx.x - nb_stat, nb_obs = gridDim.x - nb_stat;
+    double ja = 0.0, jb = 0.0, jc = 0.0;
+    for (int o = b * blockDim.x + threadIdx.x; o < P.O; o += nb_obs * blockDim.x) {
+      jb += P.obs_jv[o];
+      if (two) { ja += P.obs_jv[(size_t)P.O + o]; jc += P.obs_jv[2 * (size_t)P.O + o]; }
+    }
+    const int idx = b * 4 + (threadIdx.x >> 6);
+    tail_put(P, jb, SC_JB, idx);
+    if (two) { tail_put(P, ja, SC_JA, idx); tail_put(P, jc, SC_JC, idx); }
+    return;
+  }
   double gg = 0, gn2 = 0, gd = 0, gm = 0, vv = 0, vg = 0, nn = 0, xn = 0;
-  const int stride = gridDim.x * blockDim.x, t0 = blockIdx.x * blockDim.x + threadIdx.x;
+  const int stride = nb_stat * blockDim.x, t0 = blockIdx.x * blockDim.x + threadIdx.x;
   for (int q = t0; q < P.N; q += stride) {
     const double g = P.grad[q], d = clamp_diag(P.hdiag[q]), s = P.gn[q];
     const double w = P.vw ? P.vw[q] : 1.0;
@@ -42,84 +54,8 @@
   if ((threadIdx.x & 63) == 0) atomicMax(reinterpret_cast<unsigned long long*>(&P.scal[SC_GMAX]), (unsigned long long)__double_as_longlong(gm));
 }
 
-static_assert(kImuWaves == 4, "k_tail_jvp / k_tail_cost index their IMU and edge segments as 4 waves / 256 threads per workgroup");
-template <bool TWO, bool UNI>
-__global__ __launch_bounds__(64 * kImuWaves) void k_tail_jvp(DevProblem P, const double* __restrict__ va, const double* __restrict__ vb, int nb_obs, int nb_imu) {
-  __shared__ double sm[kImuWaves][kImuLds];
-  const int lane = threadIdx.x & 63, wave = threadIdx.x >> 6;
-  double ja = 0.0, jb = 0.0, jc = 0.0;
-  int idx;
-  if ((int)blockIdx.x < nb_obs) {
-    for (int o = blockIdx.x * blockDim.x + threadIdx.x; o < P.O; o += nb_obs * blockDim.x) {
-      ObsLin e;
-      const int kf = P.obs_kf[o], l = P.obs_lm[o];
-      eval_obs<true, UNI>(P, P.pose, P.lm, o, kf, l, e);
-      {
-        const double* vp = vb + (size_t)P.D * kf;
-        const double* vl = vb + P.n + 3 * (size_t)l;
-        double s0 = e.jl[0] * vl[0] + e.jl[1] * vl[1] + e.jl[2] * vl[2];
-        double s1 = e.jl[3] * vl[0] + e.jl[4] * vl[1] + e.jl[5] * vl[2];
-#pragma unroll
-        for (int k = 0; k < 6; ++k) { s0 += e.jp[k] * vp[k]; s1 += e.jp[6 + k] * vp[k]; }
-        jb += s0 * s0 + s1 * s1;
-        if (TWO) {
-          const double* up = va + (size_t)P.D * kf;
-          const double* ul = va + P.n + 3 * (size_t)l;
-          double t0 = e.jl[0] * ul[0] + e.jl[1] * ul[1] + e.jl[2] * ul[2];
-          double t1 = e.jl[3] * ul[0] + e.jl[4] * ul[1] + e.jl[5] * ul[2];
-#pragma unroll
-          for (int k = 0; k < 6; ++k) { t0 += e.jp[k] * up[k]; t1 += e.jp[6 + k] * up[k]; }
-          ja += t0 * t0 + t1 * t1; jc += t0 * s0 + t1 * s1;
-        }
-      }
-    }
-    idx = blockIdx.x * 4 + wave;
-  } else if ((int)blockIdx.x < nb_obs + nb_imu) {
-    const int bi = blockIdx.x - nb_obs;
-    const int f = bi * kImuWaves + wave;
-    const bool live = f < P.I;
-    double* sl = sm[wave];
-    imu_stage<true>(P, P.pose, P.sb, f, live, lane, sl);
-    if (live && lane < 15) {
-      const double* Jw = sl + 450;
-      const size_t oi = 15 * (size_t)P.imu_i[f], oj = 15 * (size_t)P.imu_j[f];
-      double s2 = 0.0, t2 = 0.0;
-      for (int c = 0; c < 15; ++c) {
-        s2 += Jw[30 * lane + c] * vb[oi + c] + Jw[30 * lane + 15 + c] * vb[oj + c];
-        if (TWO) t2 += Jw[30 * lane + c] * va[oi + c] + Jw[30 * lane + 15 + c] * va[oj + c];
-      }
-      jb = s2 * s2; ja = t2 * t2; jc = s2 * t2;
-    }
-    idx = P.part_imu + bi * kImuWaves + wave;
-  } else {
-    const int be = blockIdx.x - nb_obs - nb_imu;
-    const int e = be * 256 + threadIdx.x;
-    if (e < P.E) {
-      double r[6], J[72];
-      eval_edge<true>(P, P.pose, e, r, J);
-      const size_t oi = (size_t)P.D * P.edge_i[e], oj = (size_t)P.D * P.edge_j[e];
-#pragma unroll
-      for (int a = 0; a < 6; ++a) {
-        double s = 0.0, t = 0.0;
-#pragma unroll
-        for (int c = 0; c < 6; ++c) {
-          s += J[12 * a + c] * vb[oi + c] + J[12 * a + 6 + c] * vb[oj + c];
-          if (TWO) t += J[12 * a + c] * va[oi + c] + J[12 * a + 6 + c] * va[oj + c];
-        }
-        jb += s * s; ja += t * t; jc += s * t;
-      }
-    }
-    idx = P.part_edge + be * 4 + wave;
-    if (be * 4 + wave >= (P.E + 63) / 64) idx = -1;
-  }
-  jb = wave_sum(jb);
-  if (TWO) { ja = wave_sum(ja); jc = wave_sum(jc); }
-  if (idx >= 0) {
-    part_put(P, SC_JB, idx, jb);
-    if (TWO) { part_put(P, SC_JA, idx, ja); part_put(P, SC_JC, idx, jc); }
-  }
-}
-
+
+static_assert(kImuWaves == 4, "k_tail_cost (and k_lm_backsub_jvp, k_visual.hip) index its IMU and edge segments as 4 waves / 256 threads per workgroup");
 template <bool UNI>
 __global__ __launch_bounds__(64 * kImuWaves) void k_tail_cost(DevProblem P, int nb_obs, int nb_imu) {
   __shared__ double sm[kImuWaves][kImuLds];
@@ -294,20 +230,9 @@
   nb_imu = (P.vi && P.I > 0) ? (P.I + kImuWaves - 1) / kImuWaves : 0;
   nb_edge = P.E > 0 ? (P.E + 255) / 256 : 0;
 }
-void launch_tail_stats(const DevProblem& P, hipStream_t st) {
-  hipLaunchKernelGGL(k_tail_stats, dim3(tail_grid(P.N, 256)), dim3(256), 0, st, P);
-}
-void launch_tail_jvp(const DevProblem& P, bool two, hipStream_t st) {
-  int a, b, c;
-  tail_segments(P, a, b, c);
-  if (a + b + c == 0) return;
-  if (P.uni) {
-    if (two) hipLaunchKernelGGL((k_tail_jvp<true, true>), dim3(a + b + c), dim3(64 * kImuWaves), 0, st, P, (const double*)P.vtmp, (const double*)P.gn, a, b);
-    else hipLaunchKernelGGL((k_tail_jvp<false, true>), dim3(a + b + c), dim3(64 * kImuWaves), 0, st, P, (const double*)nullptr, (const double*)P.gn, a, b);
-    return;
-  }
-  if (two) hipLaunchKernelGGL((k_tail_jvp<true, false>), dim3(a + b + c), dim3(64 * kImuWaves), 0, st, P, (const double*)P.vtmp, (const double*)P.gn, a, b);
-  else hipLaunchKernelGGL((k_tail_jvp<false, false>), dim3(a + b + c), dim3(64 * kImuWaves), 0, st, P, (const double*)nullptr, (const double*)P.gn, a, b);
+void launch_tail_stats(const DevProblem& P, bool two, hipStream_t st) {
+  const int nb_stat = tail_grid(P.N, 256), nb_obs = P.O > 0 ? tail_grid(P.O, 2048) : 0;
+  hipLaunchKernelGGL(k_tail_stats, dim3(nb_stat + nb_obs), dim3(256), 0, st, P, nb_stat, two ? 1 : 0);
 }
 void launch_tail_cost(const DevProblem& P, hipStream_t st) {
   int a, b, c;
diff --git a/covins_amd/csrc/k_visual.hip b/covins_amd/csrc/k_visual.hip
--- a/covins_amd/csrc/k_visual.hip
+++ b/covins_amd/csrc/k_visual.hip
@@ -2,6 +2,7 @@
 
 #include "common.hpp"
 #include "dev_math.hpp"
+#include "between_dev.hpp"
 #include "reduce.hpp"
 #include "visual_dev.hpp"
 
@@ -28,7 +29,7 @@
   o[3] = (h[0] * h[5] - h[2] * h[2]) * id; o[4] = (h[1] * h[2] - h[0] * h[4]) * id; o[5] = (h[0] * h[3] - h[1] * h[1]) * id;
 }
 
-constexpr int kBuildThreads = 256;
+constexpr int kBuildThreads = kLmThreads;
 
 constexpr int kRec = 39;
 
@@ -50,13 +51,39 @@
   }
 }
 
-template <int G, bool UNI>
-__global__ __launch_bounds__(kBuildThreads) void k_lm_lin(DevProblem P, double mu, DevSignal sig) {
-  constexpr int GROUPS = kBuildThreads / G;
-  if (sig.flag != nullptr && blockIdx.x == 0 && threadIdx.x == 0) __hip_atomic_store(sig.flag, sig.seq, __ATOMIC_RELAXED, __HIP_MEMORY_SCOPE_AGENT);
-  const int lane = threadIdx.x % G, grp = threadIdx.x / G;
-  const int l = blockIdx.x * GROUPS + grp;
-  const bool lm_ok = l < P.L;
+COV_DEV int lm_seg_of(const DevProblem& P, int wb) {
+  int s = 0;
+#pragma unroll
+  for (int k = 1; k < kLmSegs; ++k) s += wb >= P.lm_seg_blk[k] ? 1 : 0;
+  return s;
+}
+template <int S>
+COV_DEV bool lm_pick(const DevProblem& P, int wb, int& l) {
+  constexpr int G = kLmSegLanes[S];
+  const int slot = P.lm_seg_lm[S] + (wb - P.lm_seg_blk[S]) * (kBuildThreads / G) + (int)threadIdx.x / G;
+  const bool ok = slot < P.lm_seg_lm[S + 1];
+  l = ok ? P.lm_work[slot] : 0;
+  return ok;
+}
+template <typename F>
+COV_DEV void lm_dispatch(const DevProblem& P, int wb, F&& f) {
+  switch (lm_seg_of(P, wb)) {
+    case 0: f(std::integral_constant<int, 0>()); break;
+    case 1: f(std::integral_constant<int, 1>()); break;
+    case 2: f(std::integral_constant<int, 2>()); break;
+    case 3: f(std::integral_constant<int, 3>()); break;
+    case 4: f(std::integral_constant<int, 4>()); break;
+    default: f(std::integral_constant<int, 5>()); break;
+  }
+}
+
+template <int S, bool UNI>
+COV_DEV void lm_lin_body(const DevProblem& P, double mu, int wb, double* scost) {
+  constexpr int G = kLmSegLanes[S];
+  constexpr bool MULTI = S == 0;
+  const int lane = threadIdx.x % G;
+  int l;
+  const bool lm_ok = lm_pick<S>(P, wb, l);
   const int o0 = lm_ok ? P.lm_obs_ptr[l] : 0;
   const int nobs = lm_ok ? P.lm_obs_ptr[l + 1] - o0 : 0;
   const int nchunk = (nobs + G - 1) / G;
@@ -110,20 +137,19 @@
     rt[8] = R[5] * gl[2];
   }
   cost = wave_sum(cost);
-  __shared__ double scost[kBuildThreads / 64];
   if ((threadIdx.x & 63) == 0) scost[threadIdx.x >> 6] = cost;
   __syncthreads();
   if (threadIdx.x == 0) {
     double c4 = 0.0;
 #pragma unroll
     for (int k = 0; k < kBuildThreads / 64; ++k) c4 += scost[k];
-    P.cost_part[blockIdx.x] = c4;
+    P.cost_part[wb] = c4;
   }
 
   for (int c = 0; c < nchunk; ++c) {
     const int a = c * G + lane;
     if (a >= nobs) continue;
-    if (nchunk > 1) {
+    if (MULTI && nchunk > 1) {
       kf = P.obs_kf[o0 + a];
       eval_obs<true, UNI>(P, P.pose, P.lm, o0 + a, kf, l, e);
     }
@@ -133,6 +159,12 @@
 #pragma unroll
     for (int k = 0; k < 9; ++k) zo[k] = double2{Z[2 * k], Z[2 * k + 1]};
   }
+}
+template <bool UNI>
+__global__ __launch_bounds__(kBuildThreads) void k_lm_lin(DevProblem P, double mu, DevSignal sig) {
+  if (sig.flag != nullptr && blockIdx.x == 0 && threadIdx.x == 0) __hip_atomic_store(sig.flag, sig.seq, __ATOMIC_RELAXED, __HIP_MEMORY_SCOPE_AGENT);
+  __shared__ double scost[kBuildThreads / 64];
+  lm_dispatch(P, blockIdx.x, [&](auto S) { lm_lin_body<decltype(S)::value, UNI>(P, mu, blockIdx.x, scost); });
 }
 
 __global__ __launch_bounds__(256) void k_cost_finish(DevProblem P, int nparts) {
@@ -260,12 +292,27 @@
   }
 }
 
-template <int G, bool UNI>
-__global__ __launch_bounds__(kBuildThreads) void k_lm_backsub(DevProblem P, const double* __restrict__ dp, double* __restrict__ out_all) {
-  constexpr int GROUPS = kBuildThreads / G;
-  const int lane = threadIdx.x % G, grp = threadIdx.x / G;
-  const int l = blockIdx.x * GROUPS + grp;
-  const bool lm_ok = l < P.L;
+COV_DEV void backsub_add(const ObsLin& e, const double* __restrict__ d, double* t) {
+  const double s0 = e.jp[0] * d[0] + e.jp[1] * d[1] + e.jp[2] * d[2] + e.jp[3] * d[3] + e.jp[4] * d[4] + e.jp[5] * d[5];
+  const double s1 = e.jp[6] * d[0] + e.jp[7] * d[1] + e.jp[8] * d[2] + e.jp[9] * d[3] + e.jp[10] * d[4] + e.jp[11] * d[5];
+  t[0] += e.jl[0] * s0 + e.jl[3] * s1;
+  t[1] += e.jl[1] * s0 + e.jl[4] * s1;
+  t[2] += e.jl[2] * s0 + e.jl[5] * s1;
+}
+COV_DEV void backsub_solve(const DevProblem& P, int l, const double* t, double* dl) {
+  const double* gl = P.grad + P.n + 3 * (size_t)l;
+  const double* hi = P.HllInv + 6 * (size_t)l;
+  const double x = -gl[0] - t[0], y = -gl[1] - t[1], z = -gl[2] - t[2];
+  dl[0] = hi[0] * x + hi[1] * y + hi[2] * z;
+  dl[1] = hi[1] * x + hi[3] * y + hi[4] * z;
+  dl[2] = hi[2] * x + hi[4] * y + hi[5] * z;
+}
+template <int S, bool UNI>
+COV_DEV void lm_backsub_body(const DevProblem& P, const double* __restrict__ dp, double* __restrict__ out_all, int wb) {
+  constexpr int G = kLmSegLanes[S];
+  const int lane = threadIdx.x % G;
+  int l;
+  const bool lm_ok = lm_pick<S>(P, wb, l);
   const int o0 = lm_ok ? P.lm_obs_ptr[l] : 0;
   const int nobs = lm_ok ? P.lm_obs_ptr[l + 1] - o0 : 0;
   double t[3] = {0, 0, 0};
@@ -273,23 +320,144 @@
     ObsLin e;
     const int kf = P.obs_kf[o0 + a];
     eval_obs<true, UNI>(P, P.pose, P.lm, o0 + a, kf, l, e);
-    const double* d = dp + (size_t)P.D * kf;
-    const double s0 = e.jp[0] * d[0] + e.jp[1] * d[1] + e.jp[2] * d[2] + e.jp[3] * d[3] + e.jp[4] * d[4] + e.jp[5] * d[5];
-    const double s1 = e.jp[6] * d[0] + e.jp[7] * d[1] + e.jp[8] * d[2] + e.jp[9] * d[3] + e.jp[10] * d[4] + e.jp[11] * d[5];
-    t[0] += e.jl[0] * s0 + e.jl[3] * s1;
-    t[1] += e.jl[1] * s0 + e.jl[4] * s1;
-    t[2] += e.jl[2] * s0 + e.jl[5] * s1;
+    backsub_add(e, dp + (size_t)P.D * kf, t);
   }
 #pragma unroll
   for (int k = 0; k < 3; ++k) t[k] = group_sum<G>(t[k]);
   if (lm_ok && lane == 0) {
-    const double* gl = P.grad + P.n + 3 * (size_t)l;
-    const double* hi = P.HllInv + 6 * (size_t)l;
-    const double x = -gl[0] - t[0], y = -gl[1] - t[1], z = -gl[2] - t[2];
+    double dl[3];
+    backsub_solve(P, l, t, dl);
     double* o = out_all + P.n + 3 * (size_t)l;
-    o[0] = hi[0] * x + hi[1] * y + hi[2] * z;
-    o[1] = hi[1] * x + hi[3] * y + hi[4] * z;
-    o[2] = hi[2] * x + hi[4] * y + hi[5] * z;
+    o[0] = dl[0]; o[1] = dl[1]; o[2] = dl[2];
+  }
+}
+template <bool UNI>
+__global__ __launch_bounds__(kBuildThreads) void k_lm_backsub(DevProblem P, const double* __restrict__ dp, double* __restrict__ out_all) {
+  lm_dispatch(P, blockIdx.x, [&](auto S) { lm_backsub_body<decltype(S)::value, UNI>(P, dp, out_all, blockIdx.x); });
+}
+
+COV_DEV double cauchy_at(const DevProblem& P, size_t q) {
+  const double d = clamp_diag(P.hdiag[q]);
+  return P.grad[q] / (d * d);
+}
+COV_DEV void jvp_rows(const ObsLin& e, const double* __restrict__ vp, const double* vl, double& s0, double& s1) {
+  s0 = e.jl[0] * vl[0] + e.jl[1] * vl[1] + e.jl[2] * vl[2];
+  s1 = e.jl[3] * vl[0] + e.jl[4] * vl[1] + e.jl[5] * vl[2];
+#pragma unroll
+  for (int k = 0; k < 6; ++k) { s0 += e.jp[k] * vp[k]; s1 += e.jp[6 + k] * vp[k]; }
+}
+template <bool TWO>
+COV_DEV void jvp_put(const DevProblem& P, const ObsLin& e, int o, int kf, const double* dl, const double* cl) {
+  double s0, s1;
+  jvp_rows(e, P.gn + (size_t)P.D * kf, dl, s0, s1);
+  P.obs_jv[o] = s0 * s0 + s1 * s1;
+  if (TWO) {
+    double cp[6];
+#pragma unroll
+    for (int k = 0; k < 6; ++k) cp[k] = cauchy_at(P, (size_t)P.D * kf + k);
+    double t0, t1;
+    jvp_rows(e, cp, cl, t0, t1);
+    P.obs_jv[(size_t)P.O + o] = t0 * t0 + t1 * t1; P.obs_jv[2 * (size_t)P.O + o] = t0 * s0 + t1 * s1;
+  }
+}
+template <int S, bool TWO, bool UNI>
+COV_DEV void lm_backsub_jvp_body(const DevProblem& P, int wb) {
+  constexpr int G = kLmSegLanes[S];
+  constexpr bool MULTI = S == 0;
+  const int lane = threadIdx.x % G;
+  int l;
+  const bool lm_ok = lm_pick<S>(P, wb, l);
+  const int o0 = lm_ok ? P.lm_obs_ptr[l] : 0;
+  const int nobs = lm_ok ? P.lm_obs_ptr[l + 1] - o0 : 0;
+  double t[3] = {0, 0, 0};
+  ObsLin e;
+  int kf = 0;
+  for (int a = lane; a < nobs; a += G) {
+    kf = P.obs_kf[o0 + a];
+    eval_obs<true, UNI>(P, P.pose, P.lm, o0 + a, kf, l, e);
+    backsub_add(e, P.gn + (size_t)P.D * kf, t);
+  }
+#pragma unroll
+  for (int k = 0; k < 3; ++k) t[k] = group_sum<G>(t[k]);
+  if (!lm_ok) return;
+  double dl[3], cl[3] = {0, 0, 0};
+  backsub_solve(P, l, t, dl);
+  if (lane == 0) {
+    double* o = P.gn + P.n + 3 * (size_t)l;
+    o[0] = dl[0]; o[1] = dl[1]; o[2] = dl[2];
+  }
+  if (TWO) {
+#pragma unroll
+    for (int k = 0; k < 3; ++k) cl[k] = cauchy_at(P, (size_t)P.n + 3 * (size_t)l + k);
+  }
+  if (MULTI && nobs > G) {
+    for (int a = lane; a < nobs; a += G) {
+      kf = P.obs_kf[o0 + a];
+      eval_obs<true, UNI>(P, P.pose, P.lm, o0 + a, kf, l, e);
+      jvp_put<TWO>(P, e, o0 + a, kf, dl, cl);
+    }
+  } else if (lane < nobs) jvp_put<TWO>(P, e, o0 + lane, kf, dl, cl);
+}
+constexpr int kLmJvpGrid = 2048;
+constexpr int kJvpWaves = kBuildThreads / 64;
+static_assert(kJvpWaves == 4 && kBuildThreads == 256, "k_lm_backsub_jvp indexes the IMU and edge ranges of the partial sums as 4 waves / 256 threads per workgroup (kImuWaves, k_tail_cost)");
+template <bool TWO, bool UNI>
+__global__ __launch_bounds__(kBuildThreads) void k_lm_backsub_jvp(DevProblem P, int nb_lm, int nb_imu) {
+  const int lane = threadIdx.x & 63, wave = threadIdx.x >> 6;
+  double ja = 0.0, jb = 0.0, jc = 0.0;
+  int idx;
+  if ((int)blockIdx.x < nb_lm) {
+    for (int wb = blockIdx.x; wb < P.lm_seg_blk[kLmSegs]; wb += nb_lm)
+      lm_dispatch(P, wb, [&](auto S) { lm_backsub_jvp_body<decltype(S)::value, TWO, UNI>(P, wb); });
+    idx = -1;
+  } else if ((int)blockIdx.x < nb_lm + nb_imu) {
+    const int bi = blockIdx.x - nb_lm;
+    const int f = bi * kJvpWaves + wave;
+    if (f < P.I) {
+      const double* Jw = P.imuJ + 450 * (size_t)f;
+      const size_t q = lane < 15 ? 15 * (size_t)P.imu_i[f] + lane : 15 * (size_t)P.imu_j[f] + (lane < 30 ? lane - 15 : 0);
+      const double nv = P.gn[q], cv = TWO ? cauchy_at(P, q) : 0.0;
+      const int row = lane < 15 ? lane : 14;
+      double s2 = 0.0, t2 = 0.0;
+      for (int c = 0; c < 15; ++c) {
+        const double ji = Jw[30 * row + c], jj = Jw[30 * row + 15 + c];
+        s2 += ji * __shfl(nv, c, 64) + jj * __shfl(nv, 15 + c, 64);
+        if (TWO) t2 += ji * __shfl(cv, c, 64) + jj * __shfl(cv, 15 + c, 64);
+      }
+      if (lane < 15) { jb = s2 * s2; ja = t2 * t2; jc = s2 * t2; }
+    }
+    idx = P.part_imu + bi * kJvpWaves + wave;
+  } else {
+    const int be = blockIdx.x - nb_lm - nb_imu;
+    const int e = be * kBuildThreads + threadIdx.x;
+    if (e < P.E) {
+      double r[6], J[72];
+      eval_edge<true>(P, P.pose, e, r, J);
+      const size_t oi = (size_t)P.D * P.edge_i[e], oj = (size_t)P.D * P.edge_j[e];
+      double ci[6] = {0, 0, 0, 0, 0, 0}, cj[6] = {0, 0, 0, 0, 0, 0};
+      if (TWO) {
+#pragma unroll
+        for (int c = 0; c < 6; ++c) { ci[c] = cauchy_at(P, oi + c); cj[c] = cauchy_at(P, oj + c); }
+      }
+#pragma unroll
+      for (int a = 0; a < 6; ++a) {
+        double s = 0.0, t = 0.0;
+#pragma unroll
+        for (int c = 0; c < 6; ++c) {
+          s += J[12 * a + c] * P.gn[oi + c] + J[12 * a + 6 + c] * P.gn[oj + c];
+          if (TWO) t += J[12 * a + c] * ci[c] + J[12 * a + 6 + c] * cj[c];
+        }
+        jb += s * s; ja += t * t; jc += s * t;
+      }
+    }
+    idx = P.part_edge + be * kJvpWaves + wave;
+    if (be * kJvpWaves + wave >= (P.E + 63) / 64) idx = -1;
+  }
+  jb = wave_sum(jb);
+  if (TWO) { ja = wave_sum(ja); jc = wave_sum(jc); }
+  if (idx >= 0) {
+    part_put(P, SC_JB, idx, jb);
+    if (TWO) { part_put(P, SC_JA, idx, ja); part_put(P, SC_JC, idx, jc); }
   }
 }
 
@@ -349,19 +517,15 @@
   return b < 1 ? 1 : (b > 2048 ? 2048 : b);
 }
 
-template <typename F> static void with_group(int g, F&& f) {
-  if (g == 4) f(std::integral_constant<int, 4>()); else if (g == 8) f(std::integral_constant<int, 8>()); else f(std::integral_constant<int, 16>());
-}
 template <typename F> static void with_uni(const DevProblem& P, F&& f) {
   if (P.uni) f(std::true_type()); else f(std::false_type());
 }
-static int lm_blocks(const DevProblem& P) { const int g = P.lm_group == 4 || P.lm_group == 8 ? P.lm_group : 16; const int groups = kBuildThreads / g; return (P.L + groups - 1) / groups; }
+static int lm_blocks(const DevProblem& P) { return P.lm_seg_blk[kLmSegs]; }
 
 void launch_lm_lin(const DevProblem& P, double mu, hipStream_t st, DevSignal sig) {
   if (P.L == 0) return;
   const int nblk = lm_blocks(P);
-  with_uni(P, [&](auto U) { with_group(P.lm_group, [&](auto G) {
-    hipLaunchKernelGGL((k_lm_lin<decltype(G)::value, decltype(U)::value>), dim3(nblk), dim3(kBuildThreads), 0, st, P, mu, sig); }); });
+  with_uni(P, [&](auto U) { hipLaunchKernelGGL(k_lm_lin<decltype(U)::value>, dim3(nblk), dim3(kBuildThreads), 0, st, P, mu, sig); });
 }
 void launch_lm_build(const DevProblem& P, double mu, hipStream_t st, hipEvent_t pose_system_cleared, hipStream_t side, hipEvent_t ev_lin, hipEvent_t ev_kf, CholAux* ax) {
   auto record = [&](hipEvent_t e, hipStream_t s) { if (ax) ax->record(e, s); else (void)hipEventRecord(e, s); };
@@ -399,8 +563,16 @@
 }
 void launch_lm_backsub(const DevProblem& P, const double* dp, double* out_all, hipStream_t st) {
   if (P.L == 0) return;
-  with_uni(P, [&](auto U) { with_group(P.lm_group, [&](auto G) {
-    hipLaunchKernelGGL((k_lm_backsub<decltype(G)::value, decltype(U)::value>), dim3(lm_blocks(P)), dim3(kBuildThreads), 0, st, P, dp, out_all); }); });
+  with_uni(P, [&](auto U) { hipLaunchKernelGGL(k_lm_backsub<decltype(U)::value>, dim3(lm_blocks(P)), dim3(kBuildThreads), 0, st, P, dp, out_all); });
+}
+void launch_lm_backsub_jvp(const DevProblem& P, bool two, hipStream_t st) {
+  const int nb_lm = P.L > 0 ? (lm_blocks(P) < kLmJvpGrid ? lm_blocks(P) : kLmJvpGrid) : 0;
+  const int nb_imu = (P.vi && P.I > 0) ? (P.I + kJvpWaves - 1) / kJvpWaves : 0, nb_edge = P.E > 0 ? (P.E + kBuildThreads - 1) / kBuildThreads : 0;
+  if (nb_lm + nb_imu + nb_edge == 0) return;
+  with_uni(P, [&](auto U) {
+    if (two) hipLaunchKernelGGL((k_lm_backsub_jvp<true, decltype(U)::value>), dim3(nb_lm + nb_imu + nb_edge), dim3(kBuildThreads), 0, st, P, nb_lm, nb_imu);
+    else hipLaunchKernelGGL((k_lm_backsub_jvp<false, decltype(U)::value>), dim3(nb_lm + nb_imu + nb_edge), dim3(kBuildThreads), 0, st, P, nb_lm, nb_imu);
+  });
 }
 void launch_obs_jvp(const DevProblem& P, const double* v_all, hipStream_t st) {
   if (P.O == 0) return;
@@ -414,13 +586,12 @@
   if (P.O == 0) return;
   with_uni(P, [&](auto U) { hipLaunchKernelGGL(k_obs_linearize<decltype(U)::value>, dim3((P.O + 255) / 256), dim3(256), 0, st, P, r, Jp, Jl, cost); });
 }
-template <int G, bool UNI>
-__global__ __launch_bounds__(kBuildThreads) void k_lm_outliers(DevProblem P, double th, unsigned char* __restrict__ erase, int* __restrict__ left,
-                                                               unsigned long long* __restrict__ counts) {
-  constexpr int GROUPS = kBuildThreads / G;
-  const int lane = threadIdx.x % G, grp = threadIdx.x / G;
-  const int l = blockIdx.x * GROUPS + grp;
-  const bool lm_ok = l < P.L;
+template <int S, bool UNI>
+COV_DEV void lm_outliers_body(const DevProblem& P, double th, unsigned char* __restrict__ erase, int* __restrict__ left, unsigned long long* __restrict__ counts, int wb) {
+  constexpr int G = kLmSegLanes[S];
+  const int lane = threadIdx.x % G;
+  int l;
+  const bool lm_ok = lm_pick<S>(P, wb, l);
   const int o0 = lm_ok ? P.lm_obs_ptr[l] : 0;
   const int nobs = lm_ok ? P.lm_obs_ptr[l + 1] - o0 : 0;
   double kept = 0.0, bad = 0.0;
@@ -438,10 +609,14 @@
     if (kept < 2.0) atomicAdd(&counts[1], 1ull);
   }
 }
+template <bool UNI>
+__global__ __launch_bounds__(kBuildThreads) void k_lm_outliers(DevProblem P, double th, unsigned char* __restrict__ erase, int* __restrict__ left,
+                                                               unsigned long long* __restrict__ counts) {
+  lm_dispatch(P, blockIdx.x, [&](auto S) { lm_outliers_body<decltype(S)::value, UNI>(P, th, erase, left, counts, blockIdx.x); });
+}
 void launch_lm_outliers(const DevProblem& P, double th, unsigned char* erase, int* left, unsigned long long* counts, hipStream_t st) {
   if (P.L == 0) return;
-  with_uni(P, [&](auto U) { with_group(P.lm_group, [&](auto G) {
-    hipLaunchKernelGGL((k_lm_outliers<decltype(G)::value, decltype(U)::value>), dim3(lm_blocks(P)), dim3(kBuildThreads), 0, st, P, th, erase, left, counts); }); });
+  with_uni(P, [&](auto U) { hipLaunchKernelGGL(k_lm_outliers<decltype(U)::value>, dim3(lm_blocks(P)), dim3(kBuildThreads), 0, st, P, th, erase, left, counts); });
 }
 
 void launch_obs_norms(const DevProblem& P, double* norms, hipStream_t st) {
diff --git a/covins_amd/csrc/solver.hip b/covins_amd/csrc/solver.hip
--- a/covins_amd/csrc/solver.hip
+++ b/covins_amd/csrc/solver.hip
@@ -702,6 +702,21 @@
   }
 }
 
+static int set_lm_work(covgpu_context* c) {
+  DevProblem& P = c->P;
+  int counts[kLmSegs];
+  if (!build_lm_work_device(P.L, P.lm_obs_ptr, P.lm_work, counts, c->st)) { g_err = "landmark work list: device allocation failed"; return COVGPU_ERR_OUT_OF_MEMORY; }
+  int lm = 0, blk = 0;
+  for (int s = 0; s < kLmSegs; ++s) {
+    const int groups = kLmThreads / kLmSegLanes[s];
+    P.lm_seg_lm[s] = lm; P.lm_seg_blk[s] = blk;
+    lm += counts[s]; blk += (counts[s] + groups - 1) / groups;
+  }
+  P.lm_seg_lm[kLmSegs] = lm; P.lm_seg_blk[kLmSegs] = blk;
+  if (lm != P.L || blk > P.L / 4 + 64) { g_err = "landmark work list: inconsistent segment counts"; return COVGPU_ERR_INVALID_ARG; }
+  return COVGPU_OK;
+}
+
 static int upload_impl(covgpu_context* c, const covgpu_options* opt, const covgpu_problem* p, bool pgo, bool allow_arrow = true) {
   HIPCHK(hipSetDevice(c->device));
   static const bool tm_on = getenv("COVGPU_PLAN_TIMING") != nullptr;
@@ -723,10 +738,6 @@
   P.I = vi ? p->num_imu : 0; P.E = p->num_edge;
   P.S = P.I ? p->imu_sample_ptr[P.I] : 0;
   P.vi = vi; P.D = vi ? 15 : 6; P.n = P.D * P.K;
-  {
-    const double mean_track = P.L > 0 ? (double)P.O / P.L : 0.0;
-    P.lm_group = mean_track <= 5.0 ? 4 : (mean_track <= 8.0 ? 8 : 16);
-  }
   P.npad = ((6 * P.K + kTile - 1) / kTile) * kTile;
   P.N = P.n + 3 * P.L;
   std::vector<int> perm, pos_kf, chain_ptr;
@@ -809,6 +820,9 @@
     RC(dev_alloc(c, &P.kobs, (size_t)3 * P.O)); RC(dev_alloc(c, &P.kobs_lm, (size_t)P.O)); RC(dev_alloc(c, &P.obs_zpos, (size_t)P.O));
     launch_kobs_build(P, P.pair_oa, P.pair_ob, pl.nent, c->st);
     RC(dev_alloc(c, &P.cost_part, (size_t)(P.L / 4 + 64)));
+    RC(dev_alloc(c, &P.lm_work, (size_t)std::max(P.L, 1)));
+    RC(dev_alloc(c, &P.obs_jv, (size_t)3 * std::max(P.O, 1)));
+    RC(set_lm_work(c));
     HIPCHK(hipStreamSynchronize(c->st));
     h_pair_i.swap(pi); h_pair_j.swap(pj);
   }
@@ -835,6 +849,7 @@
   RC(dev_alloc(c, &P.pre_delta, (size_t)11 * P.I)); RC(dev_alloc(c, &P.pre_J, (size_t)225 * P.I));
   RC(dev_alloc(c, &P.pre_P, (size_t)225 * P.I)); RC(dev_alloc(c, &P.pre_W, (size_t)225 * P.I));
   RC(dev_alloc(c, &P.pre_bias, (size_t)6 * P.I));
+  RC(dev_alloc(c, &P.imuJ, (size_t)450 * P.I));
   RC(dev_upload(c, &P.edge_i, (const int*)p->edge_i, (size_t)P.E));
   RC(dev_upload(c, &P.edge_j, (const int*)p->edge_j, (size_t)P.E));
   RC(dev_upload(c, &P.edge_meas, p->edge_meas, (size_t)7 * P.E));
@@ -1096,7 +1111,7 @@
   if (c->profiling) (void)hipEventRecord(c->ev[1], c->st);
 }
 
-static void enqueue_solve(covgpu_context* c, double* dst_all) {
+static void enqueue_solve(covgpu_context* c, double* dst_all, bool backsub = true) {
   const DevProblem& P = c->P;
   if (c->profiling) (void)hipEventRecord(c->ev[2], c->st);
   FormScope census(&c->chol.forms);
@@ -1105,7 +1120,7 @@
   }
   else launch_pose_graph_solve(P, dst_all, c->st, c->chol, c->pgo_plan.active ? &c->pgo_plan : nullptr);
   if (c->profiling) (void)hipEventRecord(c->ev[3], c->st);
-  launch_lm_backsub(P, dst_all, dst_all, c->st);
+  if (backsub) launch_lm_backsub(P, dst_all, dst_all, c->st);
 }
 
 static void collect_profile(covgpu_context* c, bool built, bool solved) {
@@ -1232,9 +1247,9 @@
       if (!reuse) {
         const double damp = (o.strategy == COVGPU_LM) ? 1.0 / h[TR_RADIUS] : h[TR_MU];
         enqueue_build(c, damp);
-        enqueue_solve(c, P.gn);
-        launch_tail_stats(P, c->st);
-        launch_tail_jvp(P, two, c->st);
+        enqueue_solve(c, P.gn, false);
+        launch_lm_backsub_jvp(P, two, c->st);
+        launch_tail_stats(P, two, c->st);
         launch_tail_finish(P, tc, 1, two, !coll, 1, c->st);
         if (coll) { reduce_scalars(c); launch_tail_logic(P, tc, 1, 1, c->st); }
       } else launch_tail_logic(P, tc, 1, 0, c->st);
@@ -1405,6 +1420,7 @@
       P.lm0 = R.lm0; P.lm_obs_ptr = R.lm_obs_ptr; P.obs_kf = R.obs_kf; P.obs_lm = R.obs_lm; P.obs_u = R.obs_u; P.obs_v = R.obs_v; P.obs_sigma = R.obs_sigma;
       P.kf_obs_ptr = R.kf_obs_ptr; P.kf_obs_idx = R.kf_obs_idx;
     } else { P.L = 0; P.O = 0; P.N = P.n; }
+    RC(set_lm_work(c));
     if (tr->kf_fixed_round2 != nullptr) {
       HIPCHK(hipMemcpyAsync(P.fixed, tr->kf_fixed_round2, (size_t)P.K, hipMemcpyHostToDevice, c->st));
       std::vector<int> key(P.K);
```

Result: no change. 291.6, median of 2 (+0.4%).
